# AronCao49/MoPA

Hardware: AMD Instinct MI355X
Metric: scans/sec (joint 2D+3D train step) at 1/2/4/8 MI355X; sparse-conv HBM GB/s (higher is better)
Workload: dtype f32

## Files before the change

### include/mopa_hip.h

```cpp
#ifndef MOPA_HIP_H
#define MOPA_HIP_H
#include <stddef.h>
#include <stdint.h>
#ifdef __cplusplus
extern "C" {
#endif


size_t mopa_scan_workspace_bytes(int64_t n);
int mopa_scan_exclusive_i32(const int32_t* in, int32_t* out, int32_t n, int32_t* total, void* ws, size_t ws_bytes, void* stream);
size_t mopa_voxel_hash_workspace_bytes(int64_t n_points);
int mopa_voxel_hash_build(const int64_t* coords, int64_t n_points, uint64_t* table_keys, int32_t* table_vals, int64_t table_cap, int32_t* point_row, uint64_t* row_keys, int32_t* num_rows, int32_t* status, void* ws, size_t ws_bytes, void* stream);
size_t mopa_coarsen_workspace_bytes(int64_t n_fine_cap);
int mopa_coarsen_build(const uint64_t* fine_keys, int32_t n_fine_cap, const int32_t* n_fine_dev, uint64_t* table_keys, int32_t* table_vals, int64_t table_cap, int32_t* parent, uint64_t* coarse_keys, int32_t* num_coarse, void* ws, size_t ws_bytes, void* stream);
int mopa_group_split(const int32_t* item_row, const int32_t* n_dev, int32_t n_host, int32_t n_cap, int32_t* out, void* stream);
int mopa_rulebook_subm(const uint64_t* row_keys, int32_t num_rows, const uint64_t* table_keys, const int32_t* table_vals, int64_t table_cap, int32_t spatial_size, int32_t* nbr , void* stream);
int mopa_rulebook_updown(const uint64_t* fine_keys, const int32_t* parent, int32_t num_fine, int32_t num_coarse, int32_t* ch , int32_t* up , void* stream);
size_t mopa_points_csr_workspace_bytes(int64_t num_rows);
int mopa_points_csr(const int32_t* point_row, int32_t n_points, int32_t num_rows, int32_t* row_start , int32_t* row_points , void* ws, size_t ws_bytes, void* stream);
int mopa_rotate_points_f32(const float* points, int32_t n, const float* rot_host , float* out, void* stream);
size_t mopa_voxelize_workspace_bytes(void);
int mopa_voxelize(const float* points, int32_t n, float scale, int32_t full_scale, const double* u_host, int32_t transl, int64_t batch_index, int64_t* coords , uint8_t* keep , void* ws, size_t ws_bytes, void* stream);

int mopa_spconv_fwd(const int32_t* nbr, int32_t K, int32_t num_out, const float* in, int32_t ld_in, int32_t cin, const float* weight, int32_t cout, int32_t w_flip, float* out, int32_t ld_out, void* stream);
// ... 40 lines not shown
int mopa_bn_act_fwd(const float* x, int32_t ldx, float* y, int32_t ldy, int32_t num_rows, int32_t C, const float* gamma, const float* beta, float* running_mean, float* running_var, float momentum, float eps, float leak, int32_t act, const float* res, int32_t ld_res, int32_t training, float* stats, void* ws, size_t ws_bytes, void* stream);
int mopa_bnrelu_rows_fwd(const float* x, int32_t ldx, float* y, int32_t ldy, int32_t num_rows, int32_t C, const float* gamma, const float* beta, float* running_mean, float* running_var, float momentum, float eps, float leak, int32_t training, float* stats, void* ws, size_t ws_bytes, void* stream);
size_t mopa_bnrelu_rows_bwd_workspace_bytes(int32_t num_rows, int32_t C);
int mopa_bn_act_bwd_groups(const float* dy, int32_t ld_dy, const float* x, int32_t ldx, float* dx, int32_t ld_dx, int32_t num_rows, int32_t C, int32_t n_groups, int32_t split1, int32_t split2, const float* stats, float leak, int32_t act, const float* ymask, int32_t ld_ym, float* dres, int32_t ld_dres, int32_t accumulate_dres, int32_t training, float* dgamma, float* dbeta, int32_t accumulate_param_grads, int32_t accumulate_dx, void* ws, size_t ws_bytes, void* stream);
size_t mopa_bn_act_bwd_groups_fused_workspace_bytes(int32_t num_rows, int32_t C);
int mopa_bn_act_bwd_groups_fused(const float* dy, int32_t ld_dy, const float* x, int32_t ldx, float* dx, int32_t ld_dx, int32_t num_rows, int32_t C, int32_t n_groups, int32_t split1, int32_t split2, const float* stats, float leak, int32_t act, int32_t use_bits, const uint32_t* bits, float* dres, int32_t ld_dres, int32_t accumulate_dres, int32_t training, float* dgamma, float* dbeta, int32_t accumulate_param_grads, int32_t accumulate_dx, float* colsum_partial, void* ws, size_t ws_bytes, void* stream);
int mopa_bn_bwd_sums_groups(const float* dy, int32_t ld_dy, const float* x, int32_t ldx, int32_t num_rows, int32_t C, int32_t n_groups, int32_t split1, int32_t split2, const float* stats, float leak, int32_t act, const float* ymask, int32_t ld_ym, float* dgamma, float* dbeta, int32_t accumulate_param_grads, float* coef_out, void* ws, size_t ws_bytes, void* stream);
int mopa_bn_bwd_sums_groups_pool(const float* dpool, int32_t ld_dpool, const uint8_t* argmax, int32_t B, int32_t H, int32_t W, float* dy, int32_t ld_dy, int32_t accumulate_dy, const float* x, int32_t ldx, int32_t C, int32_t n_groups, const float* stats, float leak, int32_t act, float* dgamma, float* dbeta, int32_t accumulate_param_grads, float* coef_out, void* ws, size_t ws_bytes, void* stream);
int mopa_bn_act_bwd(const float* dy, int32_t ld_dy, const float* x, int32_t ldx, float* dx, int32_t ld_dx, int32_t num_rows, int32_t C, const float* stats, float leak, int32_t act, const float* ymask, int32_t ld_ym, float* dres, int32_t ld_dres, int32_t accumulate_dres, int32_t training, float* dgamma, float* dbeta, int32_t accumulate_param_grads, int32_t accumulate_dx, void* ws, size_t ws_bytes, void* stream);
int mopa_bnrelu_rows_bwd(const float* dy, int32_t ld_dy, const float* x, int32_t ldx, float* dx, int32_t ld_dx, int32_t num_rows, int32_t C, const float* stats, float leak, int32_t training, float* dgamma, float* dbeta, int32_t accumulate_param_grads, int32_t accumulate_dx, void* ws, size_t ws_bytes, void* stream);
int mopa_bn_sync_moments(const float* x, int32_t ldx, int32_t num_rows, int32_t C, double* moments, void* ws, size_t ws_bytes, void* stream);
int mopa_bn_act_fwd_sync(const float* x, int32_t ldx, float* y, int32_t ldy, int32_t num_rows, int32_t C, const float* gamma, const float* beta, float* running_mean, float* running_var, float momentum, float eps, float leak, int32_t act, const float* res, int32_t ld_res, const double* gathered, int32_t world, float* stats, void* stream);
int mopa_bn_sync_bwd_sums(const float* dy, int32_t ld_dy, const float* x, int32_t ldx, int32_t num_rows, int32_t C, const float* stats, float leak, int32_t act, const float* ymask, int32_t ld_ym, float* dgamma, float* dbeta, int32_t accumulate_param_grads, double* sums, void* ws, size_t ws_bytes, void* stream);
int mopa_bn_act_bwd_sync(const float* dy, int32_t ld_dy, const float* x, int32_t ldx, float* dx, int32_t ld_dx, int32_t num_rows, int32_t C, const float* stats, float leak, int32_t act, const float* ymask, int32_t ld_ym, float* dres, int32_t ld_dres, int32_t accumulate_dres, const double* sums_global, const double* gathered, int32_t world, int32_t accumulate_dx, float* coef_ws, void* stream);
int mopa_rows_add(const float* a, int32_t lda, const float* b, int32_t ldb, float* out, int32_t ldo, int32_t rows, int32_t C, void* stream);
int mopa_input_layer_fwd(const float* feats, int32_t cin, const int32_t* row_start, const int32_t* row_points, int32_t num_rows, float* out, int32_t ld_out, void* stream);
int mopa_input_layer_bwd(const float* dout, int32_t ld_dout, const int32_t* point_row, const int32_t* row_start, int32_t n_points, int32_t cin, float* dfeats, void* stream);
int mopa_heads_supported(int32_t M, int32_t num_classes);
int mopa_output_layer_heads_fwd(const float* y, int32_t ld_y, const int32_t* point_row, int32_t n_points, int32_t M, int32_t num_classes, const float* w1, const float* b1, const float* w2, const float* b2, float* feats, float* logit1, float* logit2, void* stream);
size_t mopa_output_layer_heads_bwd_workspace_bytes(int32_t n_points, int32_t M, int32_t num_classes);
int mopa_output_layer_heads_bwd(const float* dfeats, const float* dl1, const float* dl2, const float* feats, const float* w1, const float* w2, const int32_t* row_start, const int32_t* row_points, int32_t num_rows, int32_t n_points, int32_t M, int32_t num_classes, float* dy, int32_t ld_dy, float* dw1, float* db1, float* dw2, float* db2, int32_t accumulate, void* ws, size_t ws_bytes, void* stream);
int mopa_zero_rows(float* x, int32_t ld, int64_t rows, int32_t C, void* stream);
int mopa_copy_rows(const float* src, int32_t ld_src, float* dst, int32_t ld_dst, int64_t rows, int32_t C, void* stream);
int mopa_add_i64_many(const int64_t* ptrs_host, int32_t n, int64_t value, void* stream);

int mopa_conv2d_igemm(const float* in, const float* weight, const float* bias, float* out, const int32_t* geom_host, int32_t flags, void* stream);
int mopa_conv2d_igemm_classes(const float* in, const float* weight, const float* bias, float* out, const int32_t* geom4_host, int32_t flags, void* stream);
int mopa_conv2d_igemm_batched(const float* in, const float* weight, float* out, const int32_t* geom_host, int32_t nbatch, int64_t in_stride, int64_t w_stride, int64_t out_stride, int32_t flags, void* stream);
size_t mopa_conv2d_wgrad_workspace_bytes(const int32_t* geom_host);
int mopa_conv2d_bwd_weight(const float* in, const float* dy, float* dweight, const int32_t* geom_host, int32_t flags, void* ws, size_t ws_bytes, void* stream);
size_t mopa_convt_wgrad_workspace_bytes(const int32_t* geom_host);
int mopa_convt_bwd_weight(const float* in, const float* dy, float* dweight, const int32_t* geom_host, int32_t flags, void* ws, size_t ws_bytes, void* stream);
int mopa_stem_bwd_weight_bn(const float* in, const float* dy, int32_t ld_dy, const float* xbn, int32_t ld_x, const float* stats, const float* coef, int32_t n_groups, int32_t training, float* dweight, const int32_t* geom_host, int32_t flags, void* ws, size_t ws_bytes, void* stream);
int mopa_stem_bwd_weight2(const float* in, const float* dy, float* dweight, const int32_t* geom_host, int32_t flags, void* ws, size_t ws_bytes, void* stream);
int mopa_stem_bwd_weight_bn2(const float* in, const float* dy, int32_t ld_dy, const float* xbn, int32_t ld_x, const float* stats, const float* coef, int32_t n_groups, int32_t training, float* dweight, const int32_t* geom_host, int32_t flags, void* ws, size_t ws_bytes, void* stream);
int mopa_stem_fwd(const float* in, const float* weight, float* out, const int32_t* geom_host, void* stream);
size_t mopa_wino_wgrad_workspace_bytes(int32_t T, int32_t Cin, int32_t Cout);
int mopa_wino_bwd_weight(const float* V, const float* dM, int32_t T, int32_t Cin, int32_t Cout, float* dweight, int32_t flags, void* ws, size_t ws_bytes, void* stream);
size_t mopa_wino4_wgrad_workspace_bytes(int32_t T, int32_t Cin, int32_t Cout);
int mopa_wino4_bwd_weight(const float* V, const float* dM, int32_t T, int32_t Cin, int32_t Cout, float* dweight, int32_t flags, void* ws, size_t ws_bytes, void* stream);
int mopa_conv2d_relayout_weight(const float* src, float* dst, int32_t O, int32_t I, int32_t KH, int32_t KW, int32_t mode, int32_t inverse, int32_t accumulate, void* stream);
int mopa_conv2d_stem_relayout(const float* src, float* dst, int32_t O, int32_t inverse, int32_t accumulate, void* stream);
int mopa_img_to_nhwc4(const float* img, int32_t B, int32_t H, int32_t W, int32_t Hp, int32_t Wp, float* out, void* stream);
int mopa_stem_dgrad_image(const float* dout, int32_t ld, int32_t B, int32_t Hp, int32_t Wp, int32_t H, int32_t W, const float* w, float* dimg, void* stream);

int mopa_wino_weight(const float* weight, int32_t O, int32_t I, int32_t dgrad, float* U, void* stream);
int mopa_wino_input(const float* in, int32_t ld_in, int32_t B, int32_t H, int32_t W, int32_t C, float* V, void* stream);
int mopa_wino_output(const float* M, int32_t B, int32_t H, int32_t W, int32_t C, const float* bias, float* out, int32_t ld_out, int32_t accumulate, void* stream);
int mopa_wino_dout(const float* dy, int32_t ld, int32_t B, int32_t H, int32_t W, int32_t C, float* dM, void* stream);
int mopa_wino4_weight(const float* weight, int32_t O, int32_t I, int32_t dgrad, float* U, void* stream);
int mopa_wino4_input(const float* in, int32_t ld_in, int32_t B, int32_t H, int32_t W, int32_t C, float* V, void* stream);
int mopa_wino4_input_bn(const float* in, int32_t ld_in, int32_t B, int32_t H, int32_t W, int32_t C, const float* stats, int32_t n_groups, int32_t bn_c0, float* V, void* stream);
int mopa_wino4_output(const float* M, int32_t B, int32_t H, int32_t W, int32_t C, const float* bias, float* out, int32_t ld_out, int32_t accumulate, void* stream);
int mopa_wino4_dout(const float* dy, int32_t ld, int32_t B, int32_t H, int32_t W, int32_t C, float* dM, void* stream);
int mopa_conv2d_weight_forms_batched(const int64_t* desc_host, int32_t n, void* stream);
int mopa_wino4_weight_t(const float* weight, int32_t O, int32_t I, int32_t dgrad, float* Ut, void* stream);
int mopa_wino4_gemm_output(const float* V, const float* Ut, const float* bias, float* out, int32_t ld_out, int32_t B, int32_t H, int32_t W, int32_t Cin, int32_t Cout, int32_t accumulate, void* stream);
int mopa_wino4_weight_f(const float* weight, int32_t O, int32_t I, int32_t dgrad, float* Uf, void* stream);
int mopa_wino4_weight_q(const float* weight, int32_t O, int32_t I, int32_t dgrad, float* Uq, void* stream);
int mopa_wino4_conv_tiles32(int32_t mode);
int mopa_wino4_conv(const float* in, int32_t ld_in, const float* Uf, const float* bias, float* out, int32_t ld_out, int32_t B, int32_t H, int32_t W, int32_t Cin, int32_t Cout, int32_t accumulate, const float* stats, int32_t n_groups, int32_t bn_c0, float* V, void* stream);

int mopa_wino4_conv9(const float* in, int32_t ld_in, const float* Uq, const float* bias, float* out, int32_t ld_out, int32_t B, int32_t H, int32_t W, int32_t Cin, int32_t Cout, int32_t accumulate, const float* stats, int32_t n_groups, int32_t bn_c0, void* stream);

int mopa_wino4_wgrad_fused_ok(int32_t B, int32_t H, int32_t W, int32_t Cin, int32_t Cout);
size_t mopa_wino4_wgrad_fused_workspace_bytes(int32_t B, int32_t H, int32_t W, int32_t Cin, int32_t Cout);
int mopa_wino4_wgrad_fused(const float* in, int32_t ld_in, const float* stats, int32_t n_groups, int32_t bn_c0, const float* dy, int32_t ld_dy, int32_t B, int32_t H, int32_t W, int32_t Cin, int32_t Cout, float* dweight, int32_t flags, void* ws, size_t ws_bytes, void* stream);

int mopa_maxpool3x3s2_fwd(const float* x, int32_t ldx, int32_t B, int32_t H, int32_t W, int32_t C, float* y, int32_t ldy, uint8_t* argmax, void* stream);
int mopa_maxpool3x3s2_fwd_bn(const float* x, int32_t ldx, int32_t B, int32_t H, int32_t W, int32_t C, const float* stats, int32_t n_groups, float* y, int32_t ldy, uint8_t* argmax, void* stream);
int mopa_maxpool3x3s2_bwd(const float* dy, int32_t ld_dy, const uint8_t* argmax, int32_t B, int32_t H, int32_t W, int32_t C, float* dx, int32_t ld_dx, int32_t accumulate, void* stream);
int mopa_dropout_rows(const float* x, int32_t ldx, float* y, int32_t ldy, int64_t rows, int32_t C, float p, uint64_t seed, void* stream);
int mopa_dropout_rows_dseed(const float* x, int32_t ldx, float* y, int32_t ldy, int64_t rows, int32_t C, float p, const int64_t* seed_dev, int32_t site, void* stream);
int mopa_pixel_head_supported(int32_t M, int32_t num_classes);
int mopa_pixel_head_fwd(const float* x, int32_t ld, int32_t B, int32_t Hp, int32_t Wp, int32_t H, int32_t W, int32_t M, int32_t num_classes, const float* w, const float* bias, float* pred, void* stream);
size_t mopa_pixel_head_bwd_workspace_bytes(int32_t B, int32_t H, int32_t W, int32_t M, int32_t num_classes);
int mopa_pixel_head_bwd(const float* dpred, const float* x, int32_t ld, int32_t B, int32_t Hp, int32_t Wp, int32_t H, int32_t W, int32_t M, int32_t num_classes, const float* w, float* dx, int32_t ld_dx, int32_t accumulate_dx, float* dw, float* db, int32_t accumulate_params, void* ws, size_t ws_bytes, void* stream);
size_t mopa_colsum_workspace_bytes(int64_t num_rows, int32_t C);
int mopa_colsum(const float* x, int32_t ld, int64_t num_rows, int32_t C, float* out, int32_t accumulate, void* ws, size_t ws_bytes, void* stream);
size_t mopa_colsum_partial_blocks(int64_t num_rows);
int mopa_colsum_reduce(const float* partial, int64_t num_rows, int32_t C, float* out, int32_t accumulate, void* stream);
int mopa_pack_point_pix(const int64_t* idx, const int64_t* off_host, int32_t B, int32_t H, int32_t W, int32_t* pix, int32_t* status, void* stream);

size_t mopa_loss_workspace_bytes(int64_t n_rows);
int mopa_softmax_kl_fwd(const float* logit_p, const float* logit_q, int32_t N, int32_t C, float* loss, void* ws, size_t ws_bytes, void* stream);
int mopa_softmax_kl_bwd(const float* logit_p, const float* logit_q, int32_t N, int32_t C, const float* gout, float* dlogit_p, void* stream);
int mopa_wce_fwd(const float* logits, const int64_t* labels, const float* class_weight, int32_t N, int32_t C, int64_t ignore_index, float* loss, float* den, int32_t* status, void* ws, size_t ws_bytes, void* stream);
int mopa_wce_bwd(const float* logits, const int64_t* labels, const float* class_weight, int32_t N, int32_t C, int64_t ignore_index, const float* den, const float* gout, float* dlogits, void* stream);
size_t mopa_point_losses_workspace_bytes(int64_t n_rows);
int mopa_point_losses_fwd(const float* z2_main, const float* z2_xm, const float* z3_main, const float* z3_xm, const int64_t* y2, const int64_t* y3, const float* class_weight, int32_t N, int32_t C, int64_t ignore_index, float* scalars, int64_t* conf_2d, int64_t* conf_3d, const uint8_t* acc_mask, int64_t* acc_out, int32_t* status, void* ws, size_t ws_bytes, void* stream);
int mopa_point_losses_bwd(const float* z_main, const float* z_xm, const float* z_other_main, const int64_t* y, const float* class_weight, int32_t N, int32_t C, int64_t ignore_index, const float* den, const float* g, float* dz_main, float* dz_xm, void* stream);
size_t mopa_point_losses_seg_workspace_bytes(int32_t S);
int mopa_point_losses_seg_fwd(const float* z2_main, const float* z2_xm, const float* z3_main, const float* z3_xm, const float* class_weight, const int64_t* segs_host, int32_t S, int64_t N2, int64_t N3, int32_t C, int64_t ignore_index, float* scalars, int32_t* status, void* ws, size_t ws_bytes, void* stream);
int mopa_point_losses_seg_bwd(int32_t net, const float* z_main, const float* z_xm, const float* z_other_main, const float* class_weight, const int64_t* segs_host, int32_t S, int64_t N, int64_t N_other, int32_t C, int64_t ignore_index, const float* scalars, const float* g, float* dz_main, float* dz_xm, void* stream);
int mopa_softmax_fwd(const float* logits, int64_t n_rows, int32_t C, float* probs, void* stream);
int mopa_softmax_bwd(const float* probs, const float* dprobs, int64_t n_rows, int32_t C, float* dlogits, void* stream);
size_t mopa_mask_cons_workspace_bytes(int32_t B, int32_t HW, int32_t C);
size_t mopa_mask_cons_state_floats(int32_t B, int32_t C);
int mopa_mask_cons_fwd(const float* probs, const int32_t* masks, int32_t B, int32_t HW, int32_t C, int32_t k_norm, int32_t min_entropy, float* loss, float* state, void* ws, size_t ws_bytes, void* stream);
int mopa_mask_cons_bwd(const float* probs, const int32_t* masks, int32_t B, int32_t HW, int32_t C, int32_t k_norm, int32_t min_entropy, const float* state, const float* gout, float* dprobs, void* stream);

int mopa_pseudo_fuse(const float* logit_a, const float* logit_b, int32_t N, int32_t C, float* maxp, int64_t* label, void* stream);
size_t mopa_refine_pseudo_labels_workspace_bytes(int32_t C);
int mopa_refine_pseudo_labels(const float* prob, const int64_t* label_in, int32_t N, int32_t C, int64_t ignore_label, int64_t* label_out, void* ws, size_t ws_bytes, void* stream);
int mopa_ema_update(float* shadow, const float* param, int64_t n, float decay, void* stream);

int mopa_vgi_zslots(void);
int mopa_vgi_first_points(const float* points, int32_t stride, int32_t n, float voxel_size, int32_t ox, int32_t oy, int32_t X, int32_t Y, int32_t zlo, const uint8_t* g_mask, int32_t* first, int32_t* status, void* stream);
size_t mopa_vgi_first_points_rep_workspace_bytes(int32_t X, int32_t Y);
int mopa_vgi_first_points_rep(const float* points, int32_t stride, int32_t n, float voxel_size, double voxel_size64, int32_t ox, int32_t oy, int32_t X, int32_t Y, int32_t zlo, int32_t* first, int32_t* status, void* ws, size_t ws_bytes, void* stream);
size_t mopa_vgi_box_free_workspace_bytes(int32_t X, int32_t Y, int32_t Z);
int mopa_vgi_box_free(const int32_t* first, int32_t X, int32_t Y, int32_t zlo, int32_t gz0, int32_t Z, int32_t bx, int32_t by, int32_t bz, uint8_t* free_cells, void* ws, size_t ws_bytes, void* stream);
int mopa_vgi_ground_cells(const int32_t* first, const uint8_t* g_mask, int32_t X, int32_t Y, uint8_t* ground2d, void* stream);
int mopa_vgi_candidates(const uint8_t* free_cells, int32_t Xo, int32_t Yo, int32_t Zo, const double* params_host, const uint8_t* ground2d, int32_t ox, int32_t oy, int32_t X, int32_t Y, uint8_t* cand2d, int32_t* counts, void* stream);
int mopa_vgi_compact_cells(const uint8_t* cand2d, int32_t X, int32_t Y, int32_t ox, int32_t oy, int32_t* cells , int32_t* count, void* stream);
int mopa_vgi_road_height(const float* points, int32_t stride, int32_t n, float voxel_size, const int32_t* first, const uint8_t* g_mask, int32_t ox, int32_t oy, int32_t X, int32_t Y, int32_t zlo, int32_t cell_x, int32_t cell_y, double* out , void* stream);
// ... 96 lines not shown
```

### mopa_amd/_abi.py

```python
SIGNATURES = {
    'mopa_scan_workspace_bytes': ('z', 'l'),
    'mopa_scan_exclusive_i32': ('i', 'ppippzp'),
    'mopa_voxel_hash_workspace_bytes': ('z', 'l'),
    'mopa_voxel_hash_build': ('i', 'plpplpppppzp'),
    'mopa_coarsen_workspace_bytes': ('z', 'l'),
    'mopa_coarsen_build': ('i', 'pippplppppzp'),
    'mopa_group_split': ('i', 'ppiipp'),
    'mopa_rulebook_subm': ('i', 'pipplipp'),
    'mopa_rulebook_updown': ('i', 'ppiippp'),
    'mopa_points_csr_workspace_bytes': ('z', 'l'),
    'mopa_points_csr': ('i', 'piipppzp'),
    'mopa_rotate_points_f32': ('i', 'pippp'),
    'mopa_voxelize_workspace_bytes': ('z', ''),
    'mopa_voxelize': ('i', 'pifipilpppzp'),
    'mopa_spconv_fwd': ('i', 'piipiipiipip'),
    'mopa_rulebook_groups_count': ('i', 'piipp'),
    'mopa_rulebook_groups_fill': ('i', 'piippppp'),
    'mopa_rulebook_groups_count_batched': ('i', 'piipp'),
    'mopa_rulebook_groups_fill_batched': ('i', 'piippppp'),
    'mopa_spconv_grouped_wants_packed': ('i', 'iiii'),
    'mopa_spconv_pack_weight': ('i', 'piiiiipp'),
    'mopa_spconv_pack_weights_batched': ('i', 'pip'),
    'mopa_spconv_grouped_workspace_bytes': ('z', 'iii'),
    'mopa_spconv_fwd_grouped': ('i', 'ppppiipiipiipipzp'),
# ... 25 lines not shown
    'mopa_bn_act_fwd_groups': ('i', 'pipiiiiiippppfffipiippzp'),
    'mopa_bn_act_fwd_groups_bits': ('i', 'pipiiiiiippppfffipiipippzp'),
    'mopa_bn_act_fwd': ('i', 'pipiiippppfffipiippzp'),
    'mopa_bnrelu_rows_fwd': ('i', 'pipiiippppfffippzp'),
    'mopa_bnrelu_rows_bwd_workspace_bytes': ('z', 'ii'),
    'mopa_bn_act_bwd_groups': ('i', 'pipipiiiiiipfipipiiippiipzp'),
    'mopa_bn_act_bwd_groups_fused_workspace_bytes': ('z', 'ii'),
    'mopa_bn_act_bwd_groups_fused': ('i', 'pipipiiiiiipfiippiiippiippzp'),
    'mopa_bn_bwd_sums_groups': ('i', 'pipiiiiiipfipippippzp'),
    'mopa_bn_bwd_sums_groups_pool': ('i', 'pipiiipiipiiipfippippzp'),
    'mopa_bn_act_bwd': ('i', 'pipipiiipfipipiiippiipzp'),
    'mopa_bnrelu_rows_bwd': ('i', 'pipipiiipfippiipzp'),
    'mopa_bn_sync_moments': ('i', 'piiippzp'),
    'mopa_bn_act_fwd_sync': ('i', 'pipiiippppfffipipipp'),
    'mopa_bn_sync_bwd_sums': ('i', 'pipiiipfipippippzp'),
    'mopa_bn_act_bwd_sync': ('i', 'pipipiiipfipipiippiipp'),
    'mopa_rows_add': ('i', 'pipipiiip'),
    'mopa_input_layer_fwd': ('i', 'pippipip'),
    'mopa_input_layer_bwd': ('i', 'pippiipp'),
    'mopa_heads_supported': ('i', 'ii'),
    'mopa_output_layer_heads_fwd': ('i', 'pipiiipppppppp'),
    'mopa_output_layer_heads_bwd_workspace_bytes': ('z', 'iii'),
    'mopa_output_layer_heads_bwd': ('i', 'ppppppppiiiipippppipzp'),
    'mopa_zero_rows': ('i', 'pilip'),
    'mopa_copy_rows': ('i', 'pipilip'),
    'mopa_add_i64_many': ('i', 'pilp'),
    'mopa_conv2d_igemm': ('i', 'pppppip'),
    'mopa_conv2d_igemm_classes': ('i', 'pppppip'),
    'mopa_conv2d_igemm_batched': ('i', 'ppppilllip'),
    'mopa_conv2d_wgrad_workspace_bytes': ('z', 'p'),
    'mopa_conv2d_bwd_weight': ('i', 'ppppipzp'),
    'mopa_convt_wgrad_workspace_bytes': ('z', 'p'),
    'mopa_convt_bwd_weight': ('i', 'ppppipzp'),
    'mopa_stem_bwd_weight_bn': ('i', 'ppipippiippipzp'),
    'mopa_stem_bwd_weight2': ('i', 'ppppipzp'),
    'mopa_stem_bwd_weight_bn2': ('i', 'ppipippiippipzp'),
    'mopa_stem_fwd': ('i', 'ppppp'),
    'mopa_wino_wgrad_workspace_bytes': ('z', 'iii'),
    'mopa_wino_bwd_weight': ('i', 'ppiiipipzp'),
    'mopa_wino4_wgrad_workspace_bytes': ('z', 'iii'),
    'mopa_wino4_bwd_weight': ('i', 'ppiiipipzp'),
    'mopa_conv2d_relayout_weight': ('i', 'ppiiiiiiip'),
    'mopa_conv2d_stem_relayout': ('i', 'ppiiip'),
    'mopa_img_to_nhwc4': ('i', 'piiiiipp'),
    'mopa_stem_dgrad_image': ('i', 'piiiiiippp'),
    'mopa_wino_weight': ('i', 'piiipp'),
    'mopa_wino_input': ('i', 'piiiiipp'),
    'mopa_wino_output': ('i', 'piiiippiip'),
    'mopa_wino_dout': ('i', 'piiiiipp'),
    'mopa_wino4_weight': ('i', 'piiipp'),
    'mopa_wino4_input': ('i', 'piiiiipp'),
    'mopa_wino4_input_bn': ('i', 'piiiiipiipp'),
    'mopa_wino4_output': ('i', 'piiiippiip'),
    'mopa_wino4_dout': ('i', 'piiiiipp'),
    'mopa_conv2d_weight_forms_batched': ('i', 'pip'),
    'mopa_wino4_weight_t': ('i', 'piiipp'),
    'mopa_wino4_gemm_output': ('i', 'ppppiiiiiiip'),
    'mopa_wino4_weight_f': ('i', 'piiipp'),
    'mopa_wino4_weight_q': ('i', 'piiipp'),
    'mopa_wino4_conv_tiles32': ('i', 'i'),
    'mopa_wino4_conv': ('i', 'pipppiiiiiiipiipp'),
    'mopa_wino4_conv9': ('i', 'pipppiiiiiiipiip'),
    'mopa_wino4_wgrad_fused_ok': ('i', 'iiiii'),
    'mopa_wino4_wgrad_fused_workspace_bytes': ('z', 'iiiii'),
    'mopa_wino4_wgrad_fused': ('i', 'pipiipiiiiiipipzp'),
    'mopa_maxpool3x3s2_fwd': ('i', 'piiiiipipp'),
    'mopa_maxpool3x3s2_fwd_bn': ('i', 'piiiiipipipp'),
    'mopa_maxpool3x3s2_bwd': ('i', 'pipiiiipiip'),
    'mopa_dropout_rows': ('i', 'pipilifup'),
    'mopa_dropout_rows_dseed': ('i', 'pipilifpip'),
    'mopa_pixel_head_supported': ('i', 'ii'),
    'mopa_pixel_head_fwd': ('i', 'piiiiiiiipppp'),
    'mopa_pixel_head_bwd_workspace_bytes': ('z', 'iiiii'),
    'mopa_pixel_head_bwd': ('i', 'ppiiiiiiiippiippipzp'),
    'mopa_colsum_workspace_bytes': ('z', 'li'),
    'mopa_colsum': ('i', 'pilipipzp'),
    'mopa_colsum_partial_blocks': ('z', 'l'),
    'mopa_colsum_reduce': ('i', 'plipip'),
    'mopa_pack_point_pix': ('i', 'ppiiippp'),
    'mopa_loss_workspace_bytes': ('z', 'l'),
    'mopa_softmax_kl_fwd': ('i', 'ppiippzp'),
    'mopa_softmax_kl_bwd': ('i', 'ppiippp'),
    'mopa_wce_fwd': ('i', 'pppiilppppzp'),
    'mopa_wce_bwd': ('i', 'pppiilpppp'),
    'mopa_point_losses_workspace_bytes': ('z', 'l'),
    'mopa_point_losses_fwd': ('i', 'pppppppiilpppppppzp'),
    'mopa_point_losses_bwd': ('i', 'pppppiilppppp'),
    'mopa_point_losses_seg_workspace_bytes': ('z', 'i'),
    'mopa_point_losses_seg_fwd': ('i', 'ppppppillilpppzp'),
    'mopa_point_losses_seg_bwd': ('i', 'ipppppillilppppp'),
    'mopa_softmax_fwd': ('i', 'plipp'),
    'mopa_softmax_bwd': ('i', 'pplipp'),
    'mopa_mask_cons_workspace_bytes': ('z', 'iii'),
    'mopa_mask_cons_state_floats': ('z', 'ii'),
    'mopa_mask_cons_fwd': ('i', 'ppiiiiipppzp'),
    'mopa_mask_cons_bwd': ('i', 'ppiiiiipppp'),
    'mopa_pseudo_fuse': ('i', 'ppiippp'),
    'mopa_refine_pseudo_labels_workspace_bytes': ('z', 'i'),
    'mopa_refine_pseudo_labels': ('i', 'ppiilppzp'),
    'mopa_ema_update': ('i', 'pplfp'),
    'mopa_vgi_zslots': ('i', ''),
    'mopa_vgi_first_points': ('i', 'piifiiiiipppp'),
    'mopa_vgi_first_points_rep_workspace_bytes': ('z', 'ii'),
    'mopa_vgi_first_points_rep': ('i', 'piifdiiiiipppzp'),
    'mopa_vgi_box_free_workspace_bytes': ('z', 'iii'),
    'mopa_vgi_box_free': ('i', 'piiiiiiiippzp'),
    'mopa_vgi_ground_cells': ('i', 'ppiipp'),
    'mopa_vgi_candidates': ('i', 'piiippiiiippp'),
    'mopa_vgi_compact_cells': ('i', 'piiiippp'),
    'mopa_vgi_road_height': ('i', 'piifppiiiiiiipp'),
    'mopa_vgi_range_keep_workspace_bytes': ('z', 'iii'),
    'mopa_vgi_range_keep': ('i', 'piiddiippzp'),
    'mopa_voxelize_f64_workspace_bytes': ('z', ''),
    'mopa_voxelize_f64': ('i', 'pippdipilpppzp'),
    'mopa_eval_logits_workspace_bytes': ('z', 'ii'),
# ... 135 lines not shown
```

### mopa_amd/csrc/common.h

```cpp
#pragma once
#include <hip/hip_runtime.h>
#include <stdint.h>
#include <stddef.h>

#define MOPA_OK 0
#define MOPA_ERR_ARG (-1)
#define MOPA_ERR_WORKSPACE (-2)
#define MOPA_ERR_LAUNCH (-3)
#define MOPA_ERR_UNSUPPORTED (-4)
#define MOPA_ERR_DATA (-5)

#define MOPA_API extern "C" __attribute__((visibility("default")))

#define MOPA_CHECK_LAUNCH()                                  \
  do {                                                       \
    if (hipGetLastError() != hipSuccess) return MOPA_ERR_LAUNCH; \
  } while (0)

static inline int64_t cdiv64(int64_t a, int64_t b) { return (a + b - 1) / b; }
static inline size_t align_up(size_t x, size_t a) { return (x + a - 1) / a * a; }
static inline int colsum_rows(int64_t num_rows) {
  int64_t r = cdiv64(num_rows, 2048);
  if (r < 32) r = 32;
  if (r > 1024) r = 1024;
  return (int)r;
}

static inline int stream_grid(int64_t work_items, int block) {
  int64_t g = cdiv64(work_items, block);
  if (g < 1) g = 1;
  if (g > 2048) g = 2048;
  return (int)g;
}

#include <atomic>
static inline int mopa_device_index() {
  int dev = 0;
  return hipGetDevice(&dev) == hipSuccess && dev >= 0 && dev < 64 ? dev : -1;
}
static inline int mopa_cu_count() {
  static std::atomic<int> cus[64];
  const int dev = mopa_device_index();
  if (dev < 0) return 0;
  int n = cus[dev].load(std::memory_order_relaxed);
  if (n == 0) {
    hipDeviceProp_t prop;
    if (hipGetDeviceProperties(&prop, dev) != hipSuccess) return 0;
    n = prop.multiProcessorCount > 0 ? prop.multiProcessorCount : 256;
    cus[dev].store(n, std::memory_order_relaxed);
  }
  return n;
}

#define WAVE 64

__device__ __forceinline__ float wave_sum(float v) {
#pragma unroll
  for (int o = 32; o > 0; o >>= 1) v += __shfl_xor(v, o, 64);
  return v;
}
__device__ __forceinline__ double wave_sum_d(double v) {
#pragma unroll
  for (int o = 32; o > 0; o >>= 1) v += __shfl_xor(v, o, 64);
  return v;
}
__device__ __forceinline__ int wave_sum_i(int v) {
#pragma unroll
  for (int o = 32; o > 0; o >>= 1) v += __shfl_xor(v, o, 64);
  return v;
}
```

### mopa_amd/csrc/exec_table.inc

```
static const char* const EXEC_NAMES[] = {
  "mopa_a2d2prep_map",
  "mopa_a2d2prep_points",
  "mopa_a2d2prep_remap",
  "mopa_adam_flat",
  "mopa_adam_flat_guarded",
  "mopa_adamw_flat",
  "mopa_adamw_flat_guarded",
  "mopa_add_i64_many",
  "mopa_bn_act_bwd",
  "mopa_bn_act_bwd_groups",
  "mopa_bn_act_bwd_groups_fused",
  "mopa_bn_act_bwd_sync",
  "mopa_bn_act_fwd",
  "mopa_bn_act_fwd_groups",
  "mopa_bn_act_fwd_groups_bits",
  "mopa_bn_act_fwd_sync",
  "mopa_bn_bwd_sums_groups",
  "mopa_bn_bwd_sums_groups_pool",
  "mopa_bn_sync_bwd_sums",
  "mopa_bn_sync_moments",
  "mopa_bnrelu_rows_bwd",
  "mopa_bnrelu_rows_fwd",
  "mopa_coarsen_build",
  "mopa_colsum",
// ... 55 lines not shown
  "mopa_refine_pseudo_labels_segmented",
  "mopa_rotate_points_f32",
  "mopa_rows_add",
  "mopa_rulebook_groups_count",
  "mopa_rulebook_groups_count_batched",
  "mopa_rulebook_groups_fill",
  "mopa_rulebook_groups_fill_batched",
  "mopa_rulebook_runs_build_batched",
  "mopa_rulebook_subm",
  "mopa_rulebook_updown",
  "mopa_scan_exclusive_i32",
  "mopa_scanprep_compact",
  "mopa_scanprep_count",
  "mopa_scanprep_rotate",
  "mopa_scanprep_take",
  "mopa_scn_backward",
  "mopa_scn_forward",
  "mopa_sgd_flat",
  "mopa_sgd_flat_guarded",
  "mopa_softmax_bwd",
  "mopa_softmax_fwd",
  "mopa_softmax_kl_bwd",
  "mopa_softmax_kl_fwd",
  "mopa_spconv_bwd_weight",
  "mopa_spconv_bwd_weight_run",
  "mopa_spconv_fwd",
  "mopa_spconv_fwd_grouped",
  "mopa_spconv_fwd_run",
  "mopa_spconv_pack_weight",
  "mopa_spconv_pack_weights_batched",
  "mopa_spconv_run_pack_weight",
  "mopa_spconv_transpose_weight",
  "mopa_stem_bwd_weight2",
  "mopa_stem_bwd_weight_bn",
  "mopa_stem_bwd_weight_bn2",
  "mopa_stem_dgrad_image",
  "mopa_stem_fwd",
  "mopa_vgi_box_free",
  "mopa_vgi_candidates",
  "mopa_vgi_compact_cells",
  "mopa_vgi_first_points",
  "mopa_vgi_first_points_rep",
  "mopa_vgi_ground_cells",
  "mopa_vgi_range_keep",
  "mopa_vgi_road_height",
  "mopa_voxel_hash_build",
  "mopa_voxelize",
  "mopa_voxelize_f64",
  "mopa_wce_bwd",
  "mopa_wce_fwd",
  "mopa_wino4_bwd_weight",
  "mopa_wino4_conv",
  "mopa_wino4_conv9",
  "mopa_wino4_dout",
  "mopa_wino4_gemm_output",
  "mopa_wino4_input",
  "mopa_wino4_input_bn",
  "mopa_wino4_output",
  "mopa_wino4_weight",
  "mopa_wino4_weight_f",
  "mopa_wino4_weight_q",
  "mopa_wino4_weight_t",
  "mopa_wino4_wgrad_fused",
  "mopa_wino_bwd_weight",
  "mopa_wino_dout",
  "mopa_wino_input",
  "mopa_wino_output",
  "mopa_wino_weight",
  "mopa_zero_rows",
};
static const int EXEC_N = 148;
static int exec_dispatch(int id, const int64_t* a, int nargs) {
  switch (id) {
    case 0: return nargs == 6 ? mopa_a2d2prep_map((const double*)(uintptr_t)a[0], (int32_t)a[1], (int32_t)a[2], (int16_t*)(uintptr_t)a[3], (uint16_t*)(uintptr_t)a[4], (void*)(uintptr_t)a[5]) : MOPA_ERR_ARG;
    case 1: return nargs == 21 ? mopa_a2d2prep_points((const void* const*)(uintptr_t)a[0], (const void* const*)(uintptr_t)a[1], (const void* const*)(uintptr_t)a[2], (const void* const*)(uintptr_t)a[3], (const void* const*)(uintptr_t)a[4], (const int32_t*)(uintptr_t)a[5], (int32_t)a[6], (int32_t)a[7], (int32_t)a[8], (const int16_t*)(uintptr_t)a[9], (const uint16_t*)(uintptr_t)a[10], (int32_t)a[11], (int32_t)a[12], (const uint8_t*)(uintptr_t)a[13], (int32_t)a[14], (float*)(uintptr_t)a[15], (float*)(uintptr_t)a[16], (uint8_t*)(uintptr_t)a[17], (float*)(uintptr_t)a[18], (int32_t*)(uintptr_t)a[19], (void*)(uintptr_t)a[20]) : MOPA_ERR_ARG;
    case 2: return nargs == 8 ? mopa_a2d2prep_remap((const void* const*)(uintptr_t)a[0], (void* const*)(uintptr_t)a[1], (int32_t)a[2], (int32_t)a[3], (int32_t)a[4], (const int16_t*)(uintptr_t)a[5], (const uint16_t*)(uintptr_t)a[6], (void*)(uintptr_t)a[7]) : MOPA_ERR_ARG;
    case 3: return nargs == 14 ? mopa_adam_flat((float*)(uintptr_t)a[0], (const float*)(uintptr_t)a[1], (float*)(uintptr_t)a[2], (float*)(uintptr_t)a[3], (int64_t)a[4], (float)slot_f(a[5]), (float)slot_f(a[6]), (float)slot_f(a[7]), (float)slot_f(a[8]), (float)slot_f(a[9]), (float)slot_f(a[10]), (float)slot_f(a[11]), (float)slot_f(a[12]), (void*)(uintptr_t)a[13]) : MOPA_ERR_ARG;
    case 4: return nargs == 15 ? mopa_adam_flat_guarded((float*)(uintptr_t)a[0], (const float*)(uintptr_t)a[1], (float*)(uintptr_t)a[2], (float*)(uintptr_t)a[3], (int64_t)a[4], (float)slot_f(a[5]), (float)slot_f(a[6]), (float)slot_f(a[7]), (float)slot_f(a[8]), (float)slot_f(a[9]), (float)slot_f(a[10]), (float)slot_f(a[11]), (float)slot_f(a[12]), (const void*)(uintptr_t)a[13], (void*)(uintptr_t)a[14]) : MOPA_ERR_ARG;
    case 5: return nargs == 14 ? mopa_adamw_flat((float*)(uintptr_t)a[0], (const float*)(uintptr_t)a[1], (float*)(uintptr_t)a[2], (float*)(uintptr_t)a[3], (int64_t)a[4], (float)slot_f(a[5]), (float)slot_f(a[6]), (float)slot_f(a[7]), (float)slot_f(a[8]), (float)slot_f(a[9]), (float)slot_f(a[10]), (float)slot_f(a[11]), (float)slot_f(a[12]), (void*)(uintptr_t)a[13]) : MOPA_ERR_ARG;
    case 6: return nargs == 15 ? mopa_adamw_flat_guarded((float*)(uintptr_t)a[0], (const float*)(uintptr_t)a[1], (float*)(uintptr_t)a[2], (float*)(uintptr_t)a[3], (int64_t)a[4], (float)slot_f(a[5]), (float)slot_f(a[6]), (float)slot_f(a[7]), (float)slot_f(a[8]), (float)slot_f(a[9]), (float)slot_f(a[10]), (float)slot_f(a[11]), (float)slot_f(a[12]), (const void*)(uintptr_t)a[13], (void*)(uintptr_t)a[14]) : MOPA_ERR_ARG;
    case 7: return nargs == 4 ? mopa_add_i64_many((const int64_t*)(uintptr_t)a[0], (int32_t)a[1], (int64_t)a[2], (void*)(uintptr_t)a[3]) : MOPA_ERR_ARG;
    case 8: return nargs == 24 ? mopa_bn_act_bwd((const float*)(uintptr_t)a[0], (int32_t)a[1], (const float*)(uintptr_t)a[2], (int32_t)a[3], (float*)(uintptr_t)a[4], (int32_t)a[5], (int32_t)a[6], (int32_t)a[7], (const float*)(uintptr_t)a[8], (float)slot_f(a[9]), (int32_t)a[10], (const float*)(uintptr_t)a[11], (int32_t)a[12], (float*)(uintptr_t)a[13], (int32_t)a[14], (int32_t)a[15], (int32_t)a[16], (float*)(uintptr_t)a[17], (float*)(uintptr_t)a[18], (int32_t)a[19], (int32_t)a[20], (void*)(uintptr_t)a[21], (size_t)a[22], (void*)(uintptr_t)a[23]) : MOPA_ERR_ARG;
    case 9: return nargs == 27 ? mopa_bn_act_bwd_groups((const float*)(uintptr_t)a[0], (int32_t)a[1], (const float*)(uintptr_t)a[2], (int32_t)a[3], (float*)(uintptr_t)a[4], (int32_t)a[5], (int32_t)a[6], (int32_t)a[7], (int32_t)a[8], (int32_t)a[9], (int32_t)a[10], (const float*)(uintptr_t)a[11], (float)slot_f(a[12]), (int32_t)a[13], (const float*)(uintptr_t)a[14], (int32_t)a[15], (float*)(uintptr_t)a[16], (int32_t)a[17], (int32_t)a[18], (int32_t)a[19], (float*)(uintptr_t)a[20], (float*)(uintptr_t)a[21], (int32_t)a[22], (int32_t)a[23], (void*)(uintptr_t)a[24], (size_t)a[25], (void*)(uintptr_t)a[26]) : MOPA_ERR_ARG;
    case 10: return nargs == 28 ? mopa_bn_act_bwd_groups_fused((const float*)(uintptr_t)a[0], (int32_t)a[1], (const float*)(uintptr_t)a[2], (int32_t)a[3], (float*)(uintptr_t)a[4], (int32_t)a[5], (int32_t)a[6], (int32_t)a[7], (int32_t)a[8], (int32_t)a[9], (int32_t)a[10], (const float*)(uintptr_t)a[11], (float)slot_f(a[12]), (int32_t)a[13], (int32_t)a[14], (const uint32_t*)(uintptr_t)a[15], (float*)(uintptr_t)a[16], (int32_t)a[17], (int32_t)a[18], (int32_t)a[19], (float*)(uintptr_t)a[20], (float*)(uintptr_t)a[21], (int32_t)a[22], (int32_t)a[23], (float*)(uintptr_t)a[24], (void*)(uintptr_t)a[25], (size_t)a[26], (void*)(uintptr_t)a[27]) : MOPA_ERR_ARG;
    case 11: return nargs == 22 ? mopa_bn_act_bwd_sync((const float*)(uintptr_t)a[0], (int32_t)a[1], (const float*)(uintptr_t)a[2], (int32_t)a[3], (float*)(uintptr_t)a[4], (int32_t)a[5], (int32_t)a[6], (int32_t)a[7], (const float*)(uintptr_t)a[8], (float)slot_f(a[9]), (int32_t)a[10], (const float*)(uintptr_t)a[11], (int32_t)a[12], (float*)(uintptr_t)a[13], (int32_t)a[14], (int32_t)a[15], (const double*)(uintptr_t)a[16], (const double*)(uintptr_t)a[17], (int32_t)a[18], (int32_t)a[19], (float*)(uintptr_t)a[20], (void*)(uintptr_t)a[21]) : MOPA_ERR_ARG;
    case 12: return nargs == 21 ? mopa_bn_act_fwd((const float*)(uintptr_t)a[0], (int32_t)a[1], (float*)(uintptr_t)a[2], (int32_t)a[3], (int32_t)a[4], (int32_t)a[5], (const float*)(uintptr_t)a[6], (const float*)(uintptr_t)a[7], (float*)(uintptr_t)a[8], (float*)(uintptr_t)a[9], (float)slot_f(a[10]), (float)slot_f(a[11]), (float)slot_f(a[12]), (int32_t)a[13], (const float*)(uintptr_t)a[14], (int32_t)a[15], (int32_t)a[16], (float*)(uintptr_t)a[17], (void*)(uintptr_t)a[18], (size_t)a[19], (void*)(uintptr_t)a[20]) : MOPA_ERR_ARG;
    case 13: return nargs == 24 ? mopa_bn_act_fwd_groups((const float*)(uintptr_t)a[0], (int32_t)a[1], (float*)(uintptr_t)a[2], (int32_t)a[3], (int32_t)a[4], (int32_t)a[5], (int32_t)a[6], (int32_t)a[7], (int32_t)a[8], (const float*)(uintptr_t)a[9], (const float*)(uintptr_t)a[10], (float*)(uintptr_t)a[11], (float*)(uintptr_t)a[12], (float)slot_f(a[13]), (float)slot_f(a[14]), (float)slot_f(a[15]), (int32_t)a[16], (const float*)(uintptr_t)a[17], (int32_t)a[18], (int32_t)a[19], (float*)(uintptr_t)a[20], (void*)(uintptr_t)a[21], (size_t)a[22], (void*)(uintptr_t)a[23]) : MOPA_ERR_ARG;
    case 14: return nargs == 26 ? mopa_bn_act_fwd_groups_bits((const float*)(uintptr_t)a[0], (int32_t)a[1], (float*)(uintptr_t)a[2], (int32_t)a[3], (int32_t)a[4], (int32_t)a[5], (int32_t)a[6], (int32_t)a[7], (int32_t)a[8], (const float*)(uintptr_t)a[9], (const float*)(uintptr_t)a[10], (float*)(uintptr_t)a[11], (float*)(uintptr_t)a[12], (float)slot_f(a[13]), (float)slot_f(a[14]), (float)slot_f(a[15]), (int32_t)a[16], (const float*)(uintptr_t)a[17], (int32_t)a[18], (int32_t)a[19], (float*)(uintptr_t)a[20], (int32_t)a[21], (uint32_t*)(uintptr_t)a[22], (void*)(uintptr_t)a[23], (size_t)a[24], (void*)(uintptr_t)a[25]) : MOPA_ERR_ARG;
    case 15: return nargs == 20 ? mopa_bn_act_fwd_sync((const float*)(uintptr_t)a[0], (int32_t)a[1], (float*)(uintptr_t)a[2], (int32_t)a[3], (int32_t)a[4], (int32_t)a[5], (const float*)(uintptr_t)a[6], (const float*)(uintptr_t)a[7], (float*)(uintptr_t)a[8], (float*)(uintptr_t)a[9], (float)slot_f(a[10]), (float)slot_f(a[11]), (float)slot_f(a[12]), (int32_t)a[13], (const float*)(uintptr_t)a[14], (int32_t)a[15], (const double*)(uintptr_t)a[16], (int32_t)a[17], (float*)(uintptr_t)a[18], (void*)(uintptr_t)a[19]) : MOPA_ERR_ARG;
    case 16: return nargs == 21 ? mopa_bn_bwd_sums_groups((const float*)(uintptr_t)a[0], (int32_t)a[1], (const float*)(uintptr_t)a[2], (int32_t)a[3], (int32_t)a[4], (int32_t)a[5], (int32_t)a[6], (int32_t)a[7], (int32_t)a[8], (const float*)(uintptr_t)a[9], (float)slot_f(a[10]), (int32_t)a[11], (const float*)(uintptr_t)a[12], (int32_t)a[13], (float*)(uintptr_t)a[14], (float*)(uintptr_t)a[15], (int32_t)a[16], (float*)(uintptr_t)a[17], (void*)(uintptr_t)a[18], (size_t)a[19], (void*)(uintptr_t)a[20]) : MOPA_ERR_ARG;
    case 17: return nargs == 23 ? mopa_bn_bwd_sums_groups_pool((const float*)(uintptr_t)a[0], (int32_t)a[1], (const uint8_t*)(uintptr_t)a[2], (int32_t)a[3], (int32_t)a[4], (int32_t)a[5], (float*)(uintptr_t)a[6], (int32_t)a[7], (int32_t)a[8], (const float*)(uintptr_t)a[9], (int32_t)a[10], (int32_t)a[11], (int32_t)a[12], (const float*)(uintptr_t)a[13], (float)slot_f(a[14]), (int32_t)a[15], (float*)(uintptr_t)a[16], (float*)(uintptr_t)a[17], (int32_t)a[18], (float*)(uintptr_t)a[19], (void*)(uintptr_t)a[20], (size_t)a[21], (void*)(uintptr_t)a[22]) : MOPA_ERR_ARG;
    case 18: return nargs == 18 ? mopa_bn_sync_bwd_sums((const float*)(uintptr_t)a[0], (int32_t)a[1], (const float*)(uintptr_t)a[2], (int32_t)a[3], (int32_t)a[4], (int32_t)a[5], (const float*)(uintptr_t)a[6], (float)slot_f(a[7]), (int32_t)a[8], (const float*)(uintptr_t)a[9], (int32_t)a[10], (float*)(uintptr_t)a[11], (float*)(uintptr_t)a[12], (int32_t)a[13], (double*)(uintptr_t)a[14], (void*)(uintptr_t)a[15], (size_t)a[16], (void*)(uintptr_t)a[17]) : MOPA_ERR_ARG;
    case 19: return nargs == 8 ? mopa_bn_sync_moments((const float*)(uintptr_t)a[0], (int32_t)a[1], (int32_t)a[2], (int32_t)a[3], (double*)(uintptr_t)a[4], (void*)(uintptr_t)a[5], (size_t)a[6], (void*)(uintptr_t)a[7]) : MOPA_ERR_ARG;
    case 20: return nargs == 18 ? mopa_bnrelu_rows_bwd((const float*)(uintptr_t)a[0], (int32_t)a[1], (const float*)(uintptr_t)a[2], (int32_t)a[3], (float*)(uintptr_t)a[4], (int32_t)a[5], (int32_t)a[6], (int32_t)a[7], (const float*)(uintptr_t)a[8], (float)slot_f(a[9]), (int32_t)a[10], (float*)(uintptr_t)a[11], (float*)(uintptr_t)a[12], (int32_t)a[13], (int32_t)a[14], (void*)(uintptr_t)a[15], (size_t)a[16], (void*)(uintptr_t)a[17]) : MOPA_ERR_ARG;
    case 21: return nargs == 18 ? mopa_bnrelu_rows_fwd((const float*)(uintptr_t)a[0], (int32_t)a[1], (float*)(uintptr_t)a[2], (int32_t)a[3], (int32_t)a[4], (int32_t)a[5], (const float*)(uintptr_t)a[6], (const float*)(uintptr_t)a[7], (float*)(uintptr_t)a[8], (float*)(uintptr_t)a[9], (float)slot_f(a[10]), (float)slot_f(a[11]), (float)slot_f(a[12]), (int32_t)a[13], (float*)(uintptr_t)a[14], (void*)(uintptr_t)a[15], (size_t)a[16], (void*)(uintptr_t)a[17]) : MOPA_ERR_ARG;
    case 22: return nargs == 12 ? mopa_coarsen_build((const uint64_t*)(uintptr_t)a[0], (int32_t)a[1], (const int32_t*)(uintptr_t)a[2], (uint64_t*)(uintptr_t)a[3], (int32_t*)(uintptr_t)a[4], (int64_t)a[5], (int32_t*)(uintptr_t)a[6], (uint64_t*)(uintptr_t)a[7], (int32_t*)(uintptr_t)a[8], (void*)(uintptr_t)a[9], (size_t)a[10], (void*)(uintptr_t)a[11]) : MOPA_ERR_ARG;
    case 23: return nargs == 9 ? mopa_colsum((const float*)(uintptr_t)a[0], (int32_t)a[1], (int64_t)a[2], (int32_t)a[3], (float*)(uintptr_t)a[4], (int32_t)a[5], (void*)(uintptr_t)a[6], (size_t)a[7], (void*)(uintptr_t)a[8]) : MOPA_ERR_ARG;
    case 24: return nargs == 6 ? mopa_colsum_reduce((const float*)(uintptr_t)a[0], (int64_t)a[1], (int32_t)a[2], (float*)(uintptr_t)a[3], (int32_t)a[4], (void*)(uintptr_t)a[5]) : MOPA_ERR_ARG;
    case 25: return nargs == 8 ? mopa_confusion_update((const int64_t*)(uintptr_t)a[0], (const int64_t*)(uintptr_t)a[1], (int64_t)a[2], (const int32_t*)(uintptr_t)a[3], (int32_t)a[4], (int32_t)a[5], (int64_t*)(uintptr_t)a[6], (void*)(uintptr_t)a[7]) : MOPA_ERR_ARG;
    case 26: return nargs == 8 ? mopa_conv2d_bwd_weight((const float*)(uintptr_t)a[0], (const float*)(uintptr_t)a[1], (float*)(uintptr_t)a[2], (const int32_t*)(uintptr_t)a[3], (int32_t)a[4], (void*)(uintptr_t)a[5], (size_t)a[6], (void*)(uintptr_t)a[7]) : MOPA_ERR_ARG;
    case 27: return nargs == 7 ? mopa_conv2d_igemm((const float*)(uintptr_t)a[0], (const float*)(uintptr_t)a[1], (const float*)(uintptr_t)a[2], (float*)(uintptr_t)a[3], (const int32_t*)(uintptr_t)a[4], (int32_t)a[5], (void*)(uintptr_t)a[6]) : MOPA_ERR_ARG;
    case 28: return nargs == 10 ? mopa_conv2d_igemm_batched((const float*)(uintptr_t)a[0], (const float*)(uintptr_t)a[1], (float*)(uintptr_t)a[2], (const int32_t*)(uintptr_t)a[3], (int32_t)a[4], (int64_t)a[5], (int64_t)a[6], (int64_t)a[7], (int32_t)a[8], (void*)(uintptr_t)a[9]) : MOPA_ERR_ARG;
    case 29: return nargs == 7 ? mopa_conv2d_igemm_classes((const float*)(uintptr_t)a[0], (const float*)(uintptr_t)a[1], (const float*)(uintptr_t)a[2], (float*)(uintptr_t)a[3], (const int32_t*)(uintptr_t)a[4], (int32_t)a[5], (void*)(uintptr_t)a[6]) : MOPA_ERR_ARG;
    case 30: return nargs == 10 ? mopa_conv2d_relayout_weight((const float*)(uintptr_t)a[0], (float*)(uintptr_t)a[1], (int32_t)a[2], (int32_t)a[3], (int32_t)a[4], (int32_t)a[5], (int32_t)a[6], (int32_t)a[7], (int32_t)a[8], (void*)(uintptr_t)a[9]) : MOPA_ERR_ARG;
    case 31: return nargs == 6 ? mopa_conv2d_stem_relayout((const float*)(uintptr_t)a[0], (float*)(uintptr_t)a[1], (int32_t)a[2], (int32_t)a[3], (int32_t)a[4], (void*)(uintptr_t)a[5]) : MOPA_ERR_ARG;
    case 32: return nargs == 3 ? mopa_conv2d_weight_forms_batched((const int64_t*)(uintptr_t)a[0], (int32_t)a[1], (void*)(uintptr_t)a[2]) : MOPA_ERR_ARG;
    case 33: return nargs == 8 ? mopa_convt_bwd_weight((const float*)(uintptr_t)a[0], (const float*)(uintptr_t)a[1], (float*)(uintptr_t)a[2], (const int32_t*)(uintptr_t)a[3], (int32_t)a[4], (void*)(uintptr_t)a[5], (size_t)a[6], (void*)(uintptr_t)a[7]) : MOPA_ERR_ARG;
    case 34: return nargs == 7 ? mopa_copy_rows((const float*)(uintptr_t)a[0], (int32_t)a[1], (float*)(uintptr_t)a[2], (int32_t)a[3], (int64_t)a[4], (int32_t)a[5], (void*)(uintptr_t)a[6]) : MOPA_ERR_ARG;
    case 35: return nargs == 20 ? mopa_denselabels((const void* const*)(uintptr_t)a[0], (const void* const*)(uintptr_t)a[1], (const void* const*)(uintptr_t)a[2], (int)a[3], (const int32_t*)(uintptr_t)a[4], (const void* const*)(uintptr_t)a[5], (int)a[6], (int)a[7], (int)a[8], (int)a[9], (int)a[10], (const int32_t*)(uintptr_t)a[11], (int)a[12], (int)a[13], (const int32_t*)(uintptr_t)a[14], (int32_t*)(uintptr_t)a[15], (int32_t*)(uintptr_t)a[16], (void*)(uintptr_t)a[17], (size_t)a[18], (void*)(uintptr_t)a[19]) : MOPA_ERR_ARG;
    case 36: return nargs == 9 ? mopa_dropout_rows((const float*)(uintptr_t)a[0], (int32_t)a[1], (float*)(uintptr_t)a[2], (int32_t)a[3], (int64_t)a[4], (int32_t)a[5], (float)slot_f(a[6]), (uint64_t)a[7], (void*)(uintptr_t)a[8]) : MOPA_ERR_ARG;
    case 37: return nargs == 10 ? mopa_dropout_rows_dseed((const float*)(uintptr_t)a[0], (int32_t)a[1], (float*)(uintptr_t)a[2], (int32_t)a[3], (int64_t)a[4], (int32_t)a[5], (float)slot_f(a[6]), (const int64_t*)(uintptr_t)a[7], (int32_t)a[8], (void*)(uintptr_t)a[9]) : MOPA_ERR_ARG;
    case 38: return nargs == 5 ? mopa_ema_update((float*)(uintptr_t)a[0], (const float*)(uintptr_t)a[1], (int64_t)a[2], (float)slot_f(a[3]), (void*)(uintptr_t)a[4]) : MOPA_ERR_ARG;
    case 39: return nargs == 20 ? mopa_eval_logits((const float*)(uintptr_t)a[0], (int64_t)a[1], (const float*)(uintptr_t)a[2], (int64_t)a[3], (const int64_t*)(uintptr_t)a[4], (int32_t)a[5], (int32_t)a[6], (const int32_t*)(uintptr_t)a[7], (int32_t)a[8], (int32_t)a[9], (int64_t*)(uintptr_t)a[10], (int64_t*)(uintptr_t)a[11], (int64_t*)(uintptr_t)a[12], (int64_t*)(uintptr_t)a[13], (float*)(uintptr_t)a[14], (uint8_t*)(uintptr_t)a[15], (float*)(uintptr_t)a[16], (void*)(uintptr_t)a[17], (size_t)a[18], (void*)(uintptr_t)a[19]) : MOPA_ERR_ARG;
    case 40: return nargs == 12 ? mopa_grad_stats((const float*)(uintptr_t)a[0], (const void*)(uintptr_t)a[1], (int64_t)a[2], (int64_t)a[3], (float)slot_f(a[4]), (float)slot_f(a[5]), (int)a[6], (float*)(uintptr_t)a[7], (void*)(uintptr_t)a[8], (void*)(uintptr_t)a[9], (size_t)a[10], (void*)(uintptr_t)a[11]) : MOPA_ERR_ARG;
    case 41: return nargs == 11 ? mopa_ground_estimate((const float*)(uintptr_t)a[0], (int32_t)a[1], (const int32_t*)(uintptr_t)a[2], (int32_t)a[3], (int64_t)a[4], (int64_t)a[5], (const double*)(uintptr_t)a[6], (uint8_t*)(uintptr_t)a[7], (void*)(uintptr_t)a[8], (size_t)a[9], (void*)(uintptr_t)a[10]) : MOPA_ERR_ARG;
    case 42: return nargs == 6 ? mopa_group_split((const int32_t*)(uintptr_t)a[0], (const int32_t*)(uintptr_t)a[1], (int32_t)a[2], (int32_t)a[3], (int32_t*)(uintptr_t)a[4], (void*)(uintptr_t)a[5]) : MOPA_ERR_ARG;
    case 43: return nargs == 9 ? mopa_imageprep_contrast_sums((const void* const*)(uintptr_t)a[0], (int)a[1], (int64_t)a[2], (int)a[3], (int)a[4], (const int32_t*)(uintptr_t)a[5], (const float*)(uintptr_t)a[6], (void*)(uintptr_t)a[7], (void*)(uintptr_t)a[8]) : MOPA_ERR_ARG;
    case 44: return nargs == 10 ? mopa_imageprep_contrast_sums4((const void* const*)(uintptr_t)a[0], (int)a[1], (int64_t)a[2], (int)a[3], (int)a[4], (const int32_t*)(uintptr_t)a[5], (const float*)(uintptr_t)a[6], (const int32_t*)(uintptr_t)a[7], (void*)(uintptr_t)a[8], (void*)(uintptr_t)a[9]) : MOPA_ERR_ARG;
    case 45: return nargs == 15 ? mopa_imageprep_indices((const void* const*)(uintptr_t)a[0], (const int32_t*)(uintptr_t)a[1], (int)a[2], (int)a[3], (int)a[4], (double)slot_f(a[5]), (double)slot_f(a[6]), (const int32_t*)(uintptr_t)a[7], (int)a[8], (const int32_t*)(uintptr_t)a[9], (void* const*)(uintptr_t)a[10], (void* const*)(uintptr_t)a[11], (void* const*)(uintptr_t)a[12], (int32_t*)(uintptr_t)a[13], (void*)(uintptr_t)a[14]) : MOPA_ERR_ARG;
    case 46: return nargs == 20 ? mopa_imageprep_mask((const void* const*)(uintptr_t)a[0], (int)a[1], (int)a[2], (int)a[3], (const int32_t*)(uintptr_t)a[4], (const int32_t*)(uintptr_t)a[5], (int)a[6], (int)a[7], (int)a[8], (int)a[9], (const int32_t*)(uintptr_t)a[10], (const int32_t*)(uintptr_t)a[11], (const int32_t*)(uintptr_t)a[12], (int)a[13], (int)a[14], (const int32_t*)(uintptr_t)a[15], (int32_t*)(uintptr_t)a[16], (void*)(uintptr_t)a[17], (size_t)a[18], (void*)(uintptr_t)a[19]) : MOPA_ERR_ARG;
    case 47: return nargs == 14 ? mopa_imageprep_pixels((const void* const*)(uintptr_t)a[0], (int)a[1], (int64_t)a[2], (int)a[3], (int)a[4], (const int32_t*)(uintptr_t)a[5], (const float*)(uintptr_t)a[6], (const void*)(uintptr_t)a[7], (const int32_t*)(uintptr_t)a[8], (uint8_t*)(uintptr_t)a[9], (float*)(uintptr_t)a[10], (const float*)(uintptr_t)a[11], (float*)(uintptr_t)a[12], (void*)(uintptr_t)a[13]) : MOPA_ERR_ARG;
    case 48: return nargs == 15 ? mopa_imageprep_pixels4((const void* const*)(uintptr_t)a[0], (int)a[1], (int64_t)a[2], (int)a[3], (int)a[4], (const int32_t*)(uintptr_t)a[5], (const float*)(uintptr_t)a[6], (const int32_t*)(uintptr_t)a[7], (const void*)(uintptr_t)a[8], (const int32_t*)(uintptr_t)a[9], (uint8_t*)(uintptr_t)a[10], (float*)(uintptr_t)a[11], (const float*)(uintptr_t)a[12], (float*)(uintptr_t)a[13], (void*)(uintptr_t)a[14]) : MOPA_ERR_ARG;
    case 49: return nargs == 13 ? mopa_imageprep_resize_u8((const void* const*)(uintptr_t)a[0], (int)a[1], (int)a[2], (int)a[3], (const int32_t*)(uintptr_t)a[4], (int)a[5], (const int32_t*)(uintptr_t)a[6], (int)a[7], (int)a[8], (int)a[9], (int)a[10], (uint8_t*)(uintptr_t)a[11], (void*)(uintptr_t)a[12]) : MOPA_ERR_ARG;
    case 50: return nargs == 8 ? mopa_img_to_nhwc4((const float*)(uintptr_t)a[0], (int32_t)a[1], (int32_t)a[2], (int32_t)a[3], (int32_t)a[4], (int32_t)a[5], (float*)(uintptr_t)a[6], (void*)(uintptr_t)a[7]) : MOPA_ERR_ARG;
// ... 28 lines not shown
    case 79: return nargs == 11 ? mopa_refine_pseudo_labels_segmented((const void* const*)(uintptr_t)a[0], (const void* const*)(uintptr_t)a[1], (int32_t)a[2], (const int32_t*)(uintptr_t)a[3], (void* const*)(uintptr_t)a[4], (int32_t)a[5], (int32_t)a[6], (int64_t)a[7], (void*)(uintptr_t)a[8], (size_t)a[9], (void*)(uintptr_t)a[10]) : MOPA_ERR_ARG;
    case 80: return nargs == 5 ? mopa_rotate_points_f32((const float*)(uintptr_t)a[0], (int32_t)a[1], (const float*)(uintptr_t)a[2], (float*)(uintptr_t)a[3], (void*)(uintptr_t)a[4]) : MOPA_ERR_ARG;
    case 81: return nargs == 9 ? mopa_rows_add((const float*)(uintptr_t)a[0], (int32_t)a[1], (const float*)(uintptr_t)a[2], (int32_t)a[3], (float*)(uintptr_t)a[4], (int32_t)a[5], (int32_t)a[6], (int32_t)a[7], (void*)(uintptr_t)a[8]) : MOPA_ERR_ARG;
    case 82: return nargs == 5 ? mopa_rulebook_groups_count((const int32_t*)(uintptr_t)a[0], (int32_t)a[1], (int32_t)a[2], (int32_t*)(uintptr_t)a[3], (void*)(uintptr_t)a[4]) : MOPA_ERR_ARG;
    case 83: return nargs == 5 ? mopa_rulebook_groups_count_batched((const int64_t*)(uintptr_t)a[0], (int32_t)a[1], (int32_t)a[2], (int32_t*)(uintptr_t)a[3], (void*)(uintptr_t)a[4]) : MOPA_ERR_ARG;
    case 84: return nargs == 8 ? mopa_rulebook_groups_fill((const int32_t*)(uintptr_t)a[0], (int32_t)a[1], (int32_t)a[2], (const int32_t*)(uintptr_t)a[3], (int32_t*)(uintptr_t)a[4], (int32_t*)(uintptr_t)a[5], (int32_t*)(uintptr_t)a[6], (void*)(uintptr_t)a[7]) : MOPA_ERR_ARG;
    case 85: return nargs == 8 ? mopa_rulebook_groups_fill_batched((const int64_t*)(uintptr_t)a[0], (int32_t)a[1], (int32_t)a[2], (const int32_t*)(uintptr_t)a[3], (int32_t*)(uintptr_t)a[4], (int32_t*)(uintptr_t)a[5], (int32_t*)(uintptr_t)a[6], (void*)(uintptr_t)a[7]) : MOPA_ERR_ARG;
    case 86: return nargs == 3 ? mopa_rulebook_runs_build_batched((const int64_t*)(uintptr_t)a[0], (int32_t)a[1], (void*)(uintptr_t)a[2]) : MOPA_ERR_ARG;
    case 87: return nargs == 8 ? mopa_rulebook_subm((const uint64_t*)(uintptr_t)a[0], (int32_t)a[1], (const uint64_t*)(uintptr_t)a[2], (const int32_t*)(uintptr_t)a[3], (int64_t)a[4], (int32_t)a[5], (int32_t*)(uintptr_t)a[6], (void*)(uintptr_t)a[7]) : MOPA_ERR_ARG;
    case 88: return nargs == 7 ? mopa_rulebook_updown((const uint64_t*)(uintptr_t)a[0], (const int32_t*)(uintptr_t)a[1], (int32_t)a[2], (int32_t)a[3], (int32_t*)(uintptr_t)a[4], (int32_t*)(uintptr_t)a[5], (void*)(uintptr_t)a[6]) : MOPA_ERR_ARG;
    case 89: return nargs == 7 ? mopa_scan_exclusive_i32((const int32_t*)(uintptr_t)a[0], (int32_t*)(uintptr_t)a[1], (int32_t)a[2], (int32_t*)(uintptr_t)a[3], (void*)(uintptr_t)a[4], (size_t)a[5], (void*)(uintptr_t)a[6]) : MOPA_ERR_ARG;
    case 90: return nargs == 22 ? mopa_scanprep_compact((const void* const*)(uintptr_t)a[0], (const void* const*)(uintptr_t)a[1], (const int32_t*)(uintptr_t)a[2], (const double*)(uintptr_t)a[3], (const int32_t*)(uintptr_t)a[4], (int32_t)a[5], (int32_t)a[6], (int32_t)a[7], (float)slot_f(a[8]), (int32_t)a[9], (int32_t)a[10], (const uint8_t*)(uintptr_t)a[11], (int64_t*)(uintptr_t)a[12], (int64_t*)(uintptr_t)a[13], (int64_t*)(uintptr_t)a[14], (int64_t)a[15], (uint8_t*)(uintptr_t)a[16], (int64_t*)(uintptr_t)a[17], (int32_t*)(uintptr_t)a[18], (void*)(uintptr_t)a[19], (size_t)a[20], (void*)(uintptr_t)a[21]) : MOPA_ERR_ARG;
    case 91: return nargs == 15 ? mopa_scanprep_count((const void* const*)(uintptr_t)a[0], (const void* const*)(uintptr_t)a[1], (const int32_t*)(uintptr_t)a[2], (const double*)(uintptr_t)a[3], (const int32_t*)(uintptr_t)a[4], (int32_t)a[5], (int32_t)a[6], (float)slot_f(a[7]), (int32_t)a[8], (int32_t)a[9], (uint8_t*)(uintptr_t)a[10], (int64_t*)(uintptr_t)a[11], (void*)(uintptr_t)a[12], (size_t)a[13], (void*)(uintptr_t)a[14]) : MOPA_ERR_ARG;
    case 92: return nargs == 6 ? mopa_scanprep_rotate((const void* const*)(uintptr_t)a[0], (void* const*)(uintptr_t)a[1], (const int32_t*)(uintptr_t)a[2], (const float*)(uintptr_t)a[3], (int32_t)a[4], (void*)(uintptr_t)a[5]) : MOPA_ERR_ARG;
    case 93: return nargs == 20 ? mopa_scanprep_take((const int64_t*)(uintptr_t)a[0], (int64_t)a[1], (int64_t)a[2], (const int32_t*)(uintptr_t)a[3], (int32_t)a[4], (const void* const*)(uintptr_t)a[5], (int32_t)a[6], (const int64_t*)(uintptr_t)a[7], (int64_t)a[8], (int64_t)a[9], (const void* const*)(uintptr_t)a[10], (const void* const*)(uintptr_t)a[11], (const int64_t*)(uintptr_t)a[12], (const int64_t*)(uintptr_t)a[13], (int64_t*)(uintptr_t)a[14], (int64_t*)(uintptr_t)a[15], (float*)(uintptr_t)a[16], (int64_t*)(uintptr_t)a[17], (int64_t*)(uintptr_t)a[18], (void*)(uintptr_t)a[19]) : MOPA_ERR_ARG;
    case 94: return nargs == 14 ? mopa_scn_backward((const int32_t*)(uintptr_t)a[0], (int32_t)a[1], (const int32_t*)(uintptr_t)a[2], (int32_t)a[3], (const int64_t*)(uintptr_t)a[4], (int64_t*)(uintptr_t)a[5], (const int64_t*)(uintptr_t)a[6], (const int64_t*)(uintptr_t)a[7], (const int64_t*)(uintptr_t)a[8], (const int64_t*)(uintptr_t)a[9], (const int64_t*)(uintptr_t)a[10], (void*)(uintptr_t)a[11], (size_t)a[12], (void*)(uintptr_t)a[13]) : MOPA_ERR_ARG;
    case 95: return nargs == 10 ? mopa_scn_forward((const int32_t*)(uintptr_t)a[0], (int32_t)a[1], (const int64_t*)(uintptr_t)a[2], (int64_t*)(uintptr_t)a[3], (const int64_t*)(uintptr_t)a[4], (const int64_t*)(uintptr_t)a[5], (const int64_t*)(uintptr_t)a[6], (void*)(uintptr_t)a[7], (size_t)a[8], (void*)(uintptr_t)a[9]) : MOPA_ERR_ARG;
    case 96: return nargs == 12 ? mopa_sgd_flat((float*)(uintptr_t)a[0], (const float*)(uintptr_t)a[1], (float*)(uintptr_t)a[2], (int64_t)a[3], (float)slot_f(a[4]), (float)slot_f(a[5]), (float)slot_f(a[6]), (float)slot_f(a[7]), (int)a[8], (int)a[9], (float)slot_f(a[10]), (void*)(uintptr_t)a[11]) : MOPA_ERR_ARG;
    case 97: return nargs == 13 ? mopa_sgd_flat_guarded((float*)(uintptr_t)a[0], (const float*)(uintptr_t)a[1], (float*)(uintptr_t)a[2], (int64_t)a[3], (float)slot_f(a[4]), (float)slot_f(a[5]), (float)slot_f(a[6]), (float)slot_f(a[7]), (int)a[8], (int*)(uintptr_t)a[9], (float)slot_f(a[10]), (const void*)(uintptr_t)a[11], (void*)(uintptr_t)a[12]) : MOPA_ERR_ARG;
    case 98: return nargs == 6 ? mopa_softmax_bwd((const float*)(uintptr_t)a[0], (const float*)(uintptr_t)a[1], (int64_t)a[2], (int32_t)a[3], (float*)(uintptr_t)a[4], (void*)(uintptr_t)a[5]) : MOPA_ERR_ARG;
    case 99: return nargs == 5 ? mopa_softmax_fwd((const float*)(uintptr_t)a[0], (int64_t)a[1], (int32_t)a[2], (float*)(uintptr_t)a[3], (void*)(uintptr_t)a[4]) : MOPA_ERR_ARG;
    case 100: return nargs == 7 ? mopa_softmax_kl_bwd((const float*)(uintptr_t)a[0], (const float*)(uintptr_t)a[1], (int32_t)a[2], (int32_t)a[3], (const float*)(uintptr_t)a[4], (float*)(uintptr_t)a[5], (void*)(uintptr_t)a[6]) : MOPA_ERR_ARG;
    case 101: return nargs == 8 ? mopa_softmax_kl_fwd((const float*)(uintptr_t)a[0], (const float*)(uintptr_t)a[1], (int32_t)a[2], (int32_t)a[3], (float*)(uintptr_t)a[4], (void*)(uintptr_t)a[5], (size_t)a[6], (void*)(uintptr_t)a[7]) : MOPA_ERR_ARG;
    case 102: return nargs == 14 ? mopa_spconv_bwd_weight((const int32_t*)(uintptr_t)a[0], (int32_t)a[1], (int32_t)a[2], (const float*)(uintptr_t)a[3], (int32_t)a[4], (int32_t)a[5], (const float*)(uintptr_t)a[6], (int32_t)a[7], (int32_t)a[8], (float*)(uintptr_t)a[9], (int32_t)a[10], (void*)(uintptr_t)a[11], (size_t)a[12], (void*)(uintptr_t)a[13]) : MOPA_ERR_ARG;
    case 103: return nargs == 16 ? mopa_spconv_bwd_weight_run((const int32_t*)(uintptr_t)a[0], (int32_t)a[1], (int32_t)a[2], (int32_t)a[3], (int32_t)a[4], (const float*)(uintptr_t)a[5], (int32_t)a[6], (int32_t)a[7], (const float*)(uintptr_t)a[8], (int32_t)a[9], (int32_t)a[10], (float*)(uintptr_t)a[11], (int32_t)a[12], (void*)(uintptr_t)a[13], (size_t)a[14], (void*)(uintptr_t)a[15]) : MOPA_ERR_ARG;
    case 104: return nargs == 12 ? mopa_spconv_fwd((const int32_t*)(uintptr_t)a[0], (int32_t)a[1], (int32_t)a[2], (const float*)(uintptr_t)a[3], (int32_t)a[4], (int32_t)a[5], (const float*)(uintptr_t)a[6], (int32_t)a[7], (int32_t)a[8], (float*)(uintptr_t)a[9], (int32_t)a[10], (void*)(uintptr_t)a[11]) : MOPA_ERR_ARG;
    case 105: return nargs == 17 ? mopa_spconv_fwd_grouped((const int32_t*)(uintptr_t)a[0], (const int32_t*)(uintptr_t)a[1], (const int32_t*)(uintptr_t)a[2], (const int32_t*)(uintptr_t)a[3], (int32_t)a[4], (int32_t)a[5], (const float*)(uintptr_t)a[6], (int32_t)a[7], (int32_t)a[8], (const float*)(uintptr_t)a[9], (int32_t)a[10], (int32_t)a[11], (float*)(uintptr_t)a[12], (int32_t)a[13], (void*)(uintptr_t)a[14], (size_t)a[15], (void*)(uintptr_t)a[16]) : MOPA_ERR_ARG;
    case 106: return nargs == 15 ? mopa_spconv_fwd_run((const int32_t*)(uintptr_t)a[0], (int32_t)a[1], (int32_t)a[2], (const float*)(uintptr_t)a[3], (int32_t)a[4], (int32_t)a[5], (const float*)(uintptr_t)a[6], (int32_t)a[7], (int32_t)a[8], (float*)(uintptr_t)a[9], (int32_t)a[10], (int32_t)a[11], (void*)(uintptr_t)a[12], (size_t)a[13], (void*)(uintptr_t)a[14]) : MOPA_ERR_ARG;
    case 107: return nargs == 8 ? mopa_spconv_pack_weight((const float*)(uintptr_t)a[0], (int32_t)a[1], (int32_t)a[2], (int32_t)a[3], (int32_t)a[4], (int32_t)a[5], (float*)(uintptr_t)a[6], (void*)(uintptr_t)a[7]) : MOPA_ERR_ARG;
    case 108: return nargs == 3 ? mopa_spconv_pack_weights_batched((const int64_t*)(uintptr_t)a[0], (int32_t)a[1], (void*)(uintptr_t)a[2]) : MOPA_ERR_ARG;
    case 109: return nargs == 7 ? mopa_spconv_run_pack_weight((const float*)(uintptr_t)a[0], (int32_t)a[1], (int32_t)a[2], (int32_t)a[3], (int32_t)a[4], (float*)(uintptr_t)a[5], (void*)(uintptr_t)a[6]) : MOPA_ERR_ARG;
    case 110: return nargs == 6 ? mopa_spconv_transpose_weight((const float*)(uintptr_t)a[0], (int32_t)a[1], (int32_t)a[2], (int32_t)a[3], (float*)(uintptr_t)a[4], (void*)(uintptr_t)a[5]) : MOPA_ERR_ARG;
    case 111: return nargs == 8 ? mopa_stem_bwd_weight2((const float*)(uintptr_t)a[0], (const float*)(uintptr_t)a[1], (float*)(uintptr_t)a[2], (const int32_t*)(uintptr_t)a[3], (int32_t)a[4], (void*)(uintptr_t)a[5], (size_t)a[6], (void*)(uintptr_t)a[7]) : MOPA_ERR_ARG;
    case 112: return nargs == 15 ? mopa_stem_bwd_weight_bn((const float*)(uintptr_t)a[0], (const float*)(uintptr_t)a[1], (int32_t)a[2], (const float*)(uintptr_t)a[3], (int32_t)a[4], (const float*)(uintptr_t)a[5], (const float*)(uintptr_t)a[6], (int32_t)a[7], (int32_t)a[8], (float*)(uintptr_t)a[9], (const int32_t*)(uintptr_t)a[10], (int32_t)a[11], (void*)(uintptr_t)a[12], (size_t)a[13], (void*)(uintptr_t)a[14]) : MOPA_ERR_ARG;
    case 113: return nargs == 15 ? mopa_stem_bwd_weight_bn2((const float*)(uintptr_t)a[0], (const float*)(uintptr_t)a[1], (int32_t)a[2], (const float*)(uintptr_t)a[3], (int32_t)a[4], (const float*)(uintptr_t)a[5], (const float*)(uintptr_t)a[6], (int32_t)a[7], (int32_t)a[8], (float*)(uintptr_t)a[9], (const int32_t*)(uintptr_t)a[10], (int32_t)a[11], (void*)(uintptr_t)a[12], (size_t)a[13], (void*)(uintptr_t)a[14]) : MOPA_ERR_ARG;
    case 114: return nargs == 10 ? mopa_stem_dgrad_image((const float*)(uintptr_t)a[0], (int32_t)a[1], (int32_t)a[2], (int32_t)a[3], (int32_t)a[4], (int32_t)a[5], (int32_t)a[6], (const float*)(uintptr_t)a[7], (float*)(uintptr_t)a[8], (void*)(uintptr_t)a[9]) : MOPA_ERR_ARG;
    case 115: return nargs == 5 ? mopa_stem_fwd((const float*)(uintptr_t)a[0], (const float*)(uintptr_t)a[1], (float*)(uintptr_t)a[2], (const int32_t*)(uintptr_t)a[3], (void*)(uintptr_t)a[4]) : MOPA_ERR_ARG;
    case 116: return nargs == 13 ? mopa_vgi_box_free((const int32_t*)(uintptr_t)a[0], (int32_t)a[1], (int32_t)a[2], (int32_t)a[3], (int32_t)a[4], (int32_t)a[5], (int32_t)a[6], (int32_t)a[7], (int32_t)a[8], (uint8_t*)(uintptr_t)a[9], (void*)(uintptr_t)a[10], (size_t)a[11], (void*)(uintptr_t)a[12]) : MOPA_ERR_ARG;
    case 117: return nargs == 13 ? mopa_vgi_candidates((const uint8_t*)(uintptr_t)a[0], (int32_t)a[1], (int32_t)a[2], (int32_t)a[3], (const double*)(uintptr_t)a[4], (const uint8_t*)(uintptr_t)a[5], (int32_t)a[6], (int32_t)a[7], (int32_t)a[8], (int32_t)a[9], (uint8_t*)(uintptr_t)a[10], (int32_t*)(uintptr_t)a[11], (void*)(uintptr_t)a[12]) : MOPA_ERR_ARG;
    case 118: return nargs == 8 ? mopa_vgi_compact_cells((const uint8_t*)(uintptr_t)a[0], (int32_t)a[1], (int32_t)a[2], (int32_t)a[3], (int32_t)a[4], (int32_t*)(uintptr_t)a[5], (int32_t*)(uintptr_t)a[6], (void*)(uintptr_t)a[7]) : MOPA_ERR_ARG;
    case 119: return nargs == 13 ? mopa_vgi_first_points((const float*)(uintptr_t)a[0], (int32_t)a[1], (int32_t)a[2], (float)slot_f(a[3]), (int32_t)a[4], (int32_t)a[5], (int32_t)a[6], (int32_t)a[7], (int32_t)a[8], (const uint8_t*)(uintptr_t)a[9], (int32_t*)(uintptr_t)a[10], (int32_t*)(uintptr_t)a[11], (void*)(uintptr_t)a[12]) : MOPA_ERR_ARG;
    case 120: return nargs == 15 ? mopa_vgi_first_points_rep((const float*)(uintptr_t)a[0], (int32_t)a[1], (int32_t)a[2], (float)slot_f(a[3]), (double)slot_f(a[4]), (int32_t)a[5], (int32_t)a[6], (int32_t)a[7], (int32_t)a[8], (int32_t)a[9], (int32_t*)(uintptr_t)a[10], (int32_t*)(uintptr_t)a[11], (void*)(uintptr_t)a[12], (size_t)a[13], (void*)(uintptr_t)a[14]) : MOPA_ERR_ARG;
    case 121: return nargs == 6 ? mopa_vgi_ground_cells((const int32_t*)(uintptr_t)a[0], (const uint8_t*)(uintptr_t)a[1], (int32_t)a[2], (int32_t)a[3], (uint8_t*)(uintptr_t)a[4], (void*)(uintptr_t)a[5]) : MOPA_ERR_ARG;
    case 122: return nargs == 11 ? mopa_vgi_range_keep((const double*)(uintptr_t)a[0], (int32_t)a[1], (int32_t)a[2], (double)slot_f(a[3]), (double)slot_f(a[4]), (int32_t)a[5], (int32_t)a[6], (uint8_t*)(uintptr_t)a[7], (void*)(uintptr_t)a[8], (size_t)a[9], (void*)(uintptr_t)a[10]) : MOPA_ERR_ARG;
    case 123: return nargs == 15 ? mopa_vgi_road_height((const float*)(uintptr_t)a[0], (int32_t)a[1], (int32_t)a[2], (float)slot_f(a[3]), (const int32_t*)(uintptr_t)a[4], (const uint8_t*)(uintptr_t)a[5], (int32_t)a[6], (int32_t)a[7], (int32_t)a[8], (int32_t)a[9], (int32_t)a[10], (int32_t)a[11], (int32_t)a[12], (double*)(uintptr_t)a[13], (void*)(uintptr_t)a[14]) : MOPA_ERR_ARG;
    case 124: return nargs == 12 ? mopa_voxel_hash_build((const int64_t*)(uintptr_t)a[0], (int64_t)a[1], (uint64_t*)(uintptr_t)a[2], (int32_t*)(uintptr_t)a[3], (int64_t)a[4], (int32_t*)(uintptr_t)a[5], (uint64_t*)(uintptr_t)a[6], (int32_t*)(uintptr_t)a[7], (int32_t*)(uintptr_t)a[8], (void*)(uintptr_t)a[9], (size_t)a[10], (void*)(uintptr_t)a[11]) : MOPA_ERR_ARG;
    case 125: return nargs == 12 ? mopa_voxelize((const float*)(uintptr_t)a[0], (int32_t)a[1], (float)slot_f(a[2]), (int32_t)a[3], (const double*)(uintptr_t)a[4], (int32_t)a[5], (int64_t)a[6], (int64_t*)(uintptr_t)a[7], (uint8_t*)(uintptr_t)a[8], (void*)(uintptr_t)a[9], (size_t)a[10], (void*)(uintptr_t)a[11]) : MOPA_ERR_ARG;
    case 126: return nargs == 14 ? mopa_voxelize_f64((const double*)(uintptr_t)a[0], (int32_t)a[1], (const uint8_t*)(uintptr_t)a[2], (const double*)(uintptr_t)a[3], (double)slot_f(a[4]), (int32_t)a[5], (const double*)(uintptr_t)a[6], (int32_t)a[7], (int64_t)a[8], (int64_t*)(uintptr_t)a[9], (uint8_t*)(uintptr_t)a[10], (void*)(uintptr_t)a[11], (size_t)a[12], (void*)(uintptr_t)a[13]) : MOPA_ERR_ARG;
    case 127: return nargs == 10 ? mopa_wce_bwd((const float*)(uintptr_t)a[0], (const int64_t*)(uintptr_t)a[1], (const float*)(uintptr_t)a[2], (int32_t)a[3], (int32_t)a[4], (int64_t)a[5], (const float*)(uintptr_t)a[6], (const float*)(uintptr_t)a[7], (float*)(uintptr_t)a[8], (void*)(uintptr_t)a[9]) : MOPA_ERR_ARG;
    case 128: return nargs == 12 ? mopa_wce_fwd((const float*)(uintptr_t)a[0], (const int64_t*)(uintptr_t)a[1], (const float*)(uintptr_t)a[2], (int32_t)a[3], (int32_t)a[4], (int64_t)a[5], (float*)(uintptr_t)a[6], (float*)(uintptr_t)a[7], (int32_t*)(uintptr_t)a[8], (void*)(uintptr_t)a[9], (size_t)a[10], (void*)(uintptr_t)a[11]) : MOPA_ERR_ARG;
    case 129: return nargs == 10 ? mopa_wino4_bwd_weight((const float*)(uintptr_t)a[0], (const float*)(uintptr_t)a[1], (int32_t)a[2], (int32_t)a[3], (int32_t)a[4], (float*)(uintptr_t)a[5], (int32_t)a[6], (void*)(uintptr_t)a[7], (size_t)a[8], (void*)(uintptr_t)a[9]) : MOPA_ERR_ARG;
    case 130: return nargs == 17 ? mopa_wino4_conv((const float*)(uintptr_t)a[0], (int32_t)a[1], (const float*)(uintptr_t)a[2], (const float*)(uintptr_t)a[3], (float*)(uintptr_t)a[4], (int32_t)a[5], (int32_t)a[6], (int32_t)a[7], (int32_t)a[8], (int32_t)a[9], (int32_t)a[10], (int32_t)a[11], (const float*)(uintptr_t)a[12], (int32_t)a[13], (int32_t)a[14], (float*)(uintptr_t)a[15], (void*)(uintptr_t)a[16]) : MOPA_ERR_ARG;
    case 131: return nargs == 16 ? mopa_wino4_conv9((const float*)(uintptr_t)a[0], (int32_t)a[1], (const float*)(uintptr_t)a[2], (const float*)(uintptr_t)a[3], (float*)(uintptr_t)a[4], (int32_t)a[5], (int32_t)a[6], (int32_t)a[7], (int32_t)a[8], (int32_t)a[9], (int32_t)a[10], (int32_t)a[11], (const float*)(uintptr_t)a[12], (int32_t)a[13], (int32_t)a[14], (void*)(uintptr_t)a[15]) : MOPA_ERR_ARG;
    case 132: return nargs == 8 ? mopa_wino4_dout((const float*)(uintptr_t)a[0], (int32_t)a[1], (int32_t)a[2], (int32_t)a[3], (int32_t)a[4], (int32_t)a[5], (float*)(uintptr_t)a[6], (void*)(uintptr_t)a[7]) : MOPA_ERR_ARG;
    case 133: return nargs == 12 ? mopa_wino4_gemm_output((const float*)(uintptr_t)a[0], (const float*)(uintptr_t)a[1], (const float*)(uintptr_t)a[2], (float*)(uintptr_t)a[3], (int32_t)a[4], (int32_t)a[5], (int32_t)a[6], (int32_t)a[7], (int32_t)a[8], (int32_t)a[9], (int32_t)a[10], (void*)(uintptr_t)a[11]) : MOPA_ERR_ARG;
    case 134: return nargs == 8 ? mopa_wino4_input((const float*)(uintptr_t)a[0], (int32_t)a[1], (int32_t)a[2], (int32_t)a[3], (int32_t)a[4], (int32_t)a[5], (float*)(uintptr_t)a[6], (void*)(uintptr_t)a[7]) : MOPA_ERR_ARG;
    case 135: return nargs == 11 ? mopa_wino4_input_bn((const float*)(uintptr_t)a[0], (int32_t)a[1], (int32_t)a[2], (int32_t)a[3], (int32_t)a[4], (int32_t)a[5], (const float*)(uintptr_t)a[6], (int32_t)a[7], (int32_t)a[8], (float*)(uintptr_t)a[9], (void*)(uintptr_t)a[10]) : MOPA_ERR_ARG;
    case 136: return nargs == 10 ? mopa_wino4_output((const float*)(uintptr_t)a[0], (int32_t)a[1], (int32_t)a[2], (int32_t)a[3], (int32_t)a[4], (const float*)(uintptr_t)a[5], (float*)(uintptr_t)a[6], (int32_t)a[7], (int32_t)a[8], (void*)(uintptr_t)a[9]) : MOPA_ERR_ARG;
    case 137: return nargs == 6 ? mopa_wino4_weight((const float*)(uintptr_t)a[0], (int32_t)a[1], (int32_t)a[2], (int32_t)a[3], (float*)(uintptr_t)a[4], (void*)(uintptr_t)a[5]) : MOPA_ERR_ARG;
    case 138: return nargs == 6 ? mopa_wino4_weight_f((const float*)(uintptr_t)a[0], (int32_t)a[1], (int32_t)a[2], (int32_t)a[3], (float*)(uintptr_t)a[4], (void*)(uintptr_t)a[5]) : MOPA_ERR_ARG;
    case 139: return nargs == 6 ? mopa_wino4_weight_q((const float*)(uintptr_t)a[0], (int32_t)a[1], (int32_t)a[2], (int32_t)a[3], (float*)(uintptr_t)a[4], (void*)(uintptr_t)a[5]) : MOPA_ERR_ARG;
    case 140: return nargs == 6 ? mopa_wino4_weight_t((const float*)(uintptr_t)a[0], (int32_t)a[1], (int32_t)a[2], (int32_t)a[3], (float*)(uintptr_t)a[4], (void*)(uintptr_t)a[5]) : MOPA_ERR_ARG;
    case 141: return nargs == 17 ? mopa_wino4_wgrad_fused((const float*)(uintptr_t)a[0], (int32_t)a[1], (const float*)(uintptr_t)a[2], (int32_t)a[3], (int32_t)a[4], (const float*)(uintptr_t)a[5], (int32_t)a[6], (int32_t)a[7], (int32_t)a[8], (int32_t)a[9], (int32_t)a[10], (int32_t)a[11], (float*)(uintptr_t)a[12], (int32_t)a[13], (void*)(uintptr_t)a[14], (size_t)a[15], (void*)(uintptr_t)a[16]) : MOPA_ERR_ARG;
    case 142: return nargs == 10 ? mopa_wino_bwd_weight((const float*)(uintptr_t)a[0], (const float*)(uintptr_t)a[1], (int32_t)a[2], (int32_t)a[3], (int32_t)a[4], (float*)(uintptr_t)a[5], (int32_t)a[6], (void*)(uintptr_t)a[7], (size_t)a[8], (void*)(uintptr_t)a[9]) : MOPA_ERR_ARG;
    case 143: return nargs == 8 ? mopa_wino_dout((const float*)(uintptr_t)a[0], (int32_t)a[1], (int32_t)a[2], (int32_t)a[3], (int32_t)a[4], (int32_t)a[5], (float*)(uintptr_t)a[6], (void*)(uintptr_t)a[7]) : MOPA_ERR_ARG;
    case 144: return nargs == 8 ? mopa_wino_input((const float*)(uintptr_t)a[0], (int32_t)a[1], (int32_t)a[2], (int32_t)a[3], (int32_t)a[4], (int32_t)a[5], (float*)(uintptr_t)a[6], (void*)(uintptr_t)a[7]) : MOPA_ERR_ARG;
    case 145: return nargs == 10 ? mopa_wino_output((const float*)(uintptr_t)a[0], (int32_t)a[1], (int32_t)a[2], (int32_t)a[3], (int32_t)a[4], (const float*)(uintptr_t)a[5], (float*)(uintptr_t)a[6], (int32_t)a[7], (int32_t)a[8], (void*)(uintptr_t)a[9]) : MOPA_ERR_ARG;
    case 146: return nargs == 6 ? mopa_wino_weight((const float*)(uintptr_t)a[0], (int32_t)a[1], (int32_t)a[2], (int32_t)a[3], (float*)(uintptr_t)a[4], (void*)(uintptr_t)a[5]) : MOPA_ERR_ARG;
    case 147: return nargs == 5 ? mopa_zero_rows((float*)(uintptr_t)a[0], (int32_t)a[1], (int64_t)a[2], (int32_t)a[3], (void*)(uintptr_t)a[4]) : MOPA_ERR_ARG;
    default: return MOPA_ERR_ARG;
  }
}
```

### mopa_amd/csrc/rows.hip

```cpp
#include "common.h"
#include <initializer_list>

static inline int bn_rows_per_block(int64_t num_rows) {
  int64_t r = cdiv64(num_rows, 2048);
  if (r < 32) r = 32;
  if (r > 1024) r = 1024;
  return (int)r;
}
static inline int bn_num_blocks(int64_t num_rows) { return (int)cdiv64(num_rows, bn_rows_per_block(num_rows)); }

#define BN_MAX_GROUPS 3
struct BnGroups {
  int n;
  int row0[BN_MAX_GROUPS], rows[BN_MAX_GROUPS], rpb[BN_MAX_GROUPS], nblk[BN_MAX_GROUPS], poff[BN_MAX_GROUPS];
  int nblk_max, nblk_total;
};
static inline bool bn_make_groups(BnGroups* g, int num_rows, int n_groups, int split1, int split2) {
  if (n_groups < 1 || n_groups > BN_MAX_GROUPS || num_rows <= 0) return false;
  const int b[4] = {0, n_groups > 1 ? split1 : num_rows, n_groups > 2 ? split2 : num_rows, num_rows};
  g->n = n_groups;
  g->nblk_max = g->nblk_total = 0;
  for (int k = 0; k < BN_MAX_GROUPS; ++k) { g->row0[k] = g->rows[k] = g->nblk[k] = g->poff[k] = 0; g->rpb[k] = 1; }
  for (int k = 0; k < n_groups; ++k) {
    const int r0 = b[k], r1 = k == n_groups - 1 ? num_rows : b[k + 1];
// ... 195 lines not shown
  if (y) {
    int maxrows = 0;
    for (int k = 0; k < grp.n; ++k) maxrows = grp.rows[k] > maxrows ? grp.rows[k] : maxrows;
    if (bits)
      k_bn_relu_apply<true><<<dim3(bn_apply_grid(maxrows, C), grp.n), 256, 0, st>>>(x, ldx, y, ldy, grp, C, stats, leak, res, ld_res, act,
                                                                                    bits);
    else
      k_bn_relu_apply<false><<<dim3(bn_apply_grid(maxrows, C), grp.n), 256, 0, st>>>(x, ldx, y, ldy, grp, C, stats, leak, res, ld_res,
                                                                                     act, nullptr);
  }
  MOPA_CHECK_LAUNCH();
  return MOPA_OK;
}
MOPA_API int mopa_bn_act_fwd_groups(const float* x, int32_t ldx, float* y, int32_t ldy, int32_t num_rows, int32_t C,
                                    int32_t n_groups, int32_t split1, int32_t split2,
                                    const float* gamma, const float* beta, float* running_mean, float* running_var,
                                    float momentum, float eps, float leak, int32_t act, const float* res, int32_t ld_res,
                                    int32_t training, float* stats, void* ws, size_t ws_bytes, void* stream) {
  return bn_act_fwd_groups(x, ldx, y, ldy, num_rows, C, n_groups, split1, split2, gamma, beta, running_mean, running_var, momentum, eps,
                           leak, act, res, ld_res, training, stats, nullptr, ws, ws_bytes, stream);
}
MOPA_API int mopa_bn_act_fwd_groups_bits(const float* x, int32_t ldx, float* y, int32_t ldy, int32_t num_rows, int32_t C,
                                         int32_t n_groups, int32_t split1, int32_t split2,
                                         const float* gamma, const float* beta, float* running_mean, float* running_var,
                                         float momentum, float eps, float leak, int32_t act, const float* res, int32_t ld_res,
                                         int32_t training, float* stats, int32_t want_bits, uint32_t* bits, void* ws, size_t ws_bytes,
                                         void* stream) {
  if (want_bits && (!bits || C <= 0 || (C & 31) || leak != 0.f || !res || !y || act != 1 || !training)) return MOPA_ERR_ARG;
  return bn_act_fwd_groups(x, ldx, y, ldy, num_rows, C, n_groups, split1, split2, gamma, beta, running_mean, running_var, momentum, eps,
                           leak, act, res, ld_res, training, stats, want_bits ? bits : nullptr, ws, ws_bytes, stream);
}
MOPA_API int mopa_bn_act_fwd(const float* x, int32_t ldx, float* y, int32_t ldy, int32_t num_rows, int32_t C,
                             const float* gamma, const float* beta, float* running_mean, float* running_var,
                             float momentum, float eps, float leak, int32_t act, const float* res, int32_t ld_res,
                             int32_t training, float* stats, void* ws, size_t ws_bytes, void* stream) {
  return mopa_bn_act_fwd_groups(x, ldx, y, ldy, num_rows, C, 1, 0, 0, gamma, beta, running_mean, running_var, momentum, eps, leak, act,
                                res, ld_res, training, stats, ws, ws_bytes, stream);
}

MOPA_API int mopa_bnrelu_rows_fwd(const float* x, int32_t ldx, float* y, int32_t ldy, int32_t num_rows, int32_t C,
                                  const float* gamma, const float* beta, float* running_mean, float* running_var,
                                  float momentum, float eps, float leak, int32_t training, float* stats, void* ws,
                                  size_t ws_bytes, void* stream) {
  return mopa_bn_act_fwd(x, ldx, y, ldy, num_rows, C, gamma, beta, running_mean, running_var, momentum, eps, leak, 1,
                         nullptr, 0, training, stats, ws, ws_bytes, stream);
}

__device__ __forceinline__ float bn_dz(float g, float xv, float sc, float sh, float leak, int act, bool has_ym, float ym) {
  if (!act) return g;
  const float yv = has_ym ? ym : fmaf(xv, sc, sh);
  return yv > 0.f ? g : g * leak;
}

__device__ __forceinline__ float bn_dz_bit(float g, float leak, int act, bool pos) {
  if (!act) return g;
  return pos ? g : g * leak;
}
__device__ __forceinline__ uint32_t bn_mask_nibble(const uint32_t* __restrict__ bits, int64_t row, int C, int cq) {
  return bits[row * (C >> 5) + (cq >> 3)] >> ((cq & 7) * 4);
}

struct BnRowsMask {
  const float* __restrict__ dy; int ld_dy; const float* __restrict__ ymask; int ld_ym;
  struct Row { float4 g, y; };
  __device__ __forceinline__ void load(int row, int cq, int C, Row& r) const {
    r.g = *reinterpret_cast<const float4*>(dy + (int64_t)row * ld_dy + cq * 4);
    r.y = make_float4(0.f, 0.f, 0.f, 0.f);
    if (ymask) r.y = *reinterpret_cast<const float4*>(ymask + (int64_t)row * ld_ym + cq * 4);
  }
  __device__ __forceinline__ float4 value(int row, int cq, const Row& r) const { return r.g; }
  __device__ __forceinline__ float dz(int j, float g, float xv, float sc, float sh, float leak, int act, const Row& r) const {
    const float ys[4] = {r.y.x, r.y.y, r.y.z, r.y.w};
    return bn_dz(g, xv, sc, sh, leak, act, ymask != nullptr, ys[j]);
  }
};
struct BnRowsBits {
  const float* __restrict__ dy; int ld_dy; const uint32_t* __restrict__ bits;
  struct Row { float4 g; uint32_t m; };
  __device__ __forceinline__ void load(int row, int cq, int C, Row& r) const {
    r.g = *reinterpret_cast<const float4*>(dy + (int64_t)row * ld_dy + cq * 4);
    r.m = bn_mask_nibble(bits, row, C, cq);
  }
  __device__ __forceinline__ float4 value(int row, int cq, const Row& r) const { return r.g; }
  __device__ __forceinline__ float dz(int j, float g, float xv, float sc, float sh, float leak, int act, const Row& r) const {
    return bn_dz_bit(g, leak, act, (r.m >> j) & 1u);
  }
};
struct PoolBwdArgs { const float* dpool; int ld_dpool; const unsigned char* argmax; int H, W, OH, OW; };
struct PoolRow { float4 g[4]; uchar4 w[4]; float4 q; int tap[4]; };
__device__ __forceinline__ void pool_bwd_row_load(const PoolBwdArgs& p, const float* __restrict__ dy, int ld_dy, int C, int row, int cq,
                                                  bool accumulate, PoolRow& o) {
  const int ix = row % p.W, r = row / p.W;
  const int iy = r % p.H, b = r / p.H;
  const int by = iy >> 1, py = iy & 1, bx = ix >> 1, px = ix & 1;
#pragma unroll
  for (int a = 0; a < 2; ++a)
#pragma unroll
    for (int c = 0; c < 2; ++c) {
      const bool ok = a <= py && c <= px && by + a < p.OH && bx + c < p.OW;
      const int64_t w = (int64_t)(b * p.OH + by + (ok ? a : 0)) * p.OW + bx + (ok ? c : 0);
      o.tap[a * 2 + c] = ok ? (a == 0 ? 1 + py : 0) * 3 + (c == 0 ? 1 + px : 0) : 255;
      o.w[a * 2 + c] = *reinterpret_cast<const uchar4*>(p.argmax + w * C + cq * 4);
      o.g[a * 2 + c] = *reinterpret_cast<const float4*>(p.dpool + w * p.ld_dpool + cq * 4);
    }
  o.q = make_float4(0.f, 0.f, 0.f, 0.f);
  if (accumulate) o.q = *reinterpret_cast<const float4*>(dy + (int64_t)row * ld_dy + cq * 4);
}
__device__ __forceinline__ float4 pool_bwd_row_value(const PoolRow& o, bool accumulate) {
  float s[4] = {0.f, 0.f, 0.f, 0.f};
#pragma unroll
  for (int k = 0; k < 4; ++k) {
    s[0] = o.w[k].x == o.tap[k] ? s[0] + o.g[k].x : s[0];
    s[1] = o.w[k].y == o.tap[k] ? s[1] + o.g[k].y : s[1];
// ... 783 lines not shown
```

### mopa_amd/csrc/wino2d.hip

```cpp
#include "common.h"
#include "weight_forms.h"
#include <string.h>
#include <stdio.h>
#include <stdlib.h>

__global__ void k_wino_w(const float* __restrict__ w, int O, int I, int dgrad, float* __restrict__ U) {
  wf_wino2_body(w, O, I, dgrad, U, blockIdx.x * blockDim.x + threadIdx.x, gridDim.x * blockDim.x);
}

__global__ __launch_bounds__(256) void k_wino_in(const float* __restrict__ in, int ld_in, int B, int H, int W, int C, int th, int tw,
                                                  float* __restrict__ V) {
  const int CQ = C >> 2;
  const int64_t T = (int64_t)B * th * tw;
  const int64_t total = T * CQ;
  for (int64_t i = blockIdx.x * (int64_t)blockDim.x + threadIdx.x; i < total; i += (int64_t)gridDim.x * blockDim.x) {
    const int64_t t = i / CQ;
    const int cq = (int)(i - t * CQ);
    const int b = (int)(t / (th * tw));
    const int rt = (int)(t - (int64_t)b * th * tw);
    const int ty = rt / tw, tx = rt - ty * tw;
    float4 d[4][4];
#pragma unroll
    for (int a = 0; a < 4; ++a) {
      const int y = 2 * ty - 1 + a;
// ... 157 lines not shown

__global__ void k_wino4_w(const float* __restrict__ w, int O, int I, int dgrad, float* __restrict__ U, int transpose) {
  wf_wino4_body(w, O, I, dgrad, U, transpose, blockIdx.x * blockDim.x + threadIdx.x, gridDim.x * blockDim.x);
}

template <bool BN>
__global__ __launch_bounds__(256) void k_wino4_in(const float* __restrict__ in, int ld_in, int B, int H, int W, int C, int th, int tw,
                                                   float* __restrict__ V, const float* __restrict__ stats, int imgs_per_group, int c0) {
  const int64_t T = (int64_t)B * th * tw;
  const int64_t total = T * C;
  for (int64_t i = blockIdx.x * (int64_t)blockDim.x + threadIdx.x; i < total; i += (int64_t)gridDim.x * blockDim.x) {
    const int64_t t = i / C;
    const int ch = (int)(i - t * C);
    const int b = (int)(t / (th * tw));
    const int rt = (int)(t - (int64_t)b * th * tw);
    const int ty = rt / tw, tx = rt - ty * tw;
    float sc = 1.f, sh = 0.f;
    const bool bn_ch = BN && ch >= c0;
    if (bn_ch) {
      const float* __restrict__ sg = stats + (int64_t)(b / imgs_per_group) * 4 * (C - c0);
      sc = sg[ch - c0]; sh = sg[C - c0 + ch - c0];
    }
    float m[6][6];
#pragma unroll
    for (int c = 0; c < 6; ++c) {
      const int x = 4 * tx - 1 + c;
      float d[6], tc[6];
#pragma unroll
      for (int a = 0; a < 6; ++a) {
        const int y = 4 * ty - 1 + a;
        const bool inside = (unsigned)y < (unsigned)H && (unsigned)x < (unsigned)W;
        d[a] = inside ? in[((int64_t)(b * H + y) * W + x) * ld_in + ch] : 0.f;
        if (bn_ch && inside) {
          const float o = fmaf(d[a], sc, sh);
          d[a] = o > 0.f ? o : o * 0.f;
        }
      }
      w4_bt(d, tc);
#pragma unroll
      for (int a = 0; a < 6; ++a) m[a][c] = tc[a];
    }
    float* vp = V + t * C + ch;
    const int64_t ps = T * C;
#pragma unroll
    for (int a = 0; a < 6; ++a) {
      float v[6];
      w4_bt(m[a], v);
#pragma unroll
      for (int c = 0; c < 6; ++c) vp[(a * 6 + c) * ps] = v[c];
    }
  }
}

__global__ __launch_bounds__(256) void k_wino4_out(const float* __restrict__ M, int B, int H, int W, int C, int th, int tw,
                                                    const float* __restrict__ bias, float* __restrict__ out, int ld_out, int accumulate) {
  const int64_t T = (int64_t)B * th * tw;
  const int64_t total = T * C;
  for (int64_t i = blockIdx.x * (int64_t)blockDim.x + threadIdx.x; i < total; i += (int64_t)gridDim.x * blockDim.x) {
    const int64_t t = i / C;
    const int ch = (int)(i - t * C);
    const int b = (int)(t / (th * tw));
    const int rt = (int)(t - (int64_t)b * th * tw);
    const int ty = rt / tw, tx = rt - ty * tw;
    const float* mp = M + t * C + ch;
    const int64_t ps = T * C;
    float s[4][6];
#pragma unroll
    for (int c = 0; c < 6; ++c) {
      float m[6], y[4];
#pragma unroll
      for (int a = 0; a < 6; ++a) m[a] = mp[(a * 6 + c) * ps];
      w4_at(m, y);
#pragma unroll
      for (int a = 0; a < 4; ++a) s[a][c] = y[a];
    }
    const float bv = bias ? bias[ch] : 0.f;
#pragma unroll
    for (int a = 0; a < 4; ++a) {
      const int y = 4 * ty + a;
      if (y >= H) continue;
      float o[4];
      w4_at(s[a], o);
#pragma unroll
      for (int c = 0; c < 4; ++c) {
        const int x = 4 * tx + c;
        if (x >= W) continue;
        float* p = out + ((int64_t)(b * H + y) * W + x) * ld_out + ch;
        float v = o[c] + bv;
        if (accumulate) v += *p;
        *p = v;
      }
    }
  }
}

__global__ __launch_bounds__(256) void k_wino4_dout(const float* __restrict__ dy, int ld, int B, int H, int W, int C, int th, int tw,
                                                     float* __restrict__ dM) {
  const int64_t T = (int64_t)B * th * tw;
  const int64_t total = T * C;
  for (int64_t i = blockIdx.x * (int64_t)blockDim.x + threadIdx.x; i < total; i += (int64_t)gridDim.x * blockDim.x) {
    const int64_t t = i / C;
    const int ch = (int)(i - t * C);
    const int b = (int)(t / (th * tw));
    const int rt = (int)(t - (int64_t)b * th * tw);
    const int ty = rt / tw, tx = rt - ty * tw;
    float r[6][4];
#pragma unroll
    for (int c = 0; c < 4; ++c) {
      const int x = 4 * tx + c;
      float d[4], rc[6];
#pragma unroll
      for (int a = 0; a < 4; ++a) {
        const int y = 4 * ty + a;
        d[a] = (y < H && x < W) ? dy[((int64_t)(b * H + y) * W + x) * ld + ch] : 0.f;
      }
      w4_a(d, rc);
#pragma unroll
      for (int a = 0; a < 6; ++a) r[a][c] = rc[a];
    }
    float* mp = dM + t * C + ch;
    const int64_t ps = T * C;
#pragma unroll
    for (int a = 0; a < 6; ++a) {
      float m[6];
      w4_a(r[a], m);
#pragma unroll
      for (int c = 0; c < 6; ++c) mp[(a * 6 + c) * ps] = m[c];
    }
  }
}

MOPA_API int mopa_wino4_weight(const float* weight, int32_t O, int32_t I, int32_t dgrad, float* U, void* stream) {
  if (O <= 0 || I <= 0) return MOPA_ERR_ARG;
  k_wino4_w<<<stream_grid((int64_t)O * I, 256), 256, 0, (hipStream_t)stream>>>(weight, O, I, dgrad, U, 0);
  MOPA_CHECK_LAUNCH();
  return MOPA_OK;
}
MOPA_API int mopa_wino4_input(const float* in, int32_t ld_in, int32_t B, int32_t H, int32_t W, int32_t C, float* V, void* stream) {
  if (B <= 0 || H <= 0 || W <= 0 || C <= 0 || ld_in < C) return MOPA_ERR_ARG;
  const int th = (H + 3) / 4, tw = (W + 3) / 4;
  k_wino4_in<false><<<stream_grid((int64_t)B * th * tw * C, 256), 256, 0, (hipStream_t)stream>>>(in, ld_in, B, H, W, C, th, tw, V, nullptr, 1, 0);
  MOPA_CHECK_LAUNCH();
  return MOPA_OK;
}
MOPA_API int mopa_wino4_input_bn(const float* in, int32_t ld_in, int32_t B, int32_t H, int32_t W, int32_t C, const float* stats,
                                 int32_t n_groups, int32_t bn_c0, float* V, void* stream) {
  if (B <= 0 || H <= 0 || W <= 0 || C <= 0 || ld_in < C || !stats || n_groups < 1 || B % n_groups || bn_c0 < 0 || bn_c0 >= C) return MOPA_ERR_ARG;
  const int th = (H + 3) / 4, tw = (W + 3) / 4;
  k_wino4_in<true><<<stream_grid((int64_t)B * th * tw * C, 256), 256, 0, (hipStream_t)stream>>>(in, ld_in, B, H, W, C, th, tw, V, stats,
                                                                                              B / n_groups, bn_c0);
  MOPA_CHECK_LAUNCH();
  return MOPA_OK;
}
MOPA_API int mopa_wino4_output(const float* M, int32_t B, int32_t H, int32_t W, int32_t C, const float* bias, float* out, int32_t ld_out,
                               int32_t accumulate, void* stream) {
  if (B <= 0 || H <= 0 || W <= 0 || C <= 0 || ld_out < C) return MOPA_ERR_ARG;
  const int th = (H + 3) / 4, tw = (W + 3) / 4;
  k_wino4_out<<<stream_grid((int64_t)B * th * tw * C, 256), 256, 0, (hipStream_t)stream>>>(M, B, H, W, C, th, tw, bias, out, ld_out, accumulate);
  MOPA_CHECK_LAUNCH();
  return MOPA_OK;
}
MOPA_API int mopa_wino4_dout(const float* dy, int32_t ld, int32_t B, int32_t H, int32_t W, int32_t C, float* dM, void* stream) {
  if (B <= 0 || H <= 0 || W <= 0 || C <= 0 || ld < C) return MOPA_ERR_ARG;
  const int th = (H + 3) / 4, tw = (W + 3) / 4;
  k_wino4_dout<<<stream_grid((int64_t)B * th * tw * C, 256), 256, 0, (hipStream_t)stream>>>(dy, ld, B, H, W, C, th, tw, dM);
  MOPA_CHECK_LAUNCH();
  return MOPA_OK;
}

#define WF_MAX 48
struct WeightFormDescs { int64_t src[WF_MAX], dst[WF_MAX]; int32_t O[WF_MAX], I[WF_MAX], KH[WF_MAX], KW[WF_MAX], kind[WF_MAX], arg[WF_MAX]; };
__global__ void k_weight_forms_batched(const WeightFormDescs d) {
  const int e = blockIdx.y;
  const float* src = reinterpret_cast<const float*>(d.src[e]);
  float* dst = reinterpret_cast<float*>(d.dst[e]);
  const int i0 = blockIdx.x * blockDim.x + threadIdx.x, istep = gridDim.x * blockDim.x;
  if (d.kind[e] == 0) wf_relayout_body(src, dst, d.O[e], d.I[e], d.KH[e], d.KW[e], d.arg[e], i0, istep);
  else if (d.kind[e] == 1) wf_wino2_body(src, d.O[e], d.I[e], d.arg[e] & 1, dst, i0, istep);
  else wf_wino4_body(src, d.O[e], d.I[e], d.arg[e] & 1, dst, (d.arg[e] >> 1) & 3, i0, istep);
}
MOPA_API int mopa_conv2d_weight_forms_batched(const int64_t* desc_host, int32_t n, void* stream) {
  if (!desc_host || n <= 0 || n > WF_MAX) return MOPA_ERR_ARG;
  WeightFormDescs d;
  memset(&d, 0, sizeof(d));
  int64_t nmax = 0;
  for (int e = 0; e < n; ++e) {
    const int64_t* r = desc_host + (int64_t)e * 8;
    const int64_t O = r[2], I = r[3], KH = r[4], KW = r[5], kind = r[6], arg = r[7];
    if (!r[0] || !r[1] || O <= 0 || I <= 0 || kind < 0 || kind > 2) return MOPA_ERR_ARG;
    if (kind == 0 && (KH <= 0 || KW <= 0 || arg < 0 || arg > 3 || O * I * KH * KW >= (1ll << 31))) return MOPA_ERR_ARG;
    if (kind != 0 && (KH != 3 || KW != 3 || arg < 0 || arg > 7 || (kind == 1 && (arg & 6))
                      || ((arg & 6) == 4 && (O % 16 || I % 16))
                      || ((arg & 6) == 6 && (((arg & 1) ? O : I) % 16 || ((arg & 1) ? I : O) % 32)))) return MOPA_ERR_ARG;
    d.src[e] = r[0]; d.dst[e] = r[1]; d.O[e] = (int)O; d.I[e] = (int)I; d.KH[e] = (int)KH; d.KW[e] = (int)KW; d.kind[e] = (int)kind; d.arg[e] = (int)arg;
    const int64_t ne = kind == 0 ? O * I * KH * KW : O * I;
    if (ne > nmax) nmax = ne;
  }
  int bx = (int)cdiv64(nmax, 256);
  if (bx > 256) bx = 256;
  k_weight_forms_batched<<<dim3(bx, n), 256, 0, (hipStream_t)stream>>>(d);
  MOPA_CHECK_LAUNCH();
  return MOPA_OK;
}

typedef float f32x4w __attribute__((ext_vector_type(4)));
typedef float f32x2w __attribute__((ext_vector_type(2)));
__constant__ float c_w4_at[6][4] = {{1.f, 0.f, 0.f, 0.f}, {1.f, 1.f, 1.f, 1.f}, {1.f, -1.f, 1.f, -1.f}, {1.f, 2.f, 4.f, 8.f}, {1.f, -2.f, 4.f, -8.f}, {0.f, 0.f, 0.f, 1.f}};
#define W4G_BM 64
#define W4G_BN 32
#define W4G_KB 64
#define W4G_NST 3
// ... 826 lines not shown
```

### mopa_amd/csrc/wino4c9.hip

```cpp
#include "wino4.h"
#include <stdlib.h>
#include <stdio.h>

typedef float f32x16c __attribute__((ext_vector_type(16)));
typedef float f32x4c __attribute__((ext_vector_type(4)));

#define C9_TM 32
#define C9_CN 64
#define C9_KC 16
#define C9_PITCH 34

struct C9Args {
  const float* in; const float* Uq; const float* bias; float* out; const float* stats;
  int ld_in, ld_out, B, H, W, th, tw, T, Cin, Cout, accumulate, imgs_per_group, bn_c0, nco;
  long long* prof;
};

__device__ __forceinline__ void c9_bt(float d0, float d1, float d2, float d3, float d4, float d5, float& t0, float& t1, float& t2, float& t3,
                                      float& t4, float& t5) {
  t0 = fmaf(4.f, d0, fmaf(-5.f, d2, d4));
  const float p = fmaf(-4.f, d2, d4), q = fmaf(-4.f, d1, d3);
  t1 = p + q;
  t2 = p - q;
  const float r = d4 - d2, s = d3 - d1;
  t3 = fmaf(2.f, s, r);
  t4 = fmaf(-2.f, s, r);
  t5 = fmaf(4.f, d1, fmaf(-5.f, d3, d5));
}

template <bool BN>
__global__ __launch_bounds__(512, 2) void k_wino4_conv9(const C9Args a) {
  __shared__ __attribute__((aligned(16))) float c9_lds[36 * C9_KC * C9_PITCH + 36 * 512];
  float* const Vs = c9_lds;
  float* const Ps = c9_lds + 36 * C9_KC * C9_PITCH;
  const int t = threadIdx.x, lane = t & 63, wv = __builtin_amdgcn_readfirstlane(t >> 6);
  const int nco = a.nco;
  const int grp = blockIdx.x / (8 * nco), r8 = blockIdx.x - grp * 8 * nco;
  const int cob = r8 >> 3, tg = grp * 8 + (r8 & 7);
  const int t0 = tg * C9_TM;
  if (t0 >= a.T) return;
  const int co0 = cob * C9_CN;
  const int H = a.H, W = a.W, tw = a.tw, thw = a.th * a.tw;
#ifdef C9_PROFILE
  long long pt[8] = {0, 0, 0, 0, 0, 0, 0, 0}, tprev = __builtin_readcyclecounter();
#define C9_T(K_) { const long long n_ = __builtin_readcyclecounter(); pt[K_] += n_ - tprev; tprev = n_; }
#else
#define C9_T(K_)
#endif

  const int ts = t >> 4, ch = t & 15;
  const int tile = t0 + ts;
  const bool tv = tile < a.T;
  const int tb = tile / thw, rt = tile - tb * thw, ty = rt / tw, tx = rt - ty * tw;
  const int ab = tv ? tb : 0, ay = tv ? ty : 0, ax = tv ? tx : 0;
  const uint32_t ld4 = (uint32_t)a.ld_in * 4u;
  unsigned okm = 0;
  uint32_t cof[6];
#pragma unroll
  for (int i = 0; i < 6; ++i) {
    okm |= (tv && (unsigned)(4 * ay - 1 + i) < (unsigned)H ? 1u : 0u) << i;
    okm |= ((unsigned)(4 * ax - 1 + i) < (unsigned)W ? 1u : 0u) << (8 + i);
    cof[i] = (uint32_t)min(max(4 * ax - 1 + i, 0), W - 1) * ld4 + (uint32_t)ch * 4u;
  }
  const int abH = ab * H, y0 = 4 * ay - 1;
  const bool interior = __all(tv && ty >= 1 && tx >= 1 && 4 * ty + 4 < H && 4 * tx + 4 < W) != 0;
  const char* __restrict__ inb = reinterpret_cast<const char*>(a.in);
  float* __restrict__ vw = Vs + ch * C9_PITCH + ts;
  float sc = 1.f, sh = 0.f;
// ... 80 lines not shown
#define C9_WWAIT(N, X0, X1) asm volatile("s_waitcnt vmcnt(" #N ")" : "+v"(X0), "+v"(X1))
      C9_WLOAD(b0, b1, up);
#pragma unroll
      for (int q = 0; q < 9; ++q) {
        if (q + 1 < 9) {
          const char* __restrict__ un = up + (int64_t)(((q + 1) / 3) * 6 + (q + 1) % 3) * pstride * 4;
          if (q & 1) { C9_WLOAD(b0, b1, un); } else { C9_WLOAD(n0, n1, un); }
        }
        float av[8];
#define C9_OFF(KK) "i"((((q / 3) * 6 + q % 3) * C9_KC + 2 * (KK)) * C9_PITCH * 4)
        asm volatile("ds_read_b32 %0, %8 offset:%9\n\tds_read_b32 %1, %8 offset:%10\n\tds_read_b32 %2, %8 offset:%11\n\tds_read_b32 %3, %8 offset:%12\n\t"
                     "ds_read_b32 %4, %8 offset:%13\n\tds_read_b32 %5, %8 offset:%14\n\tds_read_b32 %6, %8 offset:%15\n\tds_read_b32 %7, %8 offset:%16\n\t"
                     "s_waitcnt lgkmcnt(0)"
                     : "=&v"(av[0]), "=&v"(av[1]), "=&v"(av[2]), "=&v"(av[3]), "=&v"(av[4]), "=&v"(av[5]), "=&v"(av[6]), "=&v"(av[7])
                     : "v"(vr_b), C9_OFF(0), C9_OFF(1), C9_OFF(2), C9_OFF(3), C9_OFF(4), C9_OFF(5), C9_OFF(6), C9_OFF(7));
        if (q & 1) {
          if (q == 7) { C9_WWAIT(2, n0, n1); } else { C9_WWAIT(8, n0, n1); }
#pragma unroll
          for (int kk = 0; kk < 4; ++kk) acc[q] = __builtin_amdgcn_mfma_f32_32x32x2f32(av[kk], n0[kk], acc[q], 0, 0, 0);
#pragma unroll
          for (int kk = 0; kk < 4; ++kk) acc[q] = __builtin_amdgcn_mfma_f32_32x32x2f32(av[4 + kk], n1[kk], acc[q], 0, 0, 0);
        } else {
          if (q == 0) { C9_WWAIT(2, b0, b1); } else if (q == 8) { C9_WWAIT(0, b0, b1); } else { C9_WWAIT(8, b0, b1); }
#pragma unroll
          for (int kk = 0; kk < 4; ++kk) acc[q] = __builtin_amdgcn_mfma_f32_32x32x2f32(av[kk], b0[kk], acc[q], 0, 0, 0);
#pragma unroll
          for (int kk = 0; kk < 4; ++kk) acc[q] = __builtin_amdgcn_mfma_f32_32x32x2f32(av[4 + kk], b1[kk], acc[q], 0, 0, 0);
        }
        if (q < 6) {
#pragma unroll
          for (int n = 6 * q; n < 6 * q + 6; ++n) patch_dma(n, cb);
        }
      }
      if (more) patch_bn(cib + 1);
    }
    C9_T(4)
    __builtin_amdgcn_s_barrier();
    C9_T(5)
  }

  constexpr float AT[4][6] = {{1.f, 1.f, 1.f, 1.f, 1.f, 0.f}, {0.f, 1.f, -1.f, 2.f, -2.f, 0.f}, {0.f, 1.f, 1.f, 4.f, 4.f, 0.f},
                              {0.f, 1.f, -1.f, 8.f, -8.f, 1.f}};
  float ar_[4][3];
#pragma unroll
  for (int i = 0; i < 4; ++i)
#pragma unroll
    for (int k = 0; k < 3; ++k) ar_[i][k] = (g >> 1) ? AT[i][3 + k] : AT[i][k];
  __builtin_amdgcn_s_waitcnt(0x0F70);
  __syncthreads();
  float* __restrict__ tsb = c9_lds;
  const int stl = t0 + (t >> 4), sq = (t & 15) * 4;
  const f32x4c bv = a.bias ? *reinterpret_cast<const f32x4c*>(a.bias + co0 + sq) : (f32x4c){0.f, 0.f, 0.f, 0.f};
  const int sb_ = stl / thw, sr_ = stl - sb_ * thw, sty = sr_ / tw, stx = sr_ - sty * tw;
  float* __restrict__ obase = a.out + ((int64_t)(sb_ * H + 4 * sty) * W + 4 * stx) * a.ld_out + co0 + sq;
  for (int i = 0; i < 4; ++i) {
#pragma unroll
    for (int e = 0; e < 16; ++e) {
      const int til = 8 * (e >> 2) + 4 * lk + (e & 3);
#pragma unroll
      for (int b = 0; b < 3; ++b) {
        const float tv_ = fmaf(ar_[i][0], acc[b][e], fmaf(ar_[i][1], acc[3 + b][e], ar_[i][2] * acc[6 + b][e]));
        tsb[(((g >> 1) * 6 + pb0 + b) * C9_TM + til) * C9_CN + coh * 32 + l32] = tv_;
      }
    }
    __syncthreads();
    {
      f32x4c tt[6];
#pragma unroll
      for (int b = 0; b < 6; ++b) {
        const f32x4c u0 = *reinterpret_cast<const f32x4c*>(tsb + (b * C9_TM + (t >> 4)) * C9_CN + sq);
        const f32x4c u1 = *reinterpret_cast<const f32x4c*>(tsb + ((6 + b) * C9_TM + (t >> 4)) * C9_CN + sq);
        tt[b] = u0 + u1;
      }
      if (stl < a.T && 4 * sty + i < H) {
        float* __restrict__ o = obase + (int64_t)i * W * a.ld_out;
#pragma unroll
        for (int j = 0; j < 4; ++j) {
          f32x4c y = bv;
#pragma unroll
          for (int b = 0; b < 6; ++b)
            if (AT[j][b] != 0.f) y += AT[j][b] * tt[b];
          if (4 * stx + j < W) {
            f32x4c* __restrict__ op = reinterpret_cast<f32x4c*>(o + (int64_t)j * a.ld_out);
            *op = a.accumulate ? *op + y : y;
          }
        }
      }
    }
    __syncthreads();
  }
#ifdef C9_PROFILE
  C9_T(6)
  if (blockIdx.x == 100 && t == 0)
    for (int k = 0; k < 8; ++k) a.prof[k] = pt[k];
#endif
}


MOPA_API int mopa_wino4_conv9(const float* in, int32_t ld_in, const float* Uq, const float* bias, float* out, int32_t ld_out, int32_t B, int32_t H,
                              int32_t W, int32_t Cin, int32_t Cout, int32_t accumulate, const float* stats, int32_t n_groups, int32_t bn_c0,
                              void* stream) {
  if (B <= 0 || H <= 0 || W <= 0 || Cin <= 0 || Cout <= 0 || Cin % C9_KC || Cout % C9_CN || ld_in < Cin || ld_out < Cout ||
      ((uintptr_t)Uq & 15) || ((uintptr_t)out & 15) || (ld_out & 3) || ((uintptr_t)bias & 15) || !in || !Uq || !out)
    return MOPA_ERR_ARG;
  if (stats && (n_groups < 1 || B % n_groups || bn_c0 < 0 || bn_c0 >= Cin)) return MOPA_ERR_ARG;
  if ((int64_t)B * H * W * ld_in >= (1ll << 30) || (int64_t)B * H * W * ld_out >= (1ll << 31)) return MOPA_ERR_ARG;
  C9Args a;
  a.in = in; a.Uq = Uq; a.bias = bias; a.out = out; a.stats = stats;
  a.ld_in = ld_in; a.ld_out = ld_out; a.B = B; a.H = H; a.W = W; a.th = (H + 3) / 4; a.tw = (W + 3) / 4;
  const int64_t T = (int64_t)B * a.th * a.tw;
  if (T >= (1 << 30)) return MOPA_ERR_ARG;
  a.T = (int)T; a.Cin = Cin; a.Cout = Cout; a.accumulate = accumulate;
  a.imgs_per_group = stats ? B / n_groups : 1;
  a.bn_c0 = stats ? bn_c0 : 0;
  a.nco = Cout / C9_CN;
  a.prof = nullptr;
  const int64_t ntg = (cdiv64(T, C9_TM) + 7) / 8 * 8;
  const int64_t nblk = ntg * a.nco;
  if (nblk >= (1ll << 31)) return MOPA_ERR_ARG;
#ifdef C9_PROFILE
  static long long* prof = nullptr;
  if (!prof) hipMallocManaged(&prof, 128);
  a.prof = prof;
#endif
  if (stats) k_wino4_conv9<true><<<(unsigned)nblk, 512, 0, (hipStream_t)stream>>>(a);
  else k_wino4_conv9<false><<<(unsigned)nblk, 512, 0, (hipStream_t)stream>>>(a);
  MOPA_CHECK_LAUNCH();
#ifdef C9_PROFILE
  hipStreamSynchronize((hipStream_t)stream);
  {
    const double n_ = Cin / C9_KC;
    printf("[c9 profile] block 100 wave 0, cycles per step: loop head %.0f | patch loads + apply %.0f | transform + lds stores %.0f | barrier %.0f | "
           "multiply %.0f | barrier %.0f | output transform + exchange + store (per item) %.0f   (steps per item %.0f)\n",
           prof[0] / n_, prof[1] / n_, prof[2] / n_, prof[3] / n_, prof[4] / n_, prof[5] / n_, (double)prof[6], n_);
  }
#endif
  return MOPA_OK;
}
```

### mopa_amd/dense2d.py

```python
from __future__ import annotations

import ctypes
import os
from typing import NamedTuple

import numpy as np
import torch

from . import _lib, syncbn
from ._lib import GradSink, call, host_i32, ptr, query, stream, workspace
from .sparse3d import View

BN_EPS = 1e-5
BN_MOMENTUM = 0.1
DEBUG = None
LAYERS = [("layer1", 64, 3, 1), ("layer2", 128, 4, 2), ("layer3", 256, 6, 2), ("layer4", 512, 3, 2)]


class Img(View):

    __slots__ = ("B", "H", "W", "partial", "pool")

    def __init__(self, t, B, H, W, col=0, C=None):
        super().__init__(t, col, C)
# ... 136 lines not shown
    transposed = int(transposed)

    def build():
        R, C = (O if dgrad else I), (I if dgrad else O)
        u = torch.empty((F + 2) ** 2, (C if transposed == 1 else R), (R if transposed == 1 else C), dtype=torch.float32, device=w.device)
        name = "mopa_wino_weight" if F == 2 else ("mopa_wino4_weight", "mopa_wino4_weight_t", "mopa_wino4_weight_f", "mopa_wino4_weight_q")[transposed]
        call(name, ptr(w), O, I, int(dgrad), ptr(u), stream())
        u._mopa_wino_layout = (F, transposed)
        return u
    assert not (transposed and F != 4)
    return _cached_weight_form(w, ("wino", F, int(dgrad), transposed), build,
                               (O, I, 3, 3, 1 if F == 2 else 2, int(dgrad) | (transposed << 1)))


WINO4_FUSED_MIN_BLOCKS = int(os.environ.get("MOPA_WINO4_FUSED_MIN_BLOCKS", "700")) if os.environ.get("MOPA_WINO4_FUSED", "1") != "0" else 1 << 62


def wino4_fused(cin, cout, B, H, W):
    T = B * ((H + 3) // 4) * ((W + 3) // 4)
    blocks = ((T + 63) // 64) * (cout // 32)
    return cin % 64 == 0 and cout % 32 == 0 and (blocks >= WINO4_FUSED_MIN_BLOCKS or (cin == 64 and 2 * blocks >= WINO4_FUSED_MIN_BLOCKS))


WINO4_DIRECT = os.environ.get("MOPA_WINO4_DIRECT", "1") != "0"
WINO4_DIRECT_MIN_TILES = int(os.environ.get("MOPA_WINO4_DIRECT_MIN_TILES", "4096"))
WINO4_DIRECT_MAX_CIN = 128
WINO4_DIRECT_ROLES = tuple(r for r in os.environ.get("MOPA_WINO4_DIRECT_ROLES", "fwd_eval,dgrad").split(",") if r)


CUS = 256


def wino4_direct(cin, cout, B, H, W, role="fwd"):
    T = B * ((H + 3) // 4) * ((W + 3) // 4)
    if not (WINO4_DIRECT and role in WINO4_DIRECT_ROLES and cin % 64 == 0 and cout % 64 == 0 and cin <= WINO4_DIRECT_MAX_CIN and cout <= 128):
        return False
    if cout <= 64:
        return T >= WINO4_DIRECT_MIN_TILES
    if wino4_conv9(cin, cout, role) and T >= WINO4_DIRECT_MIN_TILES * 5 // 8:
        items = (T + 31) // 32 * (cout // 64)
        if items >= 0.7 * ((items + CUS - 1) // CUS * CUS):
            return True
    return T >= 2 * WINO4_DIRECT_MIN_TILES


WINO4_CONV9 = os.environ.get("MOPA_WINO4_CONV9", "1") != "0"


def wino4_conv9(cin, cout, role):
    return WINO4_CONV9 and role != "fwd" and cin % 16 == 0 and cout % 64 == 0


F4_FORMS = ("F4", "F4 fused", "F4 one", "F4 one9")


def wino4_layout(cin, cout, B, H, W, role="fwd", want_v=False):
    if wino4_direct(cin, cout, B, H, W, role):
        return 3 if wino4_conv9(cin, cout, role) and not want_v else 2
    return int(wino4_fused(cin, cout, B, H, W))


def wino_tile(cin, cout, k, s, p, B, H, W, role="fwd"):
    if not (WINOGRAD and k == 3 and s == 1 and p == 1 and cin % 16 == 0 and cout % 64 == 0):
        return 0
    if (role in F4_ROLES and min(H, W) >= 8 and B * H * W < F4_MAX_PIXELS
            and (role != "fwd" or B * H * W >= F4_FWD_MIN_PIXELS)):
        return 4
    return 2 if max(cin, cout) >= 128 and B * H * W < 200000 else 0


F4_MAX_PIXELS = int(os.environ.get("MOPA_WINOGRAD_F4_PIXELS", "3000000"))
WINOGRAD = os.environ.get("MOPA_WINOGRAD", "1") != "0"
WINOGRAD_WGRAD = os.environ.get("MOPA_CONV2D_MFMA", "1") != "0" and os.environ.get("MOPA_WINOGRAD_WGRAD", "1") != "0"
F4_ROLES = tuple(r for r in os.environ.get("MOPA_WINOGRAD_F4_ROLES", "fwd,dgrad,wgrad").split(",") if r) \
    if os.environ.get("MOPA_WINOGRAD_F4", "1") != "0" else ()
F4_FWD_MIN_PIXELS = 4096


def _bn_args(bn):
    return (ptr(bn[0]), bn[1], bn[2]) if bn is not None else (None, 1, 0)


def wino_conv(x_p, ld_in, B, H, W, cin, cout, U, bias, out_p, ld_out, accumulate=False, F=2, bn_in=None, role="fwd", want_v=True):
    T, NP = B * ((H + F - 1) // F) * ((W + F - 1) // F), (F + 2) ** 2
    sfx = "" if F == 2 else "4"
    form = wino4_layout(cin, cout, B, H, W, role, want_v) if F == 4 else 0
    if getattr(U, "_mopa_wino_layout", (F, form)) != (F, form) or (form and tuple(U.shape) != ((36, cout, cin) if form == 1 else (36, cin, cout))):
        raise RuntimeError(f"wino_conv: this shape, role and want_v take the weight form wino_weight_cached(..., F={F}, transposed={form})")
    if bn_in is not None and F != 4:
        raise RuntimeError("wino_conv: a deferred BatchNorm needs the F(4x4) input transform")
    V = torch.empty(NP * T * cin, dtype=torch.float32, device=U.device) if form < 2 or want_v else None
    if form == 3:
        call("mopa_wino4_conv9", x_p, ld_in, ptr(U), ptr(bias), out_p, ld_out, B, H, W, cin, cout, int(accumulate), *_bn_args(bn_in), stream())
        return None
    if form == 2:
        call("mopa_wino4_conv", x_p, ld_in, ptr(U), ptr(bias), out_p, ld_out, B, H, W, cin, cout, int(accumulate), *_bn_args(bn_in), ptr(V), stream())
        return V
    if bn_in is not None:
        call("mopa_wino4_input_bn", x_p, ld_in, B, H, W, cin, *_bn_args(bn_in), ptr(V), stream())
    else:
        call(f"mopa_wino{sfx}_input", x_p, ld_in, B, H, W, cin, ptr(V), stream())
    if form == 1:
        call("mopa_wino4_gemm_output", ptr(V), ptr(U), ptr(bias), out_p, ld_out, B, H, W, cin, cout, int(accumulate), stream())
        return V
    M = torch.empty(NP * T * cout, dtype=torch.float32, device=U.device)
    g1 = _geom(B=1, IH=1, IW=T, OHl=1, OWl=T, OHa=1, OWa=T, TH=1, TW=1, KWF=1, Cin=cin, Cout=cout, ld_in=cin, ld_out=cout)
    igemm_batched(ptr(V), ptr(U), ptr(M), g1, NP, T * cin, cin * cout, T * cout)
    call(f"mopa_wino{sfx}_output", ptr(M), B, H, W, cout, ptr(bias), out_p, ld_out, int(accumulate), stream())
    return V


def wino_wgrad_eligible(cin, cout, k, s, p, B, H, W):
    F = wino_tile(cin, cout, k, s, p, B, H, W, "wgrad")
    return (F != 0 and cin % 64 == 0 and cout % 64 == 0 and min(cin, cout) >= (64 if F == 4 else 128)
            and WINOGRAD_WGRAD)


WINO4_WGRAD_FUSED = os.environ.get("MOPA_WINO4_WGRAD_FUSED", "1") != "0"
WINO4_WGRAD_FUSED_MIN_TILES = int(os.environ.get("MOPA_WINO4_WGRAD_FUSED_MIN_TILES", "8192"))


def wino4_wgrad_fused(cin, cout, B, H, W):
    T = B * ((H + 3) // 4) * ((W + 3) // 4)
    return (WINO4_WGRAD_FUSED and cin % 32 == 0 and cout % 64 == 0 and cin <= 128 and cout <= 128
            and T >= (WINO4_WGRAD_FUSED_MIN_TILES if cout > 64 else WINO4_WGRAD_FUSED_MIN_TILES * 5 // 8)
            and bool(query("mopa_wino4_wgrad_fused_ok", B, H, W, cin, cout)))


def wino_wgrad(x: Img, dout: Img, cin, cout, dw, V=None, accumulate=False, F=2, fused=None):
    dev = dw.device
    B, H, W = x.B, x.H, x.W
    if F == 4 and V is None and (wino4_wgrad_fused(cin, cout, B, H, W) if fused is None else fused):
        ws = workspace.get(query("mopa_wino4_wgrad_fused_workspace_bytes", B, H, W, cin, cout), dev)
        call("mopa_wino4_wgrad_fused", x.p, x.ld, *_bn_args(getattr(x, "bn", None)), dout.p, dout.ld, B, H, W, cin, cout, ptr(dw),
             int(accumulate) | 2, ptr(ws), ws.numel(), stream())
        return
    T, NP = B * ((H + F - 1) // F) * ((W + F - 1) // F), (F + 2) ** 2
    sfx = "" if F == 2 else "4"
    dM = torch.empty(NP * T * cout, dtype=torch.float32, device=dev)
    if V is None:
        V = torch.empty(NP * T * cin, dtype=torch.float32, device=dev)
        if hasattr(x, "bn"):
            call("mopa_wino4_input_bn", x.p, x.ld, B, H, W, cin, *_bn_args(x.bn), ptr(V), stream())
        else:
            call(f"mopa_wino{sfx}_input", x.p, x.ld, B, H, W, cin, ptr(V), stream())
    call(f"mopa_wino{sfx}_dout", dout.p, dout.ld, B, H, W, cout, ptr(dM), stream())
    ws = workspace.get(query(f"mopa_wino{sfx}_wgrad_workspace_bytes", T, cin, cout), dev)
    call(f"mopa_wino{sfx}_bwd_weight", ptr(V), ptr(dM), T, cin, cout, ptr(dw), int(accumulate) | 2, ptr(ws), ws.numel(), stream())


_wgrad_streams = {}
WGRAD_STREAM = os.environ.get("MOPA_WGRAD_STREAM", "1") != "0"


def _shared_device_group():
    import torch.distributed as dist
    if not (dist.is_available() and dist.is_initialized()):
        return False
    if dist.get_world_size() == 1 and os.environ.get("MOPA_FORCE_COLLECTIVES") != "1":
        return False
    return dist.get_backend() != "nccl"
# ... 11 lines not shown

_on_events = {}
_REC_EVENTS = (0, 0)


class _on:

    def __init__(self, side, *tensors):
        self.side, self.tensors = side, tensors

    def __enter__(self):
        if self.side is None:
            return
        if _lib.RECORDER is not None:
            _lib.RECORDER.event_record(_REC_EVENTS[0], stream())
            _lib.RECORDER.stream_wait(self.side.cuda_stream, _REC_EVENTS[0])
        ev = _on_events.get(self.side)
        if ev is None:
            ev = _on_events[self.side] = torch.cuda.Event()
        ev.record(torch.cuda.current_stream())
        self.side.wait_event(ev)
        for t in self.tensors:
            if torch.is_tensor(t):
                t.record_stream(self.side)
        self.ctx = torch.cuda.stream(self.side)
        self.ctx.__enter__()

    def __exit__(self, *exc):
        if self.side is not None:
            self.ctx.__exit__(*exc)
        return False


def join_wgrad_stream(dev):
    ws = wgrad_stream(dev)
    if ws is not None:
        if _lib.RECORDER is not None:
            _lib.RECORDER.event_record(_REC_EVENTS[1], ws.cuda_stream)
            _lib.RECORDER.stream_wait(stream(), _REC_EVENTS[1])
        torch.cuda.current_stream().wait_stream(ws)


class ConvPlan(NamedTuple):
    fwd: str
    fwd_layout: int
    fwd_role: str
    keeps_v: bool
    takes_lazy: bool
    wgrad: str
    wgrad_F: int
    dgrad: str
    dgrad_layout: int


def conv_plan(cin, cout, k, s, p, B, H, W, training) -> ConvPlan:
    a = (cin, cout, k, s, p, B, H, W)
    Ff, Fw, Fd = wino_tile(*a, "fwd"), wino_tile(*a, "wgrad"), wino_tile(cout, cin, k, s, p, B, H, W, "dgrad")
    wg = wino_wgrad_eligible(*a)
    one = wg and Fw == 4 and wino4_wgrad_fused(cin, cout, B, H, W)
    keeps_v = bool(training and wg and Ff != 0 and Ff == Fw and not one)
    fwd_role = "fwd" if keeps_v or (training and Ff != 4) else "fwd_eval"
    fwd_layout = wino4_layout(cin, cout, B, H, W, fwd_role) if Ff == 4 else 0
    dgrad_layout = wino4_layout(cout, cin, B, H, W, "dgrad") if Fd == 4 else 0
    return ConvPlan(fwd=F4_FORMS[fwd_layout] if Ff == 4 else ("direct", "F2")[Ff // 2], fwd_layout=fwd_layout, fwd_role=fwd_role, keeps_v=keeps_v,
                    takes_lazy=bool(Ff == 4 and (not training or (Fw == 4 and wg))),
                    wgrad="direct" if not wg else "F2" if Fw == 2 else "F4 one" if one else "F4", wgrad_F=Fw if wg else 0,
                    dgrad=F4_FORMS[dgrad_layout] if Fd == 4 else ("direct", "F2")[Fd // 2], dgrad_layout=dgrad_layout)


def forward_role(cin, cout, k, s, p, B, H, W, keep_v):
    plan = conv_plan(cin, cout, k, s, p, B, H, W, keep_v)
    return plan.keeps_v and plan.fwd in F4_FORMS, plan.fwd_role


class ConvOp:

    def __init__(self, weight, bias, k, s, p):
        self.w, self.b, self.k, self.s, self.p = weight, bias, k, s, p
        self.O, self.I = weight.shape[0], weight.shape[1]

    def out_hw(self, H, W):
        return (H + 2 * self.p - self.k) // self.s + 1, (W + 2 * self.p - self.k) // self.s + 1

    def _fwd_geom(self, x: Img, out: Img):
        return _geom(B=x.B, IH=x.H, IW=x.W, OHl=out.H, OWl=out.W, OHa=out.H, OWa=out.W, IS=self.s, IY0=-self.p,
                     IX0=-self.p, TH=self.k, TW=self.k, KWF=self.k, Cin=self.I, Cout=self.O, ld_in=x.ld, ld_out=out.ld)

    def takes_lazy(self, B, H, W, training):
        return conv_plan(self.I, self.O, self.k, self.s, self.p, B, H, W, training).takes_lazy

    def forward(self, x: Img, out: Img, keep_v: bool = False):
        plan = conv_plan(self.I, self.O, self.k, self.s, self.p, x.B, x.H, x.W, keep_v)
        lazy = getattr(x, "bn", None)
        if lazy is not None and not plan.takes_lazy:
            raise RuntimeError("ConvOp.forward: this layer cannot consume a deferred BatchNorm (ask takes_lazy first)")
        if plan.fwd != "direct":
            F = int(plan.fwd[1])
            V = wino_conv(x.p, x.ld, x.B, x.H, x.W, self.I, self.O, wino_weight_cached(self.w, False, F, plan.fwd_layout), self.b, out.p,
                          out.ld, F=F, bn_in=lazy, role=plan.fwd_role, want_v=plan.keeps_v)
            return V if plan.keeps_v else None
        wl = relayout_cached(self.w, (self.k, self.k, self.I, self.O), self.O, self.I, self.k, self.k, 0)
        igemm(x.p, wl, self.b, out.p, self._fwd_geom(x, out))

    def backward(self, x: Img, dout: Img, dx: Img | None, dw: torch.Tensor, db, acc_dx: bool, acc_params: bool = False, V=None,
                 wgrad_side: bool = False, db_partial=None):
        dev = self.w.device
        k, s, p = self.k, self.s, self.p
        plan = conv_plan(self.I, self.O, k, s, p, x.B, x.H, x.W, True)
        if hasattr(x, "bn") and V is None and plan.wgrad_F != 4:
            raise RuntimeError("ConvOp.backward: the input was a deferred BatchNorm and this layer's weight gradient cannot apply it")
        ws = wgrad_stream(dev) if wgrad_side else None
        with _on(ws, dout.t, db_partial):
            if plan.wgrad_F:
                wino_wgrad(x, dout, self.I, self.O, dw, V, accumulate=acc_params, F=plan.wgrad_F, fused=plan.wgrad == "F4 one")
            else:
                wgrad(x.p, dout.p, ptr(dw), self._fwd_geom(x, dout), dev, accumulate=acc_params, oihw=True)
            if db is not None:
                colsum(dout, db, accumulate=acc_params, partial=db_partial)
        if dx is None:
            return
        if plan.dgrad != "direct":
            F = int(plan.dgrad[1])
            wino_conv(dout.p, dout.ld, x.B, x.H, x.W, self.O, self.I, wino_weight_cached(self.w, True, F, plan.dgrad_layout), None, dx.p,
                      dx.ld, acc_dx, F=F, role="dgrad", want_v=False)
            return
        wt = relayout_cached(self.w, (k, k, self.O, self.I), self.O, self.I, k, k, 1)
        if s == 1:
            g = _geom(B=x.B, IH=dout.H, IW=dout.W, OHl=x.H, OWl=x.W, OHa=x.H, OWa=x.W, IY0=p, IX0=p, IDY=-1, IDX=-1,
                      TH=k, TW=k, KWF=k, Cin=self.O, Cout=self.I, ld_in=dout.ld, ld_out=dx.ld)
            igemm(dout.p, wt, None, dx.p, g, acc_dx)
            return
        assert s == 2
        self.dgrad_s2(x, dout, dx, wt, acc_dx)

    def dgrad_s2_geoms(self, x: Img, dout: Img, dx: Img):
        k, p = self.k, self.p
        geoms = []
        for ph in range(2):
            for pw in range(2):
                khs = [kh for kh in range(k) if (ph + p - kh) % 2 == 0]
                kws = [kw for kw in range(k) if (pw + p - kw) % 2 == 0]
                ohl, owl = (x.H - ph + 1) // 2, (x.W - pw + 1) // 2
                if not khs or not kws or ohl <= 0 or owl <= 0:
                    continue
                geoms.append(_geom(B=x.B, IH=dout.H, IW=dout.W, OHl=ohl, OWl=owl, OHa=x.H, OWa=x.W, OS=2, OOY=ph, OOX=pw,
                                   IY0=(ph + p - khs[0]) // 2, IX0=(pw + p - kws[0]) // 2, IDY=-1, IDX=-1, TH=len(khs),
                                   TW=len(kws), KH0=khs[0], KW0=kws[0], KS=2, KWF=k, Cin=self.O, Cout=self.I, ld_in=dout.ld,
                                   ld_out=dx.ld))
        return geoms

    def dgrad_s2(self, x: Img, dout: Img, dx: Img, wt, acc_dx: bool):
        geoms = self.dgrad_s2_geoms(x, dout, dx)
        if len(geoms) == 4 and conv_classes(dout, dx):
            igemm_classes(dout.p, wt, None, dx.p, geoms, acc_dx)
            return
        if not acc_dx:
            call("mopa_zero_rows", dx.p, dx.ld, dx.rows, dx.C, stream())
        for g in geoms:
            igemm(dout.p, wt, None, dx.p, g, True)


class ConvTOp:

    def __init__(self, weight, bias):
        self.w, self.b = weight, bias
        self.I, self.O = weight.shape[0], weight.shape[1]

    def _geom(self, x: Img, out: Img, ky, kx):
        return _geom(B=x.B, IH=x.H, IW=x.W, OHl=x.H, OWl=x.W, OHa=out.H, OWa=out.W, OS=2, OOY=ky, OOX=kx, TH=1, TW=1,
                     KH0=ky, KW0=kx, KWF=2, Cin=self.I, Cout=self.O, ld_in=x.ld, ld_out=out.ld)

    def forward(self, x: Img, out: Img):
        wl = relayout_cached(self.w, (2, 2, self.I, self.O), self.O, self.I, 2, 2, 2)
        geoms = [self._geom(x, out, ky, kx) for ky in range(2) for kx in range(2)]
        if conv_classes(x, out):
            igemm_classes(x.p, wl, self.b, out.p, geoms)
            return
# ... 91 lines not shown
    call("mopa_bn_act_bwd_groups_fused", dy.p, dy.ld, x.p, x.ld, dx.p, dx.ld, x.rows, x.C, G, n, 2 * n, ptr(stats), 0.0, int(act),
         int(bits is not None), ptr(bits), *_pl(dres), int(acc_dres), int(training), ptr(dgamma), ptr(dbeta), int(acc_params), 0,
         ptr(partial), *_bn_tail("mopa_bn_act_bwd_groups_fused_workspace_bytes", x))
    return partial


def bn_bwd(dy: View, x: View, dx: View, stats, act, ymask, dres, acc_dres, training, dgamma, dbeta, acc_dx=False,
           acc_params=False, gathered=None):
    if gathered is not None:
        return syncbn.bwd(dy, x, dx, stats, 0.0, act, ymask, dres, acc_dres, dgamma, dbeta, acc_params, acc_dx, gathered)
    call("mopa_bn_act_bwd", dy.p, dy.ld, x.p, x.ld, dx.p, dx.ld, x.rows, x.C, ptr(stats), 0.0, int(act), *_pl(ymask), *_pl(dres),
         int(acc_dres), int(training), ptr(dgamma), ptr(dbeta), int(acc_params), int(acc_dx), *_bn_tail("mopa_bnrelu_rows_bwd_workspace_bytes", x))


def bn_bwd_sums(dy: View, x: Img, stats, act, dgamma, dbeta, G, acc_params=False, pool=None):
    n, coef = x.rows // G, torch.empty(G, 2, x.C, dtype=torch.float32, device=x.t.device)
    head = (dy.p, dy.ld, x.p, x.ld, x.rows, x.C, G, n, 2 * n) if pool is None else \
        (pool[0].p, pool[0].ld, ptr(pool[1]), x.B, x.H, x.W, dy.p, dy.ld, int(pool[2]), x.p, x.ld, x.C, G)
    call("mopa_bn_bwd_sums_groups" + ("" if pool is None else "_pool"), *head, ptr(stats), 0.0, int(act), *((None, 0) if pool is None else ()),
         ptr(dgamma), ptr(dbeta), int(acc_params), ptr(coef), *_bn_tail("mopa_bnrelu_rows_workspace_bytes", x))
    return coef


class BnPlan(NamedTuple):
    fwd: str
    bwd: str
    bits: bool
    colsum: bool
    pool_inside: bool
    stem_wgrad: str


def bn_plan(C, G, training, keep_tape, act, res, deferred, sync, biased=False, stem=False, pool_reader=False, grid=(0, 0, 0),
            want_dimg=False, bits=None) -> BnPlan:
    synced = bool(training and sync and not deferred)
    second = lambda part: part in STEM_BWD2 and STEM_BN_FUSED_BWD and grid[0] * grid[1] * grid[2] >= STEM_BWD2_MIN_PIXELS
    if bits is None:
        bits = bool(BN_MASK_BITS and not deferred and keep_tape and training and res and act == 1 and C % 32 == 0 and not sync)
    fwd = ("stats" if deferred else "groups_bits" if bits else "groups" if G > 1 and not (training and sync) else "sync" if synced else "single")
    sums = bool(STEM_BN_FUSED_BWD and stem and C == 64 and not want_dimg and not res and act == 1 and not synced)
    pool_inside = bool(sums and pool_reader and deferred and second("pool"))
    fusable = not synced and (not res or bits)
    colsum = bool(not sums and fusable and biased and BN_COLSUM_FUSED)
    bwd = (("sums_pool" if pool_inside else "sums") if sums else "sync" if synced else "fused" if fusable and (bits or colsum)
           else "groups" if G > 1 else "single")
    return BnPlan(fwd, bwd, bool(bits), colsum, pool_inside, "plain" if not sums else "strip" if second("wgrad") else "im2col_bn")


StemGrad = NamedTuple("StemGrad", [("dy", Img), ("x", Img), ("stats", torch.Tensor), ("coef", torch.Tensor)])


class BnOp:

    def __init__(self, P, name, act=1, res=None, G=1, biased=False, stem_grid=None):
        self.P, self.name, self.act, self.res, self.G, self.biased, self.stem_grid = P, name, act, res, G, biased, stem_grid
        self.x = self.y = self.stats = self.gathered = self.bits = None

    def plan(self, training, want_dimg=False, C=None, keep_tape=True, deferred=False) -> BnPlan:
        ran, stem = self.x is not None, self.stem_grid is not None
        return bn_plan(self.x.C if ran else C, self.G, training, keep_tape, self.act, self.res is not None, hasattr(self.y, "bn") if ran else deferred,
                       self.gathered is not None if ran else syncbn.active(), self.biased, stem, stem, self.stem_grid or (0, 0, 0), want_dimg,
                       self.bits is not None if ran else None)

    def forward(self, x: Img, out, training, keep_tape=True, defer=False):
        G, P, name, res = self.G, self.P, self.name, self.res
        plan = self.plan(training, C=x.C, keep_tape=keep_tape, deferred=defer)
        assert plan.fwd != "stats" or (self.act == 1 and res is None and out is None)
        stats = torch.empty(G, 4, x.C, dtype=torch.float32, device=x.t.device)
        y = None if plan.fwd == "stats" else out if out is not None else new_img(x.B, x.H, x.W, x.C, x.t.device)
        self.bits = torch.empty(x.rows, x.C // 32, dtype=torch.int32, device=x.t.device) if plan.bits else None
        if plan.fwd in ("single", "sync"):
            got = [bn_fwd(_group(x, g, G), _group(y, g, G), P, name, self.act, _group(res, g, G), training, stats[g]) for g in range(G)]
            self.gathered = got if plan.fwd == "sync" else None
        else:
            bn_fwd_groups(x, y, P, name, self.act, res, training, stats, G, self.bits)
        self.x, self.stats, self.y = x, stats, LazyImg(x, stats, G) if y is None else y
        return self.y

    def backward(self, dy: Img, dres, acc_dres, training, dgamma, dbeta, acc_params, want_dimg):
        x, stats, G, act = self.x, self.stats, self.G, self.act
        plan = self.plan(training, want_dimg)
        pool = getattr(dy, "pool", None)
        assert (pool is not None) == plan.pool_inside
        if plan.stem_wgrad != "plain":
            return StemGrad(dy, x, stats, bn_bwd_sums(dy, x, stats, act, dgamma, dbeta, G, acc_params, pool))
        dx = new_img(x.B, x.H, x.W, x.C, x.t.device)
        ymask = self.y if self.res is not None else None
        if plan.bwd == "fused":
            dx.partial = bn_bwd_fused(dy, x, dx, stats, act, self.bits, dres, acc_dres, training, dgamma, dbeta, G, acc_params, plan.colsum)
        elif plan.bwd == "groups":
            bn_bwd_groups(dy, x, dx, stats, act, ymask, dres, acc_dres, training, dgamma, dbeta, G, acc_params)
        else:
            for g in range(G):
                bn_bwd(_group(dy, g, G), _group(x, g, G), _group(dx, g, G), stats[g], act, _group(ymask, g, G), _group(dres, g, G), acc_dres,
                       training, dgamma, dbeta, acc_params=acc_params or g > 0, gathered=None if self.gathered is None else self.gathered[g])
        return dx


def _group(v: Img, g, G):
    if G == 1 or v is None:
        return v
    n = v.rows // G
    return Img(v.t[g * n:(g + 1) * n], v.B // G, v.H, v.W, v.col, v.C)


class _NoTape:

    def append(self, rec):
        pass
# ... 32 lines not shown
        out = out if out is not None else new_img(x.B, 2 * x.H, 2 * x.W, op.O, dev)
        op.forward(x, out)
        tape.append(("convT", name, op, x, out))
        return out

    def dropout(x, site, out=None):
        y = out if out is not None else new_img(x.B, x.H, x.W, x.C, dev)
        p = drop_p if training else 0.0
        for g in range(G):
            dropout_rows(_group(x, g, G), _group(y, g, G), p, seeds[g], None if seed_t is None else seed_t[g:], site)
        tape.append(("dropout", site, x, y, p))
        return y

    x4 = torch.empty(B, Hp + 6, Wp + 8, 4, dtype=torch.float32, device=dev)
    call("mopa_img_to_nhwc4", ptr(imgc), B, H, W, Hp, Wp, ptr(x4), stream())
    w1 = torch.empty(7, 2, 16, 64, dtype=torch.float32, device=dev)
    call("mopa_conv2d_stem_relayout", ptr(P[pre + "conv1.weight"]), ptr(w1), 64, 0, 0, stream())
    J = {}
    J[0] = torch.empty(B * Hp * Wp, 128, dtype=torch.float32, device=dev)
    lazy_stem = (DEFER_BN and DEFER_UP_BN and DEFER_STEM_BN and not (training and syncbn.active())
                 and takes_lazy(pre + "dec_conv_stage1", B, Hp, Wp))
    c1 = Img(J[0], B, Hp, Wp, 0, 64) if lazy_stem else new_img(B, Hp, Wp, 64, dev)
    stem_g = _geom(B=B, IH=Hp + 6, IW=Wp + 8, OHl=Hp, OWl=Wp, OHa=Hp, OWa=Wp, IDX=4, TH=7, TW=2, KWF=2, Cin=16,
                   Cout=64, ld_in=4, ld_out=c1.ld)
    stem_forward(ptr(x4), w1, c1.p, stem_g)
    bn1 = BnOp(P, pre + "bn1", G=G, stem_grid=(B, Hp, Wp))
    tape.append(("stem", x4, c1, stem_g, bn1))
    H2, W2 = Hp // 2, Wp // 2
    x = new_img(B, H2, W2, 64, dev)
    amax = torch.empty(B * H2 * W2 * 64, dtype=torch.uint8, device=dev)
    skip0 = bn(pre + "bn1", c1, out=None if lazy_stem else Img(J[0], B, Hp, Wp, 0, 64), defer=lazy_stem, op=bn1)
    if lazy_stem:
        call("mopa_maxpool3x3s2_fwd_bn", c1.p, c1.ld, B, Hp, Wp, 64, ptr(skip0.bn[0]), G, x.p, x.ld, ptr(amax), stream())
    else:
        call("mopa_maxpool3x3s2_fwd", skip0.p, skip0.ld, B, Hp, Wp, 64, x.p, x.ld, ptr(amax), stream())
    tape.append(("maxpool", skip0, x, amax, bn1))
    for li, (lname, c, nblocks, stride) in enumerate(LAYERS):
        for b in range(nblocks):
            q = f"{pre}{lname}.{b}."
            s = stride if b == 0 else 1
            has_ds = (q + "downsample.0.weight") in P
            z1 = conv(q + "conv1", x, 3, s, 1)
            defer = (DEFER_BN and not (training and syncbn.active())
                     and takes_lazy(q + "conv2", z1.B, z1.H, z1.W))
            y1 = bn(q + "bn1", z1, defer=defer)
            z = conv(q + "conv2", y1, 3, 1, 1)
            idt = bn(q + "downsample.1", conv(q + "downsample.0", x, 1, s, 0), act=0) if has_ds else x
            last = b == nblocks - 1
            out = None
            if last and lname in ("layer1", "layer2"):
                lvl = li + 1
                J[lvl] = torch.empty(z.rows, 2 * c, dtype=torch.float32, device=dev)
                out = Img(J[lvl], z.B, z.H, z.W, 0, c)
            x = bn(q + "bn2", z, act=1, res=idt, out=out)
        if lname == "layer3":
            J[3] = torch.empty(x.rows, 2 * c, dtype=torch.float32, device=dev)
            x = dropout(x, 0, out=Img(J[3], x.B, x.H, x.W, 0, c))
        if lname == "layer4":
            x = dropout(x, 1)
    for stage, lvl in (("5", 3), ("4", 2), ("3", 1), ("2", 0)):
        tname = f"{pre}dec_t_conv_stage{stage}."
        cj = J[lvl].shape[1] // 2
        cname = pre + "dec_conv_stage1" if lvl == 0 else f"{pre}dec_conv_stage{int(stage) - 1}.0"
        lazy_up = (DEFER_BN and DEFER_UP_BN and not (training and syncbn.active())
                   and takes_lazy(cname, x.B, 2 * x.H, 2 * x.W))
        if lazy_up:
            right = Img(J[lvl], x.B, 2 * x.H, 2 * x.W, cj, cj)
            up_raw = convT(tname + "0", x, out=right)
            ylazy = bn(tname + "1", up_raw, defer=True, biased=True)
            if lvl == 0 and lazy_stem:
                st2 = torch.empty(G, 4, 2 * cj, dtype=torch.float32, device=dev)
                for half, src in enumerate((skip0.bn[0], ylazy.bn[0])):
                    call("mopa_copy_rows", ptr(src), cj, ptr(st2, half * cj), 2 * cj, G * 4, cj, stream())
                joined = LazyImg(Img(J[lvl], up_raw.B, up_raw.H, up_raw.W, 0, 2 * cj), st2, G)
            else:
                joined = LazyImg(Img(J[lvl], up_raw.B, up_raw.H, up_raw.W, 0, 2 * cj), ylazy.bn[0], G, c0=cj)
        else:
            up_raw = convT(tname + "0", x)
            bn(tname + "1", up_raw, out=Img(J[lvl], up_raw.B, up_raw.H, up_raw.W, cj, cj), biased=True)
            joined = Img(J[lvl], up_raw.B, up_raw.H, up_raw.W, 0, 2 * cj)
        tape.append(("join", lvl, cj, lazy_up, lvl == 0 and lazy_stem))
        if lvl == 0:
            x = conv(pre + "dec_conv_stage1", joined, 3, 1, 1, bias=True)
        else:
            x = bn(cname[:-1] + "1", conv(cname, joined, 3, 1, 1, bias=True), biased=True)
    for i in range(0, len(nbt), 64):
        tab = np.zeros(64, np.int64)
        tab[:len(nbt[i:i + 64])] = [t.data_ptr() for t in nbt[i:i + 64]]
        call("mopa_add_i64_many", tab.ctypes.data, len(nbt[i:i + 64]), G, stream())
    return x, tape, J


def dropout_rows(x: View, y: View, p, seed, seed_t, site):
    if seed_t is not None:
        call("mopa_dropout_rows_dseed", x.p, x.ld, y.p, y.ld, x.rows, x.C, float(p), ptr(seed_t), site, stream())
    else:
        call("mopa_dropout_rows", x.p, x.ld, y.p, y.ld, x.rows, x.C, float(p), seed * 2 + site, stream())


def _backbone_backward(P, sink, tape, J, feat, dfeat, training, drop_seed, seed_t, want_dimg, H, W, groups=1):
    dev = feat.t.device
    G = groups
    seeds = tuple(drop_seed) if isinstance(drop_seed, (tuple, list)) else (drop_seed,) * G
    pre = "net_2d."
    B, Hp, Wp = feat.B, feat.H, feat.W
    gmap = {}
    dimg = None

    def key(v):
        return (v.t.data_ptr(), v.col, v.C) + ((1,) if hasattr(v, "bn") else ())

    def like(v: Img, zero=False):
        return new_img(v.B, v.H, v.W, v.C, dev, zero=zero)

    def grad_of(v):
        k = key(v)
        acc = k in gmap
        gmap[k] = gmap[k] if acc else like(v)
        return gmap[k], acc

    gmap[key(feat)] = dfeat
    for rec in reversed(tape):
        kind = rec[0]
        if kind == "bn":
            op = rec[1]
            dy = gmap.pop(key(op.y))
            dres, acc_dres = grad_of(op.res) if op.res is not None else (None, False)
            (dg, db), pacc = sink.take(op.name + ".weight", op.name + ".bias")
            gmap[key(op.x)] = op.backward(dy, dres, acc_dres, training, dg, db, pacc, want_dimg)
        elif kind == "conv":
            _, name, op, x, out, V = rec
            dout = gmap.pop(key(out))
            dx, acc = grad_of(x)
            pg, pacc = sink.take(*([name + ".weight"] + ([name + ".bias"] if op.b is not None else [])))
            op.backward(x, dout, dx, pg[0], pg[1] if op.b is not None else None, acc, acc_params=pacc, V=V, wgrad_side=True,
                        db_partial=getattr(dout, "partial", None))
        elif kind == "convT":
            _, name, op, x, out = rec
            dout = gmap.pop(key(out))
            dx = like(x)
            gmap[key(x)] = dx
            (dw, db), pacc = sink.take(name + ".weight", name + ".bias")
            op.backward(x, dout, dx, dw, db, acc_params=pacc, wgrad_side=True, db_partial=getattr(dout, "partial", None))
        elif kind == "join":
            _, lvl, cj, lazy_up, lazy_left = rec
            lz = (1,) if lazy_up else ()
            full = gmap.pop((J[lvl].data_ptr(), 0, 2 * cj) + lz)
            if DEBUG is not None:
                DEBUG[f"dJ{lvl}"] = full.t.clone()
            gmap[(J[lvl].data_ptr(), 0, cj) + ((1,) if lazy_left else ())] = Img(full.t, full.B, full.H, full.W, 0, cj)
            gmap[(J[lvl].data_ptr(), cj, cj) + lz] = Img(full.t, full.B, full.H, full.W, cj, cj)
        elif kind == "dropout":
            _, site, x, y, p = rec
            dy = gmap.pop(key(y))
            dx = like(x)
            gmap[key(x)] = dx
            for g in range(G):
                dropout_rows(_group(dy, g, G), _group(dx, g, G), p, seeds[g], None if seed_t is None else seed_t[g:], site)
        elif kind == "maxpool":
            _, x, y, amax, bn1 = rec
            dy = gmap.pop(key(y))
            dx, acc = grad_of(x)
            if bn1.plan(training, want_dimg).pool_inside:
                dx.pool = (dy, amax, acc)
            else:
                call("mopa_maxpool3x3s2_bwd", dy.p, dy.ld, ptr(amax), x.B, x.H, x.W, x.C, dx.p, dx.ld, int(acc), stream())
        elif kind == "stem":
            _, x4, c1, g, bn1 = rec
            dout = gmap.pop(key(c1))
            wg = bn1.plan(training, want_dimg).stem_wgrad
            (dw,), pacc = sink.take(pre + "conv1.weight")
            with _on(wgrad_stream(dev), *((dout.t,) if wg == "plain" else (dout.dy.t, dout.coef))):
                dwl = None if wg == "strip" else torch.empty(7, 2, 16, 64, dtype=torch.float32, device=dev)
                if wg == "plain":
                    if g[24] != dout.ld:
                        g = (ctypes.c_int32 * 25)(*g[:24], dout.ld)
                    wgrad(ptr(x4), dout.p, ptr(dwl), g, dev)
                else:
                    ws = workspace.get(query("mopa_conv2d_wgrad_workspace_bytes", ctypes.addressof(g)), dev)
                    call("mopa_stem_bwd_weight_bn" + ("2" if wg == "strip" else ""), ptr(x4), dout.dy.p, dout.dy.ld, dout.x.p, dout.x.ld,
                         ptr(dout.stats), ptr(dout.coef), G, int(training), ptr(dwl if dwl is not None else dw), ctypes.addressof(g),
                         (int(pacc) | 2) if wg == "strip" else 0, ptr(ws), ws.numel(), stream())
                if dwl is not None:
                    call("mopa_conv2d_stem_relayout", ptr(dwl), ptr(dw), 64, 1, int(pacc), stream())
            if want_dimg:
                dimg = torch.empty(B, 3, H, W, dtype=torch.float32, device=dev)
                call("mopa_stem_dgrad_image", dout.p, dout.ld, B, Hp, Wp, H, W, ptr(P[pre + "conv1.weight"]), ptr(dimg), stream())
    join_wgrad_stream(dev)
    return dimg


GRAPH_2D = os.environ.get("MOPA_GRAPH_2D", "0") == "1"
NATIVE_2D = os.environ.get("MOPA_NATIVE_2D", "1") != "0"
GRAPH_2D_MAX_KEYS = 4
GRAPH_STATS = {"recorded": 0, "forward_replays": 0, "backward_replays": 0, "eager_busy": 0, "eager_backward": 0, "dropped": 0}


class _Token:
    __slots__ = ("__weakref__",)


class Graph2D:

    def __init__(self, B, H, W, dev, groups=1):
        self.B, self.H, self.W, self.dev, self.groups = B, H, W, dev, groups
        self.calls = 0
        self.eager_backward_seen = False
        self.fwd = self.bwd = None
        self.failed = False
        self.pending = None
        self.generation = 0

    def busy(self):
        return self.pending is not None and self.pending() is not None

    def _record(self, fn, pool):
        global _CAPTURE, _REC_EVENTS
        g = torch.cuda.CUDAGraph()
        main = stream()
        _CAPTURE = main
        rec = None
        if NATIVE_2D and not GRAPH_2D:
            if getattr(self, "events", None) is None:
                self.events = (torch.cuda.Event(), torch.cuda.Event())
                for e in self.events:
                    e.record()
            rec = _lib.CommandList(self.side.cuda_stream)
            _REC_EVENTS = tuple(e.cuda_event for e in self.events)
        try:
            if rec is None:
                with torch.cuda.graph(g, pool=pool, stream=self.side, capture_error_mode="thread_local"):
                    out = fn()
            else:
                cur = torch.cuda.current_stream()
                self.side.wait_stream(cur)
                with torch.cuda.stream(self.side):
                    g.capture_begin(pool=pool, capture_error_mode="thread_local")
                    _lib.RECORDER = rec
                    try:
                        out = fn()
# ... 233 lines not shown
```

Before: 422.9.

## Fuse residual-branch gradient into Winograd dgrad output epilogue

In ResNet basic blocks with an identity shortcut, the bn2 backward no longer writes the residual gradient to a separate buffer. Instead the masked, activation-gated upstream gradient is folded into the epilogue of the following block's conv1 backward-data Winograd output (both the separate output transform and the one9 fused kernel). This removes one full-size write plus a later read/accumulate pass of the residual gradient. The cost is extra reads of the bit mask and dy inside the epilogue. It also adds bookkeeping in the backward walk so each deferred residual share is consumed by the matching convolution, gated by a tile-count threshold for the one9 form.

```diff
diff --git a/include/mopa_hip.h b/include/mopa_hip.h
--- a/include/mopa_hip.h
+++ b/include/mopa_hip.h
@@ -116,6 +116,7 @@
 int mopa_wino4_input(const float* in, int32_t ld_in, int32_t B, int32_t H, int32_t W, int32_t C, float* V, void* stream);
 int mopa_wino4_input_bn(const float* in, int32_t ld_in, int32_t B, int32_t H, int32_t W, int32_t C, const float* stats, int32_t n_groups, int32_t bn_c0, float* V, void* stream);
 int mopa_wino4_output(const float* M, int32_t B, int32_t H, int32_t W, int32_t C, const float* bias, float* out, int32_t ld_out, int32_t accumulate, void* stream);
+int mopa_wino4_output_res(const float* M, int32_t B, int32_t H, int32_t W, int32_t C, const float* bias, float* out, int32_t ld_out, const float* res_dy, int32_t ld_res, const uint32_t* bits, int32_t C_total, float leak, int32_t act, void* stream);
 int mopa_wino4_dout(const float* dy, int32_t ld, int32_t B, int32_t H, int32_t W, int32_t C, float* dM, void* stream);
 int mopa_conv2d_weight_forms_batched(const int64_t* desc_host, int32_t n, void* stream);
 int mopa_wino4_weight_t(const float* weight, int32_t O, int32_t I, int32_t dgrad, float* Ut, void* stream);
@@ -126,6 +127,7 @@
 int mopa_wino4_conv(const float* in, int32_t ld_in, const float* Uf, const float* bias, float* out, int32_t ld_out, int32_t B, int32_t H, int32_t W, int32_t Cin, int32_t Cout, int32_t accumulate, const float* stats, int32_t n_groups, int32_t bn_c0, float* V, void* stream);
 
 int mopa_wino4_conv9(const float* in, int32_t ld_in, const float* Uq, const float* bias, float* out, int32_t ld_out, int32_t B, int32_t H, int32_t W, int32_t Cin, int32_t Cout, int32_t accumulate, const float* stats, int32_t n_groups, int32_t bn_c0, void* stream);
+int mopa_wino4_conv9_res(const float* in, int32_t ld_in, const float* Uq, const float* bias, float* out, int32_t ld_out, int32_t B, int32_t H, int32_t W, int32_t Cin, int32_t Cout, const float* res_dy, int32_t ld_res, const uint32_t* bits, int32_t C_total, float leak, int32_t act, const float* stats, int32_t n_groups, int32_t bn_c0, void* stream);
 
 int mopa_wino4_wgrad_fused_ok(int32_t B, int32_t H, int32_t W, int32_t Cin, int32_t Cout);
 size_t mopa_wino4_wgrad_fused_workspace_bytes(int32_t B, int32_t H, int32_t W, int32_t Cin, int32_t Cout);
diff --git a/mopa_amd/_abi.py b/mopa_amd/_abi.py
--- a/mopa_amd/_abi.py
+++ b/mopa_amd/_abi.py
@@ -101,6 +101,7 @@
     'mopa_wino4_input': ('i', 'piiiiipp'),
     'mopa_wino4_input_bn': ('i', 'piiiiipiipp'),
     'mopa_wino4_output': ('i', 'piiiippiip'),
+    'mopa_wino4_output_res': ('i', 'piiiippipipifip'),
     'mopa_wino4_dout': ('i', 'piiiiipp'),
     'mopa_conv2d_weight_forms_batched': ('i', 'pip'),
     'mopa_wino4_weight_t': ('i', 'piiipp'),
@@ -110,6 +111,7 @@
     'mopa_wino4_conv_tiles32': ('i', 'i'),
     'mopa_wino4_conv': ('i', 'pipppiiiiiiipiipp'),
     'mopa_wino4_conv9': ('i', 'pipppiiiiiiipiip'),
+    'mopa_wino4_conv9_res': ('i', 'pipppiiiiiipipifipiip'),
     'mopa_wino4_wgrad_fused_ok': ('i', 'iiiii'),
     'mopa_wino4_wgrad_fused_workspace_bytes': ('z', 'iiiii'),
     'mopa_wino4_wgrad_fused': ('i', 'pipiipiiiiiipipzp'),
diff --git a/mopa_amd/csrc/common.h b/mopa_amd/csrc/common.h
--- a/mopa_amd/csrc/common.h
+++ b/mopa_amd/csrc/common.h
@@ -54,6 +54,15 @@
 
 #define WAVE 64
 
+__device__ __forceinline__ float bn_dz_bit(float g, float leak, int act, bool pos) {
+  if (!act) return g;
+  return pos ? g : g * leak;
+}
+__device__ __forceinline__ uint32_t bn_mask_nibble(const uint32_t* __restrict__ bits, int64_t row, int C, int cq) {
+  return bits[row * (C >> 5) + (cq >> 3)] >> ((cq & 7) * 4);
+}
+struct ResShare { const float* dy; const uint32_t* bits; int ld, C, act; };
+
 __device__ __forceinline__ float wave_sum(float v) {
 #pragma unroll
   for (int o = 32; o > 0; o >>= 1) v += __shfl_xor(v, o, 64);
diff --git a/mopa_amd/csrc/exec_table.inc b/mopa_amd/csrc/exec_table.inc
--- a/mopa_amd/csrc/exec_table.inc
+++ b/mopa_amd/csrc/exec_table.inc
@@ -131,11 +131,13 @@
   "mopa_wino4_bwd_weight",
   "mopa_wino4_conv",
   "mopa_wino4_conv9",
+  "mopa_wino4_conv9_res",
   "mopa_wino4_dout",
   "mopa_wino4_gemm_output",
   "mopa_wino4_input",
   "mopa_wino4_input_bn",
   "mopa_wino4_output",
+  "mopa_wino4_output_res",
   "mopa_wino4_weight",
   "mopa_wino4_weight_f",
   "mopa_wino4_weight_q",
@@ -148,7 +150,7 @@
   "mopa_wino_weight",
   "mopa_zero_rows",
 };
-static const int EXEC_N = 148;
+static const int EXEC_N = 150;
 static int exec_dispatch(int id, const int64_t* a, int nargs) {
   switch (id) {
     case 0: return nargs == 6 ? mopa_a2d2prep_map((const double*)(uintptr_t)a[0], (int32_t)a[1], (int32_t)a[2], (int16_t*)(uintptr_t)a[3], (uint16_t*)(uintptr_t)a[4], (void*)(uintptr_t)a[5]) : MOPA_ERR_ARG;
@@ -283,22 +285,24 @@
     case 129: return nargs == 10 ? mopa_wino4_bwd_weight((const float*)(uintptr_t)a[0], (const float*)(uintptr_t)a[1], (int32_t)a[2], (int32_t)a[3], (int32_t)a[4], (float*)(uintptr_t)a[5], (int32_t)a[6], (void*)(uintptr_t)a[7], (size_t)a[8], (void*)(uintptr_t)a[9]) : MOPA_ERR_ARG;
     case 130: return nargs == 17 ? mopa_wino4_conv((const float*)(uintptr_t)a[0], (int32_t)a[1], (const float*)(uintptr_t)a[2], (const float*)(uintptr_t)a[3], (float*)(uintptr_t)a[4], (int32_t)a[5], (int32_t)a[6], (int32_t)a[7], (int32_t)a[8], (int32_t)a[9], (int32_t)a[10], (int32_t)a[11], (const float*)(uintptr_t)a[12], (int32_t)a[13], (int32_t)a[14], (float*)(uintptr_t)a[15], (void*)(uintptr_t)a[16]) : MOPA_ERR_ARG;
     case 131: return nargs == 16 ? mopa_wino4_conv9((const float*)(uintptr_t)a[0], (int32_t)a[1], (const float*)(uintptr_t)a[2], (const float*)(uintptr_t)a[3], (float*)(uintptr_t)a[4], (int32_t)a[5], (int32_t)a[6], (int32_t)a[7], (int32_t)a[8], (int32_t)a[9], (int32_t)a[10], (int32_t)a[11], (const float*)(uintptr_t)a[12], (int32_t)a[13], (int32_t)a[14], (void*)(uintptr_t)a[15]) : MOPA_ERR_ARG;
-    case 132: return nargs == 8 ? mopa_wino4_dout((const float*)(uintptr_t)a[0], (int32_t)a[1], (int32_t)a[2], (int32_t)a[3], (int32_t)a[4], (int32_t)a[5], (float*)(uintptr_t)a[6], (void*)(uintptr_t)a[7]) : MOPA_ERR_ARG;
-    case 133: return nargs == 12 ? mopa_wino4_gemm_output((const float*)(uintptr_t)a[0], (const float*)(uintptr_t)a[1], (const float*)(uintptr_t)a[2], (float*)(uintptr_t)a[3], (int32_t)a[4], (int32_t)a[5], (int32_t)a[6], (int32_t)a[7], (int32_t)a[8], (int32_t)a[9], (int32_t)a[10], (void*)(uintptr_t)a[11]) : MOPA_ERR_ARG;
-    case 134: return nargs == 8 ? mopa_wino4_input((const float*)(uintptr_t)a[0], (int32_t)a[1], (int32_t)a[2], (int32_t)a[3], (int32_t)a[4], (int32_t)a[5], (float*)(uintptr_t)a[6], (void*)(uintptr_t)a[7]) : MOPA_ERR_ARG;
-    case 135: return nargs == 11 ? mopa_wino4_input_bn((const float*)(uintptr_t)a[0], (int32_t)a[1], (int32_t)a[2], (int32_t)a[3], (int32_t)a[4], (int32_t)a[5], (const float*)(uintptr_t)a[6], (int32_t)a[7], (int32_t)a[8], (float*)(uintptr_t)a[9], (void*)(uintptr_t)a[10]) : MOPA_ERR_ARG;
-    case 136: return nargs == 10 ? mopa_wino4_output((const float*)(uintptr_t)a[0], (int32_t)a[1], (int32_t)a[2], (int32_t)a[3], (int32_t)a[4], (const float*)(uintptr_t)a[5], (float*)(uintptr_t)a[6], (int32_t)a[7], (int32_t)a[8], (void*)(uintptr_t)a[9]) : MOPA_ERR_ARG;
-    case 137: return nargs == 6 ? mopa_wino4_weight((const float*)(uintptr_t)a[0], (int32_t)a[1], (int32_t)a[2], (int32_t)a[3], (float*)(uintptr_t)a[4], (void*)(uintptr_t)a[5]) : MOPA_ERR_ARG;
-    case 138: return nargs == 6 ? mopa_wino4_weight_f((const float*)(uintptr_t)a[0], (int32_t)a[1], (int32_t)a[2], (int32_t)a[3], (float*)(uintptr_t)a[4], (void*)(uintptr_t)a[5]) : MOPA_ERR_ARG;
-    case 139: return nargs == 6 ? mopa_wino4_weight_q((const float*)(uintptr_t)a[0], (int32_t)a[1], (int32_t)a[2], (int32_t)a[3], (float*)(uintptr_t)a[4], (void*)(uintptr_t)a[5]) : MOPA_ERR_ARG;
-    case 140: return nargs == 6 ? mopa_wino4_weight_t((const float*)(uintptr_t)a[0], (int32_t)a[1], (int32_t)a[2], (int32_t)a[3], (float*)(uintptr_t)a[4], (void*)(uintptr_t)a[5]) : MOPA_ERR_ARG;
-    case 141: return nargs == 17 ? mopa_wino4_wgrad_fused((const float*)(uintptr_t)a[0], (int32_t)a[1], (const float*)(uintptr_t)a[2], (int32_t)a[3], (int32_t)a[4], (const float*)(uintptr_t)a[5], (int32_t)a[6], (int32_t)a[7], (int32_t)a[8], (int32_t)a[9], (int32_t)a[10], (int32_t)a[11], (float*)(uintptr_t)a[12], (int32_t)a[13], (void*)(uintptr_t)a[14], (size_t)a[15], (void*)(uintptr_t)a[16]) : MOPA_ERR_ARG;
-    case 142: return nargs == 10 ? mopa_wino_bwd_weight((const float*)(uintptr_t)a[0], (const float*)(uintptr_t)a[1], (int32_t)a[2], (int32_t)a[3], (int32_t)a[4], (float*)(uintptr_t)a[5], (int32_t)a[6], (void*)(uintptr_t)a[7], (size_t)a[8], (void*)(uintptr_t)a[9]) : MOPA_ERR_ARG;
-    case 143: return nargs == 8 ? mopa_wino_dout((const float*)(uintptr_t)a[0], (int32_t)a[1], (int32_t)a[2], (int32_t)a[3], (int32_t)a[4], (int32_t)a[5], (float*)(uintptr_t)a[6], (void*)(uintptr_t)a[7]) : MOPA_ERR_ARG;
-    case 144: return nargs == 8 ? mopa_wino_input((const float*)(uintptr_t)a[0], (int32_t)a[1], (int32_t)a[2], (int32_t)a[3], (int32_t)a[4], (int32_t)a[5], (float*)(uintptr_t)a[6], (void*)(uintptr_t)a[7]) : MOPA_ERR_ARG;
-    case 145: return nargs == 10 ? mopa_wino_output((const float*)(uintptr_t)a[0], (int32_t)a[1], (int32_t)a[2], (int32_t)a[3], (int32_t)a[4], (const float*)(uintptr_t)a[5], (float*)(uintptr_t)a[6], (int32_t)a[7], (int32_t)a[8], (void*)(uintptr_t)a[9]) : MOPA_ERR_ARG;
-    case 146: return nargs == 6 ? mopa_wino_weight((const float*)(uintptr_t)a[0], (int32_t)a[1], (int32_t)a[2], (int32_t)a[3], (float*)(uintptr_t)a[4], (void*)(uintptr_t)a[5]) : MOPA_ERR_ARG;
-    case 147: return nargs == 5 ? mopa_zero_rows((float*)(uintptr_t)a[0], (int32_t)a[1], (int64_t)a[2], (int32_t)a[3], (void*)(uintptr_t)a[4]) : MOPA_ERR_ARG;
+    case 132: return nargs == 21 ? mopa_wino4_conv9_res((const float*)(uintptr_t)a[0], (int32_t)a[1], (const float*)(uintptr_t)a[2], (const float*)(uintptr_t)a[3], (float*)(uintptr_t)a[4], (int32_t)a[5], (int32_t)a[6], (int32_t)a[7], (int32_t)a[8], (int32_t)a[9], (int32_t)a[10], (const float*)(uintptr_t)a[11], (int32_t)a[12], (const uint32_t*)(uintptr_t)a[13], (int32_t)a[14], (float)slot_f(a[15]), (int32_t)a[16], (const float*)(uintptr_t)a[17], (int32_t)a[18], (int32_t)a[19], (void*)(uintptr_t)a[20]) : MOPA_ERR_ARG;
+    case 133: return nargs == 8 ? mopa_wino4_dout((const float*)(uintptr_t)a[0], (int32_t)a[1], (int32_t)a[2], (int32_t)a[3], (int32_t)a[4], (int32_t)a[5], (float*)(uintptr_t)a[6], (void*)(uintptr_t)a[7]) : MOPA_ERR_ARG;
+    case 134: return nargs == 12 ? mopa_wino4_gemm_output((const float*)(uintptr_t)a[0], (const float*)(uintptr_t)a[1], (const float*)(uintptr_t)a[2], (float*)(uintptr_t)a[3], (int32_t)a[4], (int32_t)a[5], (int32_t)a[6], (int32_t)a[7], (int32_t)a[8], (int32_t)a[9], (int32_t)a[10], (void*)(uintptr_t)a[11]) : MOPA_ERR_ARG;
+    case 135: return nargs == 8 ? mopa_wino4_input((const float*)(uintptr_t)a[0], (int32_t)a[1], (int32_t)a[2], (int32_t)a[3], (int32_t)a[4], (int32_t)a[5], (float*)(uintptr_t)a[6], (void*)(uintptr_t)a[7]) : MOPA_ERR_ARG;
+    case 136: return nargs == 11 ? mopa_wino4_input_bn((const float*)(uintptr_t)a[0], (int32_t)a[1], (int32_t)a[2], (int32_t)a[3], (int32_t)a[4], (int32_t)a[5], (const float*)(uintptr_t)a[6], (int32_t)a[7], (int32_t)a[8], (float*)(uintptr_t)a[9], (void*)(uintptr_t)a[10]) : MOPA_ERR_ARG;
+    case 137: return nargs == 10 ? mopa_wino4_output((const float*)(uintptr_t)a[0], (int32_t)a[1], (int32_t)a[2], (int32_t)a[3], (int32_t)a[4], (const float*)(uintptr_t)a[5], (float*)(uintptr_t)a[6], (int32_t)a[7], (int32_t)a[8], (void*)(uintptr_t)a[9]) : MOPA_ERR_ARG;
+    case 138: return nargs == 15 ? mopa_wino4_output_res((const float*)(uintptr_t)a[0], (int32_t)a[1], (int32_t)a[2], (int32_t)a[3], (int32_t)a[4], (const float*)(uintptr_t)a[5], (float*)(uintptr_t)a[6], (int32_t)a[7], (const float*)(uintptr_t)a[8], (int32_t)a[9], (const uint32_t*)(uintptr_t)a[10], (int32_t)a[11], (float)slot_f(a[12]), (int32_t)a[13], (void*)(uintptr_t)a[14]) : MOPA_ERR_ARG;
+    case 139: return nargs == 6 ? mopa_wino4_weight((const float*)(uintptr_t)a[0], (int32_t)a[1], (int32_t)a[2], (int32_t)a[3], (float*)(uintptr_t)a[4], (void*)(uintptr_t)a[5]) : MOPA_ERR_ARG;
+    case 140: return nargs == 6 ? mopa_wino4_weight_f((const float*)(uintptr_t)a[0], (int32_t)a[1], (int32_t)a[2], (int32_t)a[3], (float*)(uintptr_t)a[4], (void*)(uintptr_t)a[5]) : MOPA_ERR_ARG;
+    case 141: return nargs == 6 ? mopa_wino4_weight_q((const float*)(uintptr_t)a[0], (int32_t)a[1], (int32_t)a[2], (int32_t)a[3], (float*)(uintptr_t)a[4], (void*)(uintptr_t)a[5]) : MOPA_ERR_ARG;
+    case 142: return nargs == 6 ? mopa_wino4_weight_t((const float*)(uintptr_t)a[0], (int32_t)a[1], (int32_t)a[2], (int32_t)a[3], (float*)(uintptr_t)a[4], (void*)(uintptr_t)a[5]) : MOPA_ERR_ARG;
+    case 143: return nargs == 17 ? mopa_wino4_wgrad_fused((const float*)(uintptr_t)a[0], (int32_t)a[1], (const float*)(uintptr_t)a[2], (int32_t)a[3], (int32_t)a[4], (const float*)(uintptr_t)a[5], (int32_t)a[6], (int32_t)a[7], (int32_t)a[8], (int32_t)a[9], (int32_t)a[10], (int32_t)a[11], (float*)(uintptr_t)a[12], (int32_t)a[13], (void*)(uintptr_t)a[14], (size_t)a[15], (void*)(uintptr_t)a[16]) : MOPA_ERR_ARG;
+    case 144: return nargs == 10 ? mopa_wino_bwd_weight((const float*)(uintptr_t)a[0], (const float*)(uintptr_t)a[1], (int32_t)a[2], (int32_t)a[3], (int32_t)a[4], (float*)(uintptr_t)a[5], (int32_t)a[6], (void*)(uintptr_t)a[7], (size_t)a[8], (void*)(uintptr_t)a[9]) : MOPA_ERR_ARG;
+    case 145: return nargs == 8 ? mopa_wino_dout((const float*)(uintptr_t)a[0], (int32_t)a[1], (int32_t)a[2], (int32_t)a[3], (int32_t)a[4], (int32_t)a[5], (float*)(uintptr_t)a[6], (void*)(uintptr_t)a[7]) : MOPA_ERR_ARG;
+    case 146: return nargs == 8 ? mopa_wino_input((const float*)(uintptr_t)a[0], (int32_t)a[1], (int32_t)a[2], (int32_t)a[3], (int32_t)a[4], (int32_t)a[5], (float*)(uintptr_t)a[6], (void*)(uintptr_t)a[7]) : MOPA_ERR_ARG;
+    case 147: return nargs == 10 ? mopa_wino_output((const float*)(uintptr_t)a[0], (int32_t)a[1], (int32_t)a[2], (int32_t)a[3], (int32_t)a[4], (const float*)(uintptr_t)a[5], (float*)(uintptr_t)a[6], (int32_t)a[7], (int32_t)a[8], (void*)(uintptr_t)a[9]) : MOPA_ERR_ARG;
+    case 148: return nargs == 6 ? mopa_wino_weight((const float*)(uintptr_t)a[0], (int32_t)a[1], (int32_t)a[2], (int32_t)a[3], (float*)(uintptr_t)a[4], (void*)(uintptr_t)a[5]) : MOPA_ERR_ARG;
+    case 149: return nargs == 5 ? mopa_zero_rows((float*)(uintptr_t)a[0], (int32_t)a[1], (int64_t)a[2], (int32_t)a[3], (void*)(uintptr_t)a[4]) : MOPA_ERR_ARG;
     default: return MOPA_ERR_ARG;
   }
 }
diff --git a/mopa_amd/csrc/rows.hip b/mopa_amd/csrc/rows.hip
--- a/mopa_amd/csrc/rows.hip
+++ b/mopa_amd/csrc/rows.hip
@@ -271,13 +271,6 @@
   return yv > 0.f ? g : g * leak;
 }
 
-__device__ __forceinline__ float bn_dz_bit(float g, float leak, int act, bool pos) {
-  if (!act) return g;
-  return pos ? g : g * leak;
-}
-__device__ __forceinline__ uint32_t bn_mask_nibble(const uint32_t* __restrict__ bits, int64_t row, int C, int cq) {
-  return bits[row * (C >> 5) + (cq >> 3)] >> ((cq & 7) * 4);
-}
 
 struct BnRowsMask {
   const float* __restrict__ dy; int ld_dy; const float* __restrict__ ymask; int ld_ym;
diff --git a/mopa_amd/csrc/wino2d.hip b/mopa_amd/csrc/wino2d.hip
--- a/mopa_amd/csrc/wino2d.hip
+++ b/mopa_amd/csrc/wino2d.hip
@@ -233,8 +233,10 @@
   }
 }
 
+template <bool RES>
 __global__ __launch_bounds__(256) void k_wino4_out(const float* __restrict__ M, int B, int H, int W, int C, int th, int tw,
-                                                    const float* __restrict__ bias, float* __restrict__ out, int ld_out, int accumulate) {
+                                                    const float* __restrict__ bias, float* __restrict__ out, int ld_out, int accumulate,
+                                                    const ResShare res) {
   const int64_t T = (int64_t)B * th * tw;
   const int64_t total = T * C;
   for (int64_t i = blockIdx.x * (int64_t)blockDim.x + threadIdx.x; i < total; i += (int64_t)gridDim.x * blockDim.x) {
@@ -266,9 +268,16 @@
       for (int c = 0; c < 4; ++c) {
         const int x = 4 * tx + c;
         if (x >= W) continue;
-        float* p = out + ((int64_t)(b * H + y) * W + x) * ld_out + ch;
+        const int64_t row = (int64_t)(b * H + y) * W + x;
+        float* p = out + row * ld_out + ch;
         float v = o[c] + bv;
-        if (accumulate) v += *p;
+        if (RES) {
+          float r = bn_dz_bit(res.dy[row * res.ld + ch], 0.f, res.act, (bn_mask_nibble(res.bits, row, res.C, ch >> 2) >> (ch & 3)) & 1u);
+          asm volatile("" : "+v"(r));
+          v += r;
+        } else if (accumulate) {
+          v += *p;
+        }
         *p = v;
       }
     }
@@ -337,7 +346,19 @@
                                int32_t accumulate, void* stream) {
   if (B <= 0 || H <= 0 || W <= 0 || C <= 0 || ld_out < C) return MOPA_ERR_ARG;
   const int th = (H + 3) / 4, tw = (W + 3) / 4;
-  k_wino4_out<<<stream_grid((int64_t)B * th * tw * C, 256), 256, 0, (hipStream_t)stream>>>(M, B, H, W, C, th, tw, bias, out, ld_out, accumulate);
+  k_wino4_out<false><<<stream_grid((int64_t)B * th * tw * C, 256), 256, 0, (hipStream_t)stream>>>(M, B, H, W, C, th, tw, bias, out, ld_out, accumulate,
+                                                                                                  ResShare{nullptr, nullptr, 0, 0, 0});
+  MOPA_CHECK_LAUNCH();
+  return MOPA_OK;
+}
+MOPA_API int mopa_wino4_output_res(const float* M, int32_t B, int32_t H, int32_t W, int32_t C, const float* bias, float* out, int32_t ld_out,
+                                   const float* res_dy, int32_t ld_res, const uint32_t* bits, int32_t C_total, float leak, int32_t act,
+                                   void* stream) {
+  if (B <= 0 || H <= 0 || W <= 0 || C <= 0 || ld_out < C || !M || !out) return MOPA_ERR_ARG;
+  if (!res_dy || !bits || C_total <= 0 || (C_total & 31) || C > C_total || leak != 0.f || ld_res < C) return MOPA_ERR_ARG;
+  const int th = (H + 3) / 4, tw = (W + 3) / 4;
+  k_wino4_out<true><<<stream_grid((int64_t)B * th * tw * C, 256), 256, 0, (hipStream_t)stream>>>(M, B, H, W, C, th, tw, bias, out, ld_out, 0,
+                                                                                                 ResShare{res_dy, bits, ld_res, C_total, act});
   MOPA_CHECK_LAUNCH();
   return MOPA_OK;
 }
diff --git a/mopa_amd/csrc/wino4c9.hip b/mopa_amd/csrc/wino4c9.hip
--- a/mopa_amd/csrc/wino4c9.hip
+++ b/mopa_amd/csrc/wino4c9.hip
@@ -14,6 +14,7 @@
   const float* in; const float* Uq; const float* bias; float* out; const float* stats;
   int ld_in, ld_out, B, H, W, th, tw, T, Cin, Cout, accumulate, imgs_per_group, bn_c0, nco;
   long long* prof;
+  ResShare res;
 };
 
 __device__ __forceinline__ void c9_bt(float d0, float d1, float d2, float d3, float d4, float d5, float& t0, float& t1, float& t2, float& t3,
@@ -200,7 +201,8 @@
   const int stl = t0 + (t >> 4), sq = (t & 15) * 4;
   const f32x4c bv = a.bias ? *reinterpret_cast<const f32x4c*>(a.bias + co0 + sq) : (f32x4c){0.f, 0.f, 0.f, 0.f};
   const int sb_ = stl / thw, sr_ = stl - sb_ * thw, sty = sr_ / tw, stx = sr_ - sty * tw;
-  float* __restrict__ obase = a.out + ((int64_t)(sb_ * H + 4 * sty) * W + 4 * stx) * a.ld_out + co0 + sq;
+  const int64_t spix = (int64_t)(sb_ * H + 4 * sty) * W + 4 * stx;
+  float* __restrict__ obase = a.out + spix * a.ld_out + co0 + sq;
   for (int i = 0; i < 4; ++i) {
 #pragma unroll
     for (int e = 0; e < 16; ++e) {
@@ -230,7 +232,18 @@
             if (AT[j][b] != 0.f) y += AT[j][b] * tt[b];
           if (4 * stx + j < W) {
             f32x4c* __restrict__ op = reinterpret_cast<f32x4c*>(o + (int64_t)j * a.ld_out);
-            *op = a.accumulate ? *op + y : y;
+            if (a.res.dy) {
+              const int64_t row = spix + (int64_t)i * W + j;
+              const f32x4c gq = *reinterpret_cast<const f32x4c*>(a.res.dy + row * a.res.ld + co0 + sq);
+              const uint32_t mw = bn_mask_nibble(a.res.bits, row, a.res.C, (co0 + sq) >> 2);
+              f32x4c r;
+#pragma unroll
+              for (int e = 0; e < 4; ++e) r[e] = bn_dz_bit(gq[e], 0.f, a.res.act, (mw >> e) & 1u);
+              asm volatile("" : "+v"(r));
+              *op = r + y;
+            } else {
+              *op = a.accumulate ? *op + y : y;
+            }
           }
         }
       }
@@ -245,9 +258,9 @@
 }
 
 
-MOPA_API int mopa_wino4_conv9(const float* in, int32_t ld_in, const float* Uq, const float* bias, float* out, int32_t ld_out, int32_t B, int32_t H,
-                              int32_t W, int32_t Cin, int32_t Cout, int32_t accumulate, const float* stats, int32_t n_groups, int32_t bn_c0,
-                              void* stream) {
+static int wino4_conv9_run(const float* in, int32_t ld_in, const float* Uq, const float* bias, float* out, int32_t ld_out, int32_t B, int32_t H,
+                           int32_t W, int32_t Cin, int32_t Cout, int32_t accumulate, const float* stats, int32_t n_groups, int32_t bn_c0,
+                           const ResShare& res, void* stream) {
   if (B <= 0 || H <= 0 || W <= 0 || Cin <= 0 || Cout <= 0 || Cin % C9_KC || Cout % C9_CN || ld_in < Cin || ld_out < Cout ||
       ((uintptr_t)Uq & 15) || ((uintptr_t)out & 15) || (ld_out & 3) || ((uintptr_t)bias & 15) || !in || !Uq || !out)
     return MOPA_ERR_ARG;
@@ -258,7 +271,7 @@
   a.ld_in = ld_in; a.ld_out = ld_out; a.B = B; a.H = H; a.W = W; a.th = (H + 3) / 4; a.tw = (W + 3) / 4;
   const int64_t T = (int64_t)B * a.th * a.tw;
   if (T >= (1 << 30)) return MOPA_ERR_ARG;
-  a.T = (int)T; a.Cin = Cin; a.Cout = Cout; a.accumulate = accumulate;
+  a.T = (int)T; a.Cin = Cin; a.Cout = Cout; a.accumulate = accumulate; a.res = res;
   a.imgs_per_group = stats ? B / n_groups : 1;
   a.bn_c0 = stats ? bn_c0 : 0;
   a.nco = Cout / C9_CN;
@@ -285,3 +298,20 @@
 #endif
   return MOPA_OK;
 }
+
+MOPA_API int mopa_wino4_conv9(const float* in, int32_t ld_in, const float* Uq, const float* bias, float* out, int32_t ld_out, int32_t B, int32_t H,
+                              int32_t W, int32_t Cin, int32_t Cout, int32_t accumulate, const float* stats, int32_t n_groups, int32_t bn_c0,
+                              void* stream) {
+  return wino4_conv9_run(in, ld_in, Uq, bias, out, ld_out, B, H, W, Cin, Cout, accumulate, stats, n_groups, bn_c0,
+                         ResShare{nullptr, nullptr, 0, 0, 0}, stream);
+}
+MOPA_API int mopa_wino4_conv9_res(const float* in, int32_t ld_in, const float* Uq, const float* bias, float* out, int32_t ld_out, int32_t B,
+                                  int32_t H, int32_t W, int32_t Cin, int32_t Cout, const float* res_dy, int32_t ld_res,
+                                  const uint32_t* bits, int32_t C_total, float leak, int32_t act, const float* stats, int32_t n_groups,
+                                  int32_t bn_c0, void* stream) {
+  if (!res_dy || !bits || C_total <= 0 || (C_total & 31) || Cout > C_total || leak != 0.f || ld_res < Cout || (ld_res & 3) ||
+      ((uintptr_t)res_dy & 15))
+    return MOPA_ERR_ARG;
+  return wino4_conv9_run(in, ld_in, Uq, bias, out, ld_out, B, H, W, Cin, Cout, 0, stats, n_groups, bn_c0,
+                         ResShare{res_dy, bits, ld_res, C_total, act}, stream);
+}
diff --git a/mopa_amd/dense2d.py b/mopa_amd/dense2d.py
--- a/mopa_amd/dense2d.py
+++ b/mopa_amd/dense2d.py
@@ -212,6 +212,9 @@
 
 
 F4_FORMS = ("F4", "F4 fused", "F4 one", "F4 one9")
+RES_EPILOGUE = os.environ.get("MOPA_RES_EPILOGUE", "1") != "0"
+F4_RES_FORMS = ("F4", "F4 one9")
+RES_EPILOGUE_MIN_TILES = int(os.environ.get("MOPA_RES_EPILOGUE_MIN_TILES", "2560"))
 
 
 def wino4_layout(cin, cout, B, H, W, role="fwd", want_v=False):
@@ -241,7 +244,7 @@
     return (ptr(bn[0]), bn[1], bn[2]) if bn is not None else (None, 1, 0)
 
 
-def wino_conv(x_p, ld_in, B, H, W, cin, cout, U, bias, out_p, ld_out, accumulate=False, F=2, bn_in=None, role="fwd", want_v=True):
+def wino_conv(x_p, ld_in, B, H, W, cin, cout, U, bias, out_p, ld_out, accumulate=False, F=2, bn_in=None, role="fwd", want_v=True, res=None):
     T, NP = B * ((H + F - 1) // F) * ((W + F - 1) // F), (F + 2) ** 2
     sfx = "" if F == 2 else "4"
     form = wino4_layout(cin, cout, B, H, W, role, want_v) if F == 4 else 0
@@ -249,7 +252,13 @@
         raise RuntimeError(f"wino_conv: this shape, role and want_v take the weight form wino_weight_cached(..., F={F}, transposed={form})")
     if bn_in is not None and F != 4:
         raise RuntimeError("wino_conv: a deferred BatchNorm needs the F(4x4) input transform")
+    if res is not None and (F != 4 or F4_FORMS[form] not in F4_RES_FORMS or accumulate):
+        raise RuntimeError("wino_conv: this form has no residual output mode (ask conv_plan(...).dgrad_res(B, H, W) first)")
+    res_args = () if res is None else (res[0].p, res[0].ld, ptr(res[1]), res[1].shape[1] * 32, 0.0, int(res[2]))
     V = torch.empty(NP * T * cin, dtype=torch.float32, device=U.device) if form < 2 or want_v else None
+    if form == 3 and res is not None:
+        call("mopa_wino4_conv9_res", x_p, ld_in, ptr(U), ptr(bias), out_p, ld_out, B, H, W, cin, cout, *res_args, *_bn_args(bn_in), stream())
+        return None
     if form == 3:
         call("mopa_wino4_conv9", x_p, ld_in, ptr(U), ptr(bias), out_p, ld_out, B, H, W, cin, cout, int(accumulate), *_bn_args(bn_in), stream())
         return None
@@ -266,7 +275,10 @@
     M = torch.empty(NP * T * cout, dtype=torch.float32, device=U.device)
     g1 = _geom(B=1, IH=1, IW=T, OHl=1, OWl=T, OHa=1, OWa=T, TH=1, TW=1, KWF=1, Cin=cin, Cout=cout, ld_in=cin, ld_out=cout)
     igemm_batched(ptr(V), ptr(U), ptr(M), g1, NP, T * cin, cin * cout, T * cout)
-    call(f"mopa_wino{sfx}_output", ptr(M), B, H, W, cout, ptr(bias), out_p, ld_out, int(accumulate), stream())
+    if res is not None:
+        call("mopa_wino4_output_res", ptr(M), B, H, W, cout, ptr(bias), out_p, ld_out, *res_args, stream())
+    else:
+        call(f"mopa_wino{sfx}_output", ptr(M), B, H, W, cout, ptr(bias), out_p, ld_out, int(accumulate), stream())
     return V
 
 
@@ -384,6 +396,10 @@
     dgrad: str
     dgrad_layout: int
 
+    def dgrad_res(self, B, H, W) -> bool:
+        T = B * ((H + 3) // 4) * ((W + 3) // 4)
+        return RES_EPILOGUE and (self.dgrad == "F4" or (self.dgrad == "F4 one9" and T >= RES_EPILOGUE_MIN_TILES))
+
 
 def conv_plan(cin, cout, k, s, p, B, H, W, training) -> ConvPlan:
     a = (cin, cout, k, s, p, B, H, W)
@@ -435,7 +451,7 @@
         igemm(x.p, wl, self.b, out.p, self._fwd_geom(x, out))
 
     def backward(self, x: Img, dout: Img, dx: Img | None, dw: torch.Tensor, db, acc_dx: bool, acc_params: bool = False, V=None,
-                 wgrad_side: bool = False, db_partial=None):
+                 wgrad_side: bool = False, db_partial=None, res=None):
         dev = self.w.device
         k, s, p = self.k, self.s, self.p
         plan = conv_plan(self.I, self.O, k, s, p, x.B, x.H, x.W, True)
@@ -449,12 +465,14 @@
                 wgrad(x.p, dout.p, ptr(dw), self._fwd_geom(x, dout), dev, accumulate=acc_params, oihw=True)
             if db is not None:
                 colsum(dout, db, accumulate=acc_params, partial=db_partial)
+        if res is not None and (dx is None or acc_dx or not plan.dgrad_res(x.B, x.H, x.W)):
+            raise RuntimeError("ConvOp.backward: a residual share was left to a backward-data kernel that cannot form it")
         if dx is None:
             return
         if plan.dgrad != "direct":
             F = int(plan.dgrad[1])
             wino_conv(dout.p, dout.ld, x.B, x.H, x.W, self.O, self.I, wino_weight_cached(self.w, True, F, plan.dgrad_layout), None, dx.p,
-                      dx.ld, acc_dx, F=F, role="dgrad", want_v=False)
+                      dx.ld, acc_dx, F=F, role="dgrad", want_v=False, res=res)
             return
         wt = relayout_cached(self.w, (k, k, self.O, self.I), self.O, self.I, k, k, 1)
         if s == 1:
@@ -652,9 +670,16 @@
 
 class BnOp:
 
-    def __init__(self, P, name, act=1, res=None, G=1, biased=False, stem_grid=None):
+    def __init__(self, P, name, act=1, res=None, G=1, biased=False, stem_grid=None, res_conv=None):
         self.P, self.name, self.act, self.res, self.G, self.biased, self.stem_grid = P, name, act, res, G, biased, stem_grid
+        self.res_conv = res_conv
         self.x = self.y = self.stats = self.gathered = self.bits = None
+
+    def leaves_dres(self, training, acc_dres, want_dimg=False) -> bool:
+        if self.res_conv is None or self.res is None or acc_dres or self.bits is None or self.plan(training, want_dimg).bwd != "fused":
+            return False
+        r = self.res
+        return conv_plan(*self.res_conv, r.B, r.H, r.W, True).dgrad_res(r.B, r.H, r.W)
 
     def plan(self, training, want_dimg=False, C=None, keep_tape=True, deferred=False) -> BnPlan:
         ran, stem = self.x is not None, self.stem_grid is not None
@@ -793,7 +818,7 @@
                 lvl = li + 1
                 J[lvl] = torch.empty(z.rows, 2 * c, dtype=torch.float32, device=dev)
                 out = Img(J[lvl], z.B, z.H, z.W, 0, c)
-            x = bn(q + "bn2", z, act=1, res=idt, out=out)
+            x = bn(q + "bn2", z, act=1, res=idt, out=out, res_conv=None if has_ds else (P[q + "conv1.weight"].shape[1], c, 3, 1, 1))
         if lname == "layer3":
             J[3] = torch.empty(x.rows, 2 * c, dtype=torch.float32, device=dev)
             x = dropout(x, 0, out=Img(J[3], x.B, x.H, x.W, 0, c))
@@ -846,6 +871,7 @@
     pre = "net_2d."
     B, Hp, Wp = feat.B, feat.H, feat.W
     gmap = {}
+    res_left = {}
     dimg = None
 
     def key(v):
@@ -866,7 +892,10 @@
         if kind == "bn":
             op = rec[1]
             dy = gmap.pop(key(op.y))
-            dres, acc_dres = grad_of(op.res) if op.res is not None else (None, False)
+            if op.res is not None and op.leaves_dres(training, key(op.res) in gmap, want_dimg):
+                dres, acc_dres, res_left[key(op.res)] = None, False, (dy, op.bits, op.act)
+            else:
+                dres, acc_dres = grad_of(op.res) if op.res is not None else (None, False)
             (dg, db), pacc = sink.take(op.name + ".weight", op.name + ".bias")
             gmap[key(op.x)] = op.backward(dy, dres, acc_dres, training, dg, db, pacc, want_dimg)
         elif kind == "conv":
@@ -875,7 +904,7 @@
             dx, acc = grad_of(x)
             pg, pacc = sink.take(*([name + ".weight"] + ([name + ".bias"] if op.b is not None else [])))
             op.backward(x, dout, dx, pg[0], pg[1] if op.b is not None else None, acc, acc_params=pacc, V=V, wgrad_side=True,
-                        db_partial=getattr(dout, "partial", None))
+                        db_partial=getattr(dout, "partial", None), res=res_left.pop(key(x), None))
         elif kind == "convT":
             _, name, op, x, out = rec
             dout = gmap.pop(key(out))
@@ -927,6 +956,7 @@
             if want_dimg:
                 dimg = torch.empty(B, 3, H, W, dtype=torch.float32, device=dev)
                 call("mopa_stem_dgrad_image", dout.p, dout.ld, B, Hp, Wp, H, W, ptr(P[pre + "conv1.weight"]), ptr(dimg), stream())
+    assert not res_left, "a residual share was left to a convolution that never came"
     join_wgrad_stream(dev)
     return dimg
 
```

After: 424.0, median of 6. About the same (+0.3%).
